# jzombie/rust-simd-r-drive

Measured on AMD Instinct MI355X. Metric: GiB/s hashed (device-resident), full-file validate+index scan, higher is better.
Workload: dtype u8

## Files before the change

include/srd_amd.h:

```cpp
#ifndef SRD_AMD_H
#define SRD_AMD_H
#include <stddef.h>
#include <stdint.h>

#ifdef __cplusplus
extern "C" {
#endif

#define SRD_OK 0
#define SRD_ERR_HIP (-1)
#define SRD_ERR_ALLOC (-2)
#define SRD_ERR_ARG (-3)
#define SRD_ERR_INTERNAL (-4)

#define SRD_MODE_OPTIMISTIC 0
#define SRD_MODE_FULL 1
#define SRD_MODE_SPAN_UNPROVEN 3

#define SRD_FULL_NONE 0
#define SRD_FULL_FORCED 1
#define SRD_FULL_SLOT_SPACE 2
#define SRD_FULL_WAVES 3
#define SRD_FULL_NO_START 4
#define SRD_FULL_UNPROVEN 5
#define SRD_FULL_CAP 6
#define SRD_FULL_LOOKBACK 7

#define SRD_FLAG_FORCE_FULL 1u
#define SRD_FLAG_NO_CRC 2u
#define SRD_FLAG_STAGE_PAGEABLE 4u
#define SRD_FLAG_STAGE_REGISTER 8u

typedef struct srd_ctx srd_ctx;

int srd_ctx_create(int device, srd_ctx **out);
void srd_ctx_destroy(srd_ctx *ctx);
void *srd_ctx_stream(srd_ctx *ctx);
uint64_t srd_ctx_device_bytes(srd_ctx *ctx);
int srd_ctx_scan_loads(srd_ctx *ctx);
int srd_ctx_scan_trial(srd_ctx *ctx, double *ms);
#define SRD_SCAN_BLOCKS_LAST 0
#define SRD_SCAN_BLOCKS_NEXT 1
#define SRD_SCAN_BLOCKS_EVEN 0
#define SRD_SCAN_BLOCKS_MEASURED 1
#define SRD_SCAN_BLOCKS_INSTALLED 2
typedef struct {
  uint64_t n_spans;
  uint32_t n_blocks;
  uint32_t source;
  uint32_t attempts;
  uint32_t first_source;
} srd_scan_blocks_info;
int srd_ctx_set_scan_blocks(srd_ctx *ctx, const uint64_t *starts,
                            uint32_t n_blocks, uint64_t n_spans);
int srd_ctx_scan_blocks(srd_ctx *ctx, int which, uint64_t *starts,
                        uint32_t cap, srd_scan_blocks_info *info);
const char *srd_last_error(void);
const char *srd_build_info(void);
#define SRD_TIMING_NONE 0
#define SRD_TIMING_SCAN 1
#define SRD_TIMING_CALL 2
int srd_ctx_set_timing(srd_ctx *ctx, int level);
int srd_ctx_set_timing_every(srd_ctx *ctx, int n);

int srd_ctx_timings(srd_ctx *ctx, double *scan_ms, int *scan_launches,
                    double *total_ms);
int srd_ctx_scan_list(srd_ctx *ctx, float *out, int cap);

typedef struct {
  uint64_t file_len;
  uint64_t final_len;
  uint64_t n_chain;
  uint64_t n_index;
  uint64_t n_crc_bad;
  uint64_t n_candidates;
  uint64_t full_reason;
  uint32_t mode;
  uint32_t reserved;
  uint64_t *meta_off, *key_hash, *prev_offset, *payload_start, *payload_len;
  uint32_t *crc_stored, *crc_computed;
  uint8_t *crc_ok;
  uint64_t *index_key_hash, *index_packed;
} srd_device_result;

uint64_t srd_padded_size(uint64_t file_len);

int srd_validate_index_device(srd_ctx *ctx, const uint8_t *d_file,
                              uint64_t file_len, uint32_t flags,
                              srd_device_result *out);

int srd_validate_span_device(srd_ctx *ctx, const uint8_t *d_span,
                             uint64_t span_off, uint64_t lo, uint64_t hi,
                             uint32_t flags, srd_device_result *out);

int srd_shard_cuts(const uint8_t *file, uint64_t file_len, uint32_t world,
                   uint64_t *cuts);

int srd_index_partition_device(srd_ctx *ctx, const uint64_t *d_keys,
                               const uint64_t *d_vals, uint64_t n,
                               uint32_t world, uint64_t *d_out_pairs,
                               uint64_t *counts);

int srd_index_build_device(srd_ctx *ctx, const uint64_t *d_pairs, uint64_t n,
                           uint64_t *d_out_keys, uint64_t *d_out_packed,
                           uint64_t *n_index);

typedef srd_device_result srd_result;
int srd_validate_index(srd_ctx *ctx, const uint8_t *file, uint64_t file_len,
                       uint32_t flags, srd_result *out);
void srd_result_free(srd_result *res);

int srd_validate_index_multi(srd_ctx *const *ctxs, uint32_t n_ctx,
                             const uint8_t *file, uint64_t file_len,
                             uint32_t flags, srd_result *out);

#define SRD_FLAG_MERGE_INDEX 16u
#define SRD_MULTI_COMPOSED 0u
#define SRD_MULTI_NEIGHBOUR 1u
#define SRD_MULTI_WHOLE_FILE 2u
typedef struct {
  uint64_t file_len, final_len;
  uint64_t n_chain, n_index, n_crc_bad, n_candidates;
  uint32_t mode;
  uint32_t path;
  uint32_t n_shards;
  uint32_t merged;
  uint32_t shard_errors;
  uint32_t peer_errors;
  double validate_ms;
  double exchange_ms;
  double total_ms;
  uint64_t *index_key_hash, *index_packed;
} srd_multi_summary;
int srd_validate_index_multi_device(srd_ctx *const *ctxs, uint32_t n_ctx,
                                    const uint8_t *const *d_spans,
                                    const uint64_t *span_offs,
                                    const uint64_t *cuts, uint32_t flags,
                                    srd_device_result *shards,
                                    srd_multi_summary *summary);
int srd_ctx_multi_summary(srd_ctx *ctx, srd_multi_summary *out);
int srd_ctx_multi_shard_ms(srd_ctx *ctx, double *out, int cap);
int srd_ctx_stage_info(srd_ctx *ctx, int *mode, double *stage_ms);

int srd_index_hash_device(srd_ctx *ctx, const uint64_t *d_keys, uint64_t n,
                          uint64_t *d_out, void *stream);

int srd_stream_probe_device(srd_ctx *ctx, const uint8_t *d_buf, uint64_t bytes,
                            int reps, double *best_ms, double *median_ms);

int srd_recover_valid_chain(srd_ctx *ctx, const uint8_t *file,
                            uint64_t file_len, uint64_t *final_len);

int srd_key_indexer_build(srd_ctx *ctx, const uint8_t *file, uint64_t tail,
                          uint64_t *key_hash_out, uint64_t *packed_out,
                          uint64_t cap, uint64_t *n_out);

int srd_crc32_batch(srd_ctx *ctx, const uint8_t *buf, uint64_t buf_len,
                    const uint64_t *offs, const uint64_t *lens, uint64_t n,
                    uint32_t *out);
int srd_crc32_batch_device(srd_ctx *ctx, const uint8_t *d_buf,
                           const uint64_t *d_offs, const uint64_t *d_lens,
                           uint64_t n, uint32_t *d_out, void *stream);

int srd_xxh3_64_batch(srd_ctx *ctx, const uint8_t *keys, uint64_t keys_len,
                      const uint64_t *offs, const uint64_t *lens, uint64_t n,
                      uint64_t *out);
int srd_xxh3_64_batch_device(srd_ctx *ctx, const uint8_t *d_keys,
                             const uint64_t *d_offs, const uint64_t *d_lens,
                             uint64_t n, uint64_t *d_out, void *stream);

#define SRD_WRITE_ALLOW_NULL 1u

typedef struct {
  uint64_t src;
  uint64_t len;
  uint64_t key_src;
  uint64_t tail;
  uint32_t key_len;
  uint32_t flags;
} srd_write_entry;
#define SRD_ENTRY_TOMB 1u
#define SRD_ENTRY_HASHED 2u

int srd_batch_layout(uint64_t tail, const uint8_t *payloads,
                     const uint64_t *key_offs, const uint64_t *key_lens,
                     const uint64_t *pay_offs, const uint64_t *pay_lens,
                     uint64_t n, uint32_t flags, srd_write_entry *out,
                     uint64_t *new_tail);

int srd_batch_write(srd_ctx *ctx, uint64_t tail, const uint8_t *keys,
                    const uint64_t *key_offs, const uint64_t *key_lens,
                    const uint8_t *payloads, const uint64_t *pay_offs,
// ... 119 lines not shown
```

rust-simd-r-drive_amd/csrc/srd_ctx.hip:

```cpp
static thread_local std::string g_err;
static void set_err(const std::string& s) { g_err = s; }

#define HIPCHK(x)                                                                         \
  do {                                                                                    \
    hipError_t e_ = (x);                                                                  \
    if (e_ != hipSuccess) {                                                               \
      set_err(std::string(#x) + ": " + hipGetErrorString(e_));                            \
      return SRD_ERR_HIP;                                                                 \
    }                                                                                     \
  } while (0)

namespace {

#define TRY(x)                 \
  do {                         \
    int r_ = (x);              \
    if (r_) return r_;         \
  } while (0)

static int launched(hipStream_t s, const char* name) {
  static const bool sync = [] { const char* e = getenv("SRD_SYNC_DEBUG"); return e && *e && *e != '0'; }();
  HIPCHK(hipGetLastError());
  if (!sync) return 0;
  hipError_t e = hipStreamSynchronize(s);
  if (e == hipSuccess) e = hipGetLastError();
  if (e == hipSuccess) return 0;
  set_err(std::string("kernel ") + name + ": " + hipGetErrorString(e));
  fprintf(stderr, "srd: kernel %s failed: %s\n", name, hipGetErrorString(e));
  return SRD_ERR_HIP;
}
#define LAUNCHED(s, name) TRY(launched(s, name))

struct Buf {
  void* p = nullptr;
  size_t n = 0;
};

struct CandCap {
  uint32_t cap;
  uint32_t grown_cap;
  uint64_t grown_bytes;
  uint32_t floor;
};

struct Worker {
  std::thread th;
  std::mutex mu;
  std::condition_variable cv;
  std::function<void()> job;
  bool has = false, stop = false;
  Worker() {
    th = std::thread([this] {
      std::unique_lock<std::mutex> lk(mu);
      for (;;) {
        cv.wait(lk, [this] { return has || stop; });
        if (!has) return;
        lk.unlock();
        job();
        lk.lock();
        has = false;
        job = nullptr;
        cv.notify_all();
      }
    });
  }
  ~Worker() {
    {
      std::lock_guard<std::mutex> lk(mu);
      stop = true;
    }
    cv.notify_all();
    th.join();
  }
  void post(std::function<void()> f) {
    std::lock_guard<std::mutex> lk(mu);
    job = std::move(f);
    has = true;
    cv.notify_all();
  }
  void wait() {
    std::unique_lock<std::mutex> lk(mu);
    cv.wait(lk, [this] { return !has; });
  }
};

struct Ctx {
  int device = 0;
  hipStream_t stream = nullptr;
  std::vector<Buf> bufs;
  CandCap copt{8, 8, 0, 8};
  CandCap cfull{32, 32, 0, 32};
  unsigned scan_blocks = 256;
  unsigned scan_cus = 256;
  uint32_t scan_wq[16] = {};
  uint32_t scan_variant = 0;
  uint64_t slot_limit = 1ull << 31;
  int loads_pin = -1;
  int last_loads = -1;
  struct LoadTune {
    uint64_t ns = ~0ull;
    uint32_t g = 0;
    uint32_t calls = 0;
    uint64_t best[2] = {0, 0};
    uint32_t n[2] = {0, 0};
    int choice = -1;
  } tune;
  bool glue_fused = true;
  uint32_t lb_fail = ~0u;
  bool xpart_on = true, xp_valid = false;
  uint32_t xp_par = 0, xp_g = 0;
  uint64_t xp_ns = 0;
  bool xp_installed = false;
  struct LastPart {
    bool any = false;
    uint64_t ns = 0;
    uint32_t g = 0, src = 0, par = 0;
    uint32_t attempts = 0, first_src = 0;
  } xp_last;
  srd_device_result res{};
  Buf file;
  hipEvent_t ev[4] = {nullptr, nullptr, nullptr, nullptr};
  int timing = SRD_TIMING_NONE;
  static constexpr uint32_t kScanRing = 64;
  hipEvent_t sev[2 * kScanRing] = {};
  uint32_t sev_next = 0, sev_pending = 0;
  double scan_ms = 0, total_ms = 0;
  int scan_launches = 0;
  uint32_t timing_every = 1, timing_seq = 0;
  std::vector<float> scan_list, scan_last;
  uint32_t gen = 0;
  uint64_t last_n = 0;
  Plan* h_plan = nullptr;
  uint64_t* h_pub = nullptr;
  uint64_t* h_small = nullptr;
  uint32_t pub_seq = 0;
  hipStream_t cstream = nullptr;
  hipEvent_t wev_copied[2] = {nullptr, nullptr}, wev_done[2] = {nullptr, nullptr};
  void* pin_ent[2] = {nullptr, nullptr};
  int stage_workers = 8;
  int stage_mode = -1;
  double stage_ms = 0;
  bool ev3_recorded = false;
  std::vector<void*> stage_pin;
  std::vector<hipStream_t> stage_streams;
  std::vector<hipEvent_t> stage_ev;
  srd_multi_summary last_multi{};
  std::vector<double> last_shard_ms;
  void* h_out = nullptr;
  uint64_t h_out_n = 0;
  uint8_t lgen = 0;
  Worker* worker = nullptr;
  hipEvent_t ev_ready = nullptr;
  bool ready_recorded = false;
};

enum BufId {
  B_TILE, B_SPAN_COUNT, B_SPAN_BASE,
  B_CM, B_CREC,
  B_COUNTERS,
  B_DM, B_DPAR, B_DSLOT, B_DHEAD, B_RUNHEAD, B_INTS, B_WALK,
  B_ST, B_JMP, B_VFLAG, B_VLIST, B_NV, B_VPOS, B_VPAR, B_VHEAD, B_VSLOT,
  B_ONPATH, B_CPOS, B_CHAIN_G, B_CORE,
  B_O_MO, B_O_KH, B_O_PREV, B_O_START, B_O_LEN, B_O_CRCST, B_O_CRC, B_O_OK,
  B_O_PIECES, B_O_SUF, B_O_SXM, B_O_TAIL, B_SLOW,
  B_HKEYS, B_HVALS, B_LATEST, B_IPOS, B_IKEY, B_IPACKED,
  B_CUB_TMP,
  B_PLAN, B_HASCHILD, B_CHILDOF, B_FLAG, B_PART, B_PARTEX, B_HOFF, B_SKEY, B_SIDX, B_LATEST8, B_XPART,
  B_MPLAN, B_MKEY, B_MVAL, B_PCNT, B_POFF, B_HASCHILD2,
  B_WPAY0, B_WPAY1, B_WKEY0, B_WKEY1, B_WENT0, B_WENT1, B_WKH, B_WMO,
  B_IT_FLAG, B_IT_POS, B_IT_ST, B_IT_EN, B_IT_KEPT, B_IT_OST, B_IT_OEN, B_IT_OKH, B_IT_ENT, B_IT_RLEN, B_IT_PST,
  B_GKEY, B_GVAL, B_GOKEY, B_GOPACKED,
  B_WTOT, B_WROOT, B_KTOT, B_DONE, B_SPAN_FIRST,
  B_XKEY, B_XVAL, B_GATHER, B_RFLAG, B_O_PACKED, B_VSCAN, B_LOOKB, B_PROBE, B_XTOT,
  B_LV_DSLOT, B_LV_DTOMB, B_LV_LSLOT, B_LV_OPS, B_LV_OPV, B_LV_CNT,
  B_LV_XK, B_LV_XP, B_LV_FLAG, B_LV_POS, B_LV_ENT, B_LV_TOMB,
  B_GA_ST, B_GA_PLEN, B_GA_CHK, B_GA_OFF, B_GA_CPRE, B_GA_CNT, B_GA_UNIT, B_GA_RAW, B_GA_CRC,
  B_AP_END, B_AP_NZ,
  B_CL_XK, B_CL_XP, B_CL_LEN, B_CL_MO, B_CL_PACKED, B_CL_CNT,
  B_COUNT_
};

int ensure(Ctx* c, BufId id, size_t bytes) {
  Buf& b = c->bufs[id];
  if (b.n >= bytes && b.p) return 0;
  if (b.p) HIPCHK(hipFree(b.p));
  b.p = nullptr;
  b.n = 0;
  size_t want = std::max<size_t>(bytes, 256);
  if (hipMalloc(&b.p, want) != hipSuccess) {
    set_err("hipMalloc failed for " + std::to_string(want) + " bytes");
    b.p = nullptr;
    return SRD_ERR_ALLOC;
  }
  b.n = want;
  return 0;
}
template <class T>
T* P(Ctx* c, BufId id) { return (T*)c->bufs[id].p; }

int ensure_z(Ctx* c, BufId id, size_t bytes) {
  void* before = c->bufs[id].p;
  size_t nb = c->bufs[id].n;
  int r = ensure(c, id, bytes);
  if (r) return r;
  if (c->bufs[id].p != before || c->bufs[id].n != nb) HIPCHK(hipMemsetAsync(c->bufs[id].p, 0, c->bufs[id].n, c->stream));
  return 0;
}

const CrcTables& host_tabs() {
  static CrcTables t;
  static const bool built = (build_crc_tables(t), true);
  (void)built;
  return t;
}

int upload_tables() {
  static std::mutex mu;
  std::lock_guard<std::mutex> lk(mu);
  const CrcTables& ht = host_tabs();
  int dev = 0;
  HIPCHK(hipGetDevice(&dev));
  static uint64_t uploaded = 0;
  if (uploaded & (1ull << dev)) return 0;
  DevTables t;
  memcpy(t.tab, ht.tab, sizeof t.tab);
  memcpy(t.lw, ht.lw, sizeof t.lw);
  memcpy(t.winit, ht.winit, sizeof t.winit);
  memcpy(t.zero_crc, ht.zero_crc, sizeof t.zero_crc);
  t.x32768 = ht.x32768;
  t.xtile[0] = kX0;
  for (int e = 1; e <= 64; e++) t.xtile[e] = mulp(ht.x32768, t.xtile[e - 1]);
  t.xt64[0] = kX0;
  for (int q = 1; q <= 64; q++) t.xt64[q] = mulp(t.xtile[64], t.xt64[q - 1]);
  for (int tb = 0; tb < 4; tb++)
    for (int b = 0; b < 256; b++) t.mx64[tb][b] = mulp(t.xtile[64], (uint32_t)b << (8 * tb));
  memcpy(t.pow8, ht.pow8, sizeof t.pow8);
  memcpy(t.invpow, ht.invpow, sizeof t.invpow);
  memcpy(t.m16k, ht.m16k, sizeof t.m16k);
  memcpy(t.m32k, ht.m32k, sizeof t.m32k);
  memcpy(t.mtk, ht.mtk, sizeof t.mtk);
  for (int pos = 0; pos < 8; pos++)
    for (int nb = 0; nb < 16; nb++)
      for (int l = 0; l < 32; l++)
        t.nib[((pos * 16 + nb) << 5) + l] = mulp(ht.lw[l + 32], (uint32_t)nb << (4 * pos));
  {
    for (int tb = 0; tb < 4; tb++)
      for (int b = 0; b < 256; b++) {
        for (int q = 0; q < 3; q++) {
          t.last[q][tb][b] = mulp(host_xpow8(ht, 4 + 16 * (3 - q)), (uint32_t)b << (8 * tb));
          t.last_c[q][tb][b] = mulp(host_xpow8(ht, 4 + 1024 * (3 - q)), (uint32_t)b << (8 * tb));
        }
        t.m4096[tb][b] = mulp(host_xpow8(ht, 512), (uint32_t)b << (8 * tb));
      }
    for (int pos = 0; pos < 8; pos++)
      for (int nb = 0; nb < 16; nb++)
        for (int l = 0; l < 32; l++)
          t.nib_c[((pos * 16 + nb) << 5) + l] = mulp(host_xpow8(ht, 16 * (31 - l)), (uint32_t)nb << (4 * pos));
  }
  HIPCHK(hipMemcpyToSymbol(HIP_SYMBOL(g_tabs), &t, sizeof t));
  uploaded |= 1ull << dev;
  return 0;
// ... 32 lines not shown
};
template <class T>
static SmallRead rd(const T* src, T* dst) { return SmallRead{src, dst, sizeof(T)}; }
static int read_small(Ctx* c, hipStream_t s, std::initializer_list<SmallRead> reads) {
  uint64_t* w = c->h_small + 8;
  for (const SmallRead& r : reads) {
    if (w + (r.bytes + 7) / 8 > c->h_small + 32) { set_err("internal: read_small over its pinned area"); return SRD_ERR_INTERNAL; }
    if (r.bytes) HIPCHK(hipMemcpyAsync(w, r.src, r.bytes, hipMemcpyDeviceToHost, s));
    w += (r.bytes + 7) / 8;
  }
  HIPCHK(spin_sync(s));
  w = c->h_small + 8;
  for (const SmallRead& r : reads) {
    if (r.bytes) memcpy(r.dst, w, r.bytes);
    w += (r.bytes + 7) / 8;
  }
  return 0;
}
static int enqueue_counters(Ctx* c) {
  HIPCHK(hipMemcpyAsync(c->h_small, P<uint64_t>(c, B_COUNTERS), 8 * 8, hipMemcpyDeviceToHost, c->stream));
  return 0;
}
static void counters_landed(Ctx* c, uint64_t* h) { memcpy(h, c->h_small, 64); }
int read_counters(Ctx* c, uint64_t* h, const uint64_t* extra_src = nullptr, uint64_t* extra = nullptr) {
  TRY(enqueue_counters(c));
  if (extra_src) TRY(read_small(c, c->stream, {rd(extra_src, extra)}));
  else HIPCHK(spin_sync(c->stream));
  counters_landed(c, h);
  return 0;
}

template <class In, class Out>
static int ensure_scan(Ctx* c, In in, Out out, uint64_t n) {
  size_t tb = 0;
  HIPCHK(hipcub::DeviceScan::ExclusiveSum(nullptr, tb, in, out, (int)n));
  return ensure(c, B_CUB_TMP, tb + 256);
}
template <class In, class Out>
static int scan_max(Ctx* c, In in, Out out, uint64_t n) {
  size_t tb = c->bufs[B_CUB_TMP].n;
  HIPCHK(hipcub::DeviceScan::InclusiveScan(P<void>(c, B_CUB_TMP), tb, in, out, hipcub::Max(), (int)n, c->stream));
  LAUNCHED(c->stream, "hipcub");
  return 0;
}
template <class In, class Out>
static int scan_sum(Ctx* c, In in, Out out, uint64_t n, hipStream_t s = nullptr) {
  if (!s) s = c->stream;
  size_t tb = c->bufs[B_CUB_TMP].n;
  HIPCHK(hipcub::DeviceScan::ExclusiveSum(P<void>(c, B_CUB_TMP), tb, in, out, (int)n, s));
  LAUNCHED(s, "hipcub");
  return 0;
}
template <class T, class U>
static int scan_sum_total(Ctx* c, T* in, U* out, uint64_t n, hipStream_t s, uint64_t* total, SmallRead r1 = {},
                          SmallRead r2 = {}, SmallRead r3 = {}) {
  if (!s) s = c->stream;
  TRY(scan_sum(c, in, out, n, s));
  U prefix{};
  typename std::remove_const<T>::type term{};
  TRY(read_small(c, s, {rd(out + n - 1, &prefix), rd(in + n - 1, &term), r1, r2, r3}));
  *total = (uint64_t)prefix + term;
  return 0;
}
static int sort_pairs48(Ctx* c, const uint64_t* kin, uint64_t* kout, const uint64_t* vin, uint64_t* vout, uint64_t n) {
  size_t tb = 0;
  HIPCHK(hipcub::DeviceRadixSort::SortPairs(nullptr, tb, kin, kout, vin, vout, (int)n, 0, 48, c->stream));
  TRY(ensure(c, B_CUB_TMP, tb + 256));
  tb = c->bufs[B_CUB_TMP].n;
  HIPCHK(hipcub::DeviceRadixSort::SortPairs(P<void>(c, B_CUB_TMP), tb, kin, kout, vin, vout, (int)n, 0, 48, c->stream));
  LAUNCHED(c->stream, "hipcub");
  return 0;
}

}

struct srd_ctx : Ctx {};

static int drain_scan_events(Ctx* c, uint32_t n) {
  for (; n && c->sev_pending; n--) {
    const uint32_t i = (c->sev_next - c->sev_pending) % Ctx::kScanRing;
    float ms = 0;
    HIPCHK(hipEventElapsedTime(&ms, c->sev[2 * i], c->sev[2 * i + 1]));
    c->scan_ms += ms;
    c->scan_launches++;
    if (c->scan_list.size() < (1u << 16)) c->scan_list.push_back(ms);
    c->sev_pending--;
  }
  return 0;
}
static int next_scan_events(Ctx* c, hipEvent_t* e0, hipEvent_t* e1) {
  *e0 = *e1 = nullptr;
  if (c->timing < SRD_TIMING_SCAN) return 0;
  if (c->timing_seq++ % c->timing_every) return 0;
  if (c->sev_pending == Ctx::kScanRing) TRY(drain_scan_events(c, 1));
  const uint32_t i = c->sev_next++ % Ctx::kScanRing;
  c->sev_pending++;
  *e0 = c->sev[2 * i];
  *e1 = c->sev[2 * i + 1];
  return 0;
}

static void weights_to_shares(const double (&f)[16], uint32_t (&wq)[16]) {
  double sum = 0;
  for (double x : f) sum += x;
  uint32_t used = 0;
  for (int v = 0; v < 15; v++) used += wq[v] = (uint32_t)(65536.0 * f[v] / sum);
  wq[15] = 65536 - used;
}

static void scan_weights(uint32_t (&wq)[16]) {
  double f[16] = {1.0000, 0.9787, 0.9796, 0.9788, 0.9081, 0.9072, 0.9074, 0.8915,
                  0.8432, 0.8324, 0.8337, 0.8314, 0.7726, 0.7701, 0.7712, 0.7590};
  if (const char* e = getenv("SRD_SCAN_WEIGHTS")) {
    double g[16], gs = 0;
    int n = 0;
    for (const char* q = e; n < 16 && *q;) {
      char* end = nullptr;
      const double x = strtod(q, &end);
      if (end == q || !(x > 0) || !std::isfinite(x)) { n = 0; break; }
      g[n++] = x;
      gs += x;
      q = *end == ',' ? end + 1 : end;
      if (*end && *end != ',') { n = 0; break; }
    }
    if (!std::isfinite(gs)) n = 0;
    if (n == 4)
      for (int v = 0; v < 16; v++) f[v] = g[v / 4];
    else if (n == 16)
      for (int v = 0; v < 16; v++) f[v] = g[v];
  }
  weights_to_shares(f, wq);
}
#ifdef SRD_DEBUG_API
extern "C" int srd_debug_set_scan_variant(srd_ctx* c, int v) {
  if (!c || !(v == 0 || v == 7 || v == 8 || v == SCAN_LINES)) return SRD_ERR_ARG;
  c->scan_variant = (uint32_t)v;
  return 0;
}
extern "C" int srd_debug_set_scan_bpc(srd_ctx* c, int bpc) {
  if (!c || bpc < 1 || bpc > 2) return SRD_ERR_ARG;
  c->scan_blocks = c->scan_cus * (unsigned)bpc;
  return 0;
}
extern "C" int srd_debug_set_xpart(srd_ctx* c, int on) {
  if (!c) return SRD_ERR_ARG;
  c->xpart_on = on != 0;
  return 0;
}
extern "C" int srd_debug_set_glue_fused(srd_ctx* c, int fused) {
  if (!c) return SRD_ERR_ARG;
  c->glue_fused = fused != 0;
  return 0;
}
extern "C" int srd_debug_set_scan_weights(srd_ctx* c, const double* w, int n) {
  if (!c || !w || (n != 4 && n != 16)) return SRD_ERR_ARG;
  double f[16], sum = 0;
  for (int v = 0; v < 16; v++) {
    sum += f[v] = n == 4 ? w[v / 4] : w[v];
    if (!(f[v] > 0) || !std::isfinite(f[v])) return SRD_ERR_ARG;
  }
  if (!std::isfinite(sum)) return SRD_ERR_ARG;
  weights_to_shares(f, c->scan_wq);
  return 0;
}
#endif
static int ctx_init(srd_ctx* c, int device) {
  c->device = device;
  c->bufs.resize(B_COUNT_);
  if (hipStreamCreateWithFlags(&c->stream, hipStreamNonBlocking) != hipSuccess) {
    set_err("hipStreamCreate failed");
    return SRD_ERR_HIP;
  }
  TRY(upload_tables());
  for (auto& e : c->ev) HIPCHK(hipEventCreateWithFlags(&e, hipEventReleaseToDevice));
  HIPCHK(hipEventCreateWithFlags(&c->ev_ready, hipEventDisableTiming));
  HIPCHK(hipHostMalloc((void**)&c->h_plan, sizeof(Plan), hipHostMallocDefault));
  HIPCHK(hipHostMalloc((void**)&c->h_pub, 64, hipHostMallocCoherent));
  memset(c->h_pub, 0, 64);
  HIPCHK(hipHostMalloc((void**)&c->h_small, 256, hipHostMallocDefault));
  c->stage_workers = (int)std::max(1u, std::min(8u, std::thread::hardware_concurrency()));
  int ncu = 0;
  if (hipDeviceGetAttribute(&ncu, hipDeviceAttributeMultiprocessorCount, device) == hipSuccess && ncu > 0)
    c->scan_cus = c->scan_blocks = (unsigned)ncu;
  scan_weights(c->scan_wq);
  if (const char* e = getenv("SRD_SLOT_LIMIT_LOG2")) {
    const long v = strtol(e, nullptr, 10);
    if (v >= 10 && v <= 31) c->slot_limit = 1ull << v;
  }
  if (const char* e = getenv("SRD_SCAN_LOADS")) {
    if (!strcmp(e, "lines")) c->loads_pin = SCAN_LINES;
    else if (!strcmp(e, "coal")) c->loads_pin = 0;
  }
  if (const char* e = getenv("SRD_GLUE_FUSED")) c->glue_fused = strcmp(e, "0") != 0;
  if (const char* e = getenv("SRD_XPART")) c->xpart_on = strcmp(e, "0") != 0;
  if (const char* e = getenv("SRD_LB_FAIL_BLOCK")) {
    char* end = nullptr;
    const unsigned long v = strtoul(e, &end, 10);
    if (end != e && v < CHAIN_BLOCKS) c->lb_fail = (uint32_t)v;
  }
  return 0;
}

extern "C" int srd_ctx_create(int device, srd_ctx** out) {
  if (!out) { set_err("null out"); return SRD_ERR_ARG; }
  int n = 0;
  HIPCHK(hipGetDeviceCount(&n));
  if (device < 0 || device >= n) { set_err("bad device index"); return SRD_ERR_ARG; }
  HIPCHK(hipSetDevice(device));
  auto* c = new srd_ctx();
  const int r = ctx_init(c, device);
  if (r) {
    srd_ctx_destroy(c);
    return r;
  }
  *out = c;
  return 0;
}

extern "C" void srd_ctx_destroy(srd_ctx* c) {
  if (!c) return;
  delete c->worker;
  hipSetDevice(c->device);
  if (c->ev_ready) hipEventDestroy(c->ev_ready);
  for (auto& b : c->bufs)
    if (b.p) hipFree(b.p);
  if (c->file.p) hipFree(c->file.p);
  for (auto& e : c->ev)
    if (e) hipEventDestroy(e);
  for (auto& e : c->sev)
    if (e) hipEventDestroy(e);
  if (c->h_plan) hipHostFree(c->h_plan);
  if (c->h_pub) hipHostFree(c->h_pub);
  if (c->h_small) hipHostFree(c->h_small);
  if (c->h_out) hipHostFree(c->h_out);
  for (int i = 0; i < 2; i++) {
    if (c->pin_ent[i]) hipHostFree(c->pin_ent[i]);
    if (c->wev_copied[i]) hipEventDestroy(c->wev_copied[i]);
    if (c->wev_done[i]) hipEventDestroy(c->wev_done[i]);
  }
  if (c->cstream) hipStreamDestroy(c->cstream);
  for (auto p : c->stage_pin)
    if (p) hipHostFree(p);
  for (auto e : c->stage_ev)
    if (e) hipEventDestroy(e);
  for (auto st : c->stage_streams)
    if (st) hipStreamDestroy(st);
  if (c->stream) hipStreamDestroy(c->stream);
  delete c;
}

extern "C" void* srd_ctx_stream(srd_ctx* c) { return c ? (void*)c->stream : nullptr; }
extern "C" int srd_ctx_scan_loads(srd_ctx* c) { return c ? c->last_loads : -1; }
extern "C" int srd_ctx_scan_trial(srd_ctx* c, double* ms) {
  if (!c) return -1;
  if (ms)
    for (int k = 0; k < 2; k++) ms[k] = c->tune.n[k] ? (double)c->tune.best[k] * 1e-5 : 0.0;
  return c->tune.choice;
}
extern "C" int srd_ctx_set_scan_blocks(srd_ctx* c, const uint64_t* starts, uint32_t n_blocks, uint64_t n_spans) {
  if (!c || !starts) { set_err("bad argument"); return SRD_ERR_ARG; }
  if (!c->xpart_on) { set_err("XCD-aware block shares are off on this context (SRD_XPART=0)"); return SRD_ERR_ARG; }
  if (!part_table_ok(starts, n_blocks, n_spans)) {
    set_err("bad argument: not a block-start table of n_blocks blocks over n_spans spans (srd_ctx_set_scan_blocks)");
    return SRD_ERR_ARG;
  }
  HIPCHK(hipSetDevice(c->device));
  TRY(ensure_z(c, B_XPART, sizeof(XPart)));
  HIPCHK(hipMemcpyAsync(&P<XPart>(c, B_XPART)->bs[c->xp_par][0], starts, ((size_t)n_blocks + 1) * 8,
                        hipMemcpyHostToDevice, c->stream));
  HIPCHK(hipStreamSynchronize(c->stream));
  c->xp_valid = true;
  c->xp_installed = true;
  c->xp_ns = n_spans;
  c->xp_g = n_blocks;
  return 0;
}
extern "C" int srd_ctx_scan_blocks(srd_ctx* c, int which, uint64_t* starts, uint32_t cap,
                                   srd_scan_blocks_info* info) {
  if (!c || !info || (cap && !starts) || (which != SRD_SCAN_BLOCKS_LAST && which != SRD_SCAN_BLOCKS_NEXT)) {
    set_err("bad argument");
    return SRD_ERR_ARG;
  }
  *info = srd_scan_blocks_info{};
  const Ctx::LastPart& l = c->xp_last;
  uint32_t par = 0;
  if (which == SRD_SCAN_BLOCKS_LAST) {
    if (!l.any) return 0;
    info->n_spans = l.ns;
    info->n_blocks = l.g;
    info->source = l.src;
    info->attempts = l.attempts;
    info->first_source = l.first_src;
    par = l.par;
  } else {
    if (!c->xp_valid) return 0;
    info->n_spans = c->xp_ns;
    info->n_blocks = c->xp_g;
    info->source = c->xp_installed ? SRD_SCAN_BLOCKS_INSTALLED : SRD_SCAN_BLOCKS_MEASURED;
    par = c->xp_par;
  }
  const size_t n = std::min<size_t>(cap, (size_t)info->n_blocks + 1);
  if (!n) return 0;
  if (info->source == SRD_SCAN_BLOCKS_EVEN) {
    for (size_t b = 0; b < n; b++) starts[b] = b * info->n_spans / info->n_blocks;
    return 0;
  }
  HIPCHK(hipSetDevice(c->device));
  HIPCHK(hipMemcpyAsync(starts, &P<XPart>(c, B_XPART)->bs[par][0], n * 8, hipMemcpyDeviceToHost, c->stream));
  HIPCHK(hipStreamSynchronize(c->stream));
  return 0;
}
extern "C" uint64_t srd_ctx_device_bytes(srd_ctx* c) {
  if (!c) return 0;
  uint64_t n = c->file.n;
  for (const Buf& b : c->bufs) n += b.n;
  return n;
}

extern "C" int srd_ctx_set_timing(srd_ctx* c, int level) {
  if (!c || level < SRD_TIMING_NONE || level > SRD_TIMING_CALL) { set_err("bad argument"); return SRD_ERR_ARG; }
  if (level >= SRD_TIMING_SCAN && !c->sev[0]) {
    HIPCHK(hipSetDevice(c->device));
    for (auto& e : c->sev) HIPCHK(hipEventCreateWithFlags(&e, hipEventReleaseToDevice));
  }
  c->timing = level;
  return 0;
}

extern "C" int srd_ctx_set_timing_every(srd_ctx* c, int n) {
  if (!c || n < 1) { set_err("bad argument"); return SRD_ERR_ARG; }
  c->timing_every = (uint32_t)n;
  c->timing_seq = 0;
  return 0;
}

extern "C" int srd_ctx_timings(srd_ctx* c, double* scan_ms, int* scan_launches, double* total_ms) {
  if (!c) { set_err("bad argument"); return SRD_ERR_ARG; }
  HIPCHK(hipSetDevice(c->device));
  TRY(drain_scan_events(c, c->sev_pending));
  if (scan_ms) *scan_ms = c->scan_ms;
  if (scan_launches) *scan_launches = c->scan_launches;
  if (total_ms) *total_ms = c->total_ms;
  c->scan_ms = 0;
  c->scan_launches = 0;
  c->scan_last.swap(c->scan_list);
  c->scan_list.clear();
  return 0;
}

extern "C" int srd_ctx_scan_list(srd_ctx* c, float* out, int cap) {
  if (!c || (cap > 0 && !out)) { set_err("bad argument"); return SRD_ERR_ARG; }
  const int n = (int)std::min<size_t>(c->scan_last.size(), (size_t)std::max(cap, 0));
  for (int i = 0; i < n; i++) out[i] = c->scan_last[i];
  return (int)c->scan_last.size();
}
```

rust-simd-r-drive_amd/csrc/srd_glue.hip:

```cpp
#pragma once

namespace srd {

#define GST(ptr, val) srd_gst(&(ptr), (val))

struct Plan {
  uint64_t K;
  uint64_t n_chain;
  uint64_t root_t;
  uint64_t start;
  uint64_t n_index;
  uint64_t n_bad;
  uint64_t n_slow;
  uint64_t chain_core;
  uint64_t max_root, top_gap, overflow;
  uint32_t status;
  uint32_t nroot;
  uint32_t troot;
  uint32_t idx_overflow;
  uint32_t idx_alias;
};
constexpr uint32_t ST_NOSTART = 1, ST_SHAPE = 2, ST_ROOTS = 4, ST_OVERFLOW = 16;
constexpr uint64_t NO_NODE = ~0ull;

constexpr int GLUE_BLOCKS = 1024;
constexpr int GLUE_THREADS = 256;

__device__ __forceinline__ uint32_t block_rank256(bool f, uint32_t* wsum, uint32_t* total) {
  const int lane = threadIdx.x & 63, w = threadIdx.x >> 6;
  const uint64_t bal = __ballot(f);
  const uint32_t pre = (uint32_t)__popcll(bal & ((1ull << lane) - 1));
  if (lane == 0) wsum[w] = (uint32_t)__popcll(bal);
  __syncthreads();
  uint32_t off = 0, tot = 0;
#pragma unroll
  for (int i = 0; i < 4; i++) {
    const uint32_t v = wsum[i];
    off += i < w ? v : 0u;
    tot += v;
  }
  __syncthreads();
  *total = tot;
  return off + pre;
}

template <int NW>
__device__ __forceinline__ uint32_t block_rank_n(bool f, uint32_t* wsum, uint32_t* total) {
  const int lane = threadIdx.x & 63, w = threadIdx.x >> 6;
  const uint64_t bal = __ballot(f);
  const uint32_t pre = (uint32_t)__popcll(bal & ((1ull << lane) - 1));
  if (lane == 0) wsum[w] = (uint32_t)__popcll(bal);
  __syncthreads();
  uint32_t off = 0, tot = 0;
#pragma unroll
  for (int i = 0; i < NW; i++) {
    const uint32_t v = wsum[i];
    off += i < w ? v : 0u;
    tot += v;
  }
  __syncthreads();
  *total = tot;
  return off + pre;
}
template <int NW>
__device__ __forceinline__ uint32_t block_sum_n(uint32_t v, uint32_t* wsum) {
  const int lane = threadIdx.x & 63, w = threadIdx.x >> 6;
#pragma unroll
  for (int o = 32; o; o >>= 1) v += __shfl_xor(v, o);
  if (lane == 0) wsum[w] = v;
  __syncthreads();
  uint32_t t = 0;
#pragma unroll
  for (int i = 0; i < NW; i++) t += wsum[i];
  __syncthreads();
  return t;
}
constexpr int CHAIN_BLOCKS = 256;
constexpr int CHAIN_THREADS = 1024;
constexpr int CHAIN_WAVES = CHAIN_THREADS / 64;

__device__ __forceinline__ uint32_t block_sum256(uint32_t v, uint32_t* wsum) {
  const int lane = threadIdx.x & 63, w = threadIdx.x >> 6;
#pragma unroll
  for (int o = 32; o; o >>= 1) v += __shfl_xor(v, o);
  if (lane == 0) wsum[w] = v;
  __syncthreads();
  const uint32_t t = wsum[0] + wsum[1] + wsum[2] + wsum[3];
  __syncthreads();
  return t;
}

__device__ __forceinline__ void chunk_of(uint64_t n, uint64_t* lo, uint64_t* hi) {
  const uint64_t ch = (n + gridDim.x - 1) / gridDim.x;
  *lo = min(n, (uint64_t)blockIdx.x * ch);
  *hi = min(n, *lo + ch);
}

__device__ __forceinline__ void block_prefix(const uint32_t* part, uint32_t np, uint32_t* wsum, uint64_t* before,
                                             uint64_t* total) {
  uint32_t b = 0, t = 0;
  for (uint32_t i = threadIdx.x; i < np; i += blockDim.x) {
    const uint32_t v = part[i];
    t += v;
    b += i < blockIdx.x ? v : 0u;
  }
  *before = block_sum256(b, wsum);
  *total = block_sum256(t, wsum);
}



__device__ uint64_t block_scan_partials(const uint32_t* part, uint32_t np, uint32_t* part_ex) {
  __shared__ uint64_t s[1024];
  const uint32_t t = threadIdx.x;
  uint64_t v = t < np ? part[t] : 0;
  s[t] = v;
  __syncthreads();
  for (uint32_t o = 1; o < 1024; o <<= 1) {
    const uint64_t a = t >= o ? s[t - o] : 0;
    __syncthreads();
    s[t] += a;
    __syncthreads();
  }
  if (t < np) part_ex[t] = (uint32_t)(s[t] - v);
  const uint64_t total = s[1023];
  __syncthreads();
  return total;
}

struct ShapeArgs {
  const uint8_t* file;
  uint64_t flen;
  uint32_t gen;
  const uint64_t* Kp;
  const uint64_t* wave_total;
  uint64_t wcap;
  uint32_t n_waves, wpb;
  uint64_t n_slots;
  const uint64_t* c_m;
  const int32_t* d_par;
  const u32x4* c_rec;
  const uint32_t* has_child;
  uint64_t* childof;
  uint8_t* flag;
  uint32_t* part;
  uint32_t* wpart;
  const unsigned long long* counters;
  Plan* plan;
  uint32_t coff;
  uint32_t* zero;
  uint32_t n_zero;
  uint32_t lb_fail;
};

__device__ __forceinline__ uint64_t start_node(const ShapeArgs& a) {
  const uint64_t t = a.counters[1], s1 = a.Kp[1];
  return (s1 && t >= 21 && a.c_m[s1 - 1] == t - 20) ? s1 - 1 : NO_NODE;
}
__device__ __forceinline__ bool dense_incomplete(const ShapeArgs& a) { return a.counters[2] != 0; }

constexpr uint32_t BW_MAX = 64;
__device__ __forceinline__ uint32_t block_waves(const ShapeArgs& a, uint32_t* s_pre) {
  const uint64_t w0 = (uint64_t)blockIdx.x * a.wpb;
  const uint32_t t = threadIdx.x, lane = t & 63;
  if (t < 64) {
    const uint64_t w = w0 + lane;
    const uint32_t c = lane < a.wpb && w < a.n_waves ? (uint32_t)min(a.wave_total[w] & ~(1ull << 63), a.wcap) : 0u;
    uint32_t x = c;
#pragma unroll
    for (int d = 1; d < 64; d <<= 1) {
      const uint32_t y = __shfl_up(x, d);
      if (lane >= (uint32_t)d) x += y;
    }
    s_pre[lane + 1] = x;
    if (lane == 0) s_pre[0] = 0;
  }
  __syncthreads();
  return s_pre[a.wpb];
}
__device__ __forceinline__ uint64_t slot_of(const ShapeArgs& a, const uint32_t* s_pre, uint32_t i) {
  uint32_t v = 0;
  for (uint32_t st = BW_MAX / 2; st; st >>= 1)
    if (v + st < a.wpb && s_pre[v + st] <= i) v += st;
  return ((uint64_t)blockIdx.x * a.wpb + v) * a.wcap + (i - s_pre[v]);
}

__device__ __forceinline__ bool is_core(const ShapeArgs& a, uint64_t g, uint64_t start) {
  if (g == start) return true;
  const int64_t p = a.d_par[g];
  return a.has_child[g] == a.gen && (p >= 0 || p == PAR_ROOT);
}

__global__ __launch_bounds__(256) void marks_from_claims_kernel(ShapeArgs a, uint32_t* marks_out) {
  if (dense_incomplete(a)) return;
  for (uint64_t g = (uint64_t)blockIdx.x * blockDim.x + threadIdx.x; g < a.n_slots; g += (uint64_t)gridDim.x * blockDim.x)
    if ((a.childof[g] >> 32) == a.gen) marks_out[g] = a.gen;
}

__global__ __launch_bounds__(256) void prune_kernel(ShapeArgs a, uint32_t* marks_out, uint32_t gen_out) {
  if (dense_incomplete(a)) return;
  const uint64_t start = start_node(a);
  for (uint64_t g = (uint64_t)blockIdx.x * blockDim.x + threadIdx.x; g < a.n_slots; g += (uint64_t)gridDim.x * blockDim.x) {
    const int64_t p = a.d_par[g];
    if (p >= 0 && is_core(a, g, start)) marks_out[p] = gen_out;
  }
}

__global__ __launch_bounds__(256) void child2_kernel(ShapeArgs a) {
  for (uint32_t i = blockIdx.x * blockDim.x + threadIdx.x; i < a.n_zero; i += gridDim.x * blockDim.x) a.zero[i] = 0;
  if (dense_incomplete(a)) return;
  const uint64_t start = start_node(a);
  const uint64_t K = a.n_slots;
  constexpr int CR = 4;
  const uint64_t stride = (uint64_t)gridDim.x * blockDim.x;
  for (uint64_t g0 = (uint64_t)blockIdx.x * blockDim.x + threadIdx.x; g0 < K; g0 += CR * stride) {
    int64_t par[CR];
    uint32_t hc[CR];
#pragma unroll
    for (int r = 0; r < CR; r++) {
      const uint64_t g = g0 + r * stride, gg = g < K ? g : g0;
      par[r] = a.d_par[gg];
      hc[r] = a.has_child[gg];
    }
#pragma unroll
    for (int r = 0; r < CR; r++) {
      const uint64_t g = g0 + r * stride;
      if (g >= K) break;
      const int64_t p = par[r];
      if (p >= 0 && (g == start || hc[r] == a.gen)) a.childof[p] = claim_word(a.gen, g);
    }
  }
}

enum Shape { SHAPE_LEAF, SHAPE_CORE, SHAPE_ROOT, SHAPE_FAIL };
template <class Linked, class IsStart>
__device__ __forceinline__ Shape shape_test(uint32_t gen, uint64_t g, int64_t p, int64_t pp, uint64_t cp, Linked linked,
                                            IsStart is_start) {
  if (!(is_start(g) || (linked(false) && (p >= 0 || p == PAR_ROOT)))) return SHAPE_LEAF;
  if (p == PAR_ROOT) return SHAPE_ROOT;
  if (p < 0 || !(is_start((uint64_t)p) || (linked(true) && (pp >= 0 || pp == PAR_ROOT)))) return SHAPE_FAIL;
  return cp != claim_word(gen, g) ? SHAPE_FAIL : SHAPE_CORE;
}
__global__ __launch_bounds__(CHAIN_THREADS) void check_kernel(ShapeArgs a) {
  __shared__ uint32_t wsum[CHAIN_WAVES];
  __shared__ uint32_t s_pre[BW_MAX + 1];
  if (dense_incomplete(a)) return;
  const uint64_t start = start_node(a);
  const uint64_t tag = (uint64_t)a.gen << 32;
  const bool marks = a.has_child != nullptr;
  const uint32_t n = block_waves(a, s_pre);
  uint32_t cnt = 0;
  bool fail = false;
  const uint32_t wi = threadIdx.x >> 6, lane = threadIdx.x & 63;
  const uint32_t chunk = (n + CHAIN_WAVES - 1) / CHAIN_WAVES;
  const uint32_t c0 = min(n, wi * chunk), c1 = min(n, c0 + chunk);
  constexpr int CR = 4;
  for (uint32_t base = c0; base < c1; base += CR * 64) {
    uint64_t g[CR], cg[CR], cp[CR];
    int64_t par[CR], pp[CR];
    uint32_t hc[CR], hp[CR];
    bool in[CR];
#pragma unroll
    for (int r = 0; r < CR; r++) {
      const uint32_t i = base + (uint32_t)r * 64 + lane;
      in[r] = i < c1;
      g[r] = slot_of(a, s_pre, in[r] ? i : c0);
      par[r] = a.d_par[g[r]];
      cg[r] = a.childof[g[r]];
      hc[r] = marks ? a.has_child[g[r]] : 0u;
    }
#pragma unroll
    for (int r = 0; r < CR; r++) {
      const uint64_t q = par[r] >= 0 ? (uint64_t)par[r] : g[r];
      pp[r] = a.d_par[q];
      cp[r] = a.childof[q];
      hp[r] = marks ? a.has_child[q] : 0u;
    }
#pragma unroll
    for (int r = 0; r < CR; r++) {
      if (!in[r]) break;
      const Shape s = shape_test(
          a.gen, g[r], par[r], pp[r], cp[r],
          [&](bool parent) {
            return marks ? (parent ? hp[r] : hc[r]) == a.gen : ((parent ? cp[r] : cg[r]) & ~0xffffffffull) == tag;
          },
          [&](uint64_t node) { return node == start; });
      GST(a.flag[g[r]], (uint8_t)(s != SHAPE_LEAF));
      if (s == SHAPE_LEAF) continue;
      cnt++;
      fail = fail || s == SHAPE_FAIL;
      if (s == SHAPE_ROOT) {
        atomicAdd(&a.plan->nroot, 1u);
        const u32x4 r0 = a.c_rec[g[r]];
        a.plan->root_t = (uint64_t)r0[0] | ((uint64_t)r0[1] << 32);
      }
    }
  }
  {
    uint32_t wc = cnt;
#pragma unroll
    for (int o = 32; o; o >>= 1) wc += __shfl_xor(wc, o);
    if (lane == 0) a.wpart[blockIdx.x * CHAIN_WAVES + wi] = wc;
  }
  const uint32_t tot = block_sum_n<CHAIN_WAVES>(cnt, wsum);
  if (__syncthreads_or(fail) && threadIdx.x == 0) atomicOr(&a.plan->status, ST_SHAPE);
  if (threadIdx.x == 0) a.part[blockIdx.x] = tot;
}

constexpr int IDX_HBLOCKS = 256;
constexpr int IDX_TCAP = 2048;
constexpr int IDX_BUCKET_AVG = 1280;
constexpr uint64_t IDX_EMPTY = ~0ull;
constexpr int PUB_WORDS = 7;

struct IdxArgs {
  const uint64_t* kh;
  const uint64_t* mo;
  const uint64_t* n_dev;
  const uint32_t* status;
  uint32_t log2_nbk;
  uint32_t* bfill;
  uint64_t* srec;
  uint8_t* latest;
  uint8_t lgen;
  uint32_t alias;
  uint64_t* pub;
  uint32_t pub_seq;
  uint32_t* ccount;
  const uint64_t* scan_ticks;
  uint64_t* okey;
  uint64_t* opacked;
  Plan* plan;
};

__device__ __forceinline__ uint64_t idx_n(const IdxArgs& a) { return *a.status ? 0 : *a.n_dev; }

template <int NW>
__device__ __forceinline__ void block_prefix_n(const uint32_t* part, uint32_t np, uint32_t* wsum, uint64_t* before,
                                               uint64_t* total) {
  uint32_t b = 0, t = 0;
  for (uint32_t i = threadIdx.x; i < np; i += blockDim.x) {
    const uint32_t v = part[i];
    t += v;
    b += i < blockIdx.x ? v : 0u;
  }
  *before = block_sum_n<NW>(b, wsum);
  *total = block_sum_n<NW>(t, wsum);
}

__device__ __forceinline__ uint32_t idx_bucket(uint64_t key, uint32_t log2_nbk) {
  return (uint32_t)(xxh3_64_u64(key) >> (64 - log2_nbk));
}
__device__ __forceinline__ uint64_t idx_rec(uint64_t hh, uint64_t c) { return (c << 32) | (uint32_t)hh; }

template <int NW, int R>
__device__ __forceinline__ uint32_t block_rank_rounds(const bool* f, uint32_t* wsum, uint32_t* rank) {
  const int lane = threadIdx.x & 63, w = threadIdx.x >> 6;
  const uint64_t lt = (1ull << lane) - 1;
  uint32_t pre[R];
#pragma unroll
  for (int r = 0; r < R; r++) {
    const uint64_t bal = __ballot(f[r]);
    pre[r] = (uint32_t)__popcll(bal & lt);
    if (lane == 0) wsum[r * NW + w] = (uint32_t)__popcll(bal);
  }
  __syncthreads();
  uint32_t acc = 0;
#pragma unroll
  for (int r = 0; r < R; r++) {
    uint32_t off = 0, t = 0;
#pragma unroll
    for (int i = 0; i < NW; i++) {
      const uint32_t v = wsum[r * NW + i];
      off += i < w ? v : 0u;
      t += v;
    }
    rank[r] = acc + off + pre[r];
    acc += t;
  }
  __syncthreads();
  return acc;
}

#ifndef SRD_FIN_R
#define SRD_FIN_R 2
#endif
constexpr int FIN_R = SRD_FIN_R;
constexpr uint32_t WSLOW = 256;

struct FinLds {
  uint32_t tab[1024];
  uint32_t m16k[1024];
  uint32_t m32k[1024];
  uint32_t mtk[3 * 1024];
  uint32_t winit[64], zero_crc[64];
  uint32_t invpow[4097];
};
constexpr int FIN_LDS_WORDS = 13;
__device__ __forceinline__ void fin_lds_words(FinLds& lt, uint32_t ti, uint32_t (&r)[FIN_LDS_WORDS], bool store) {
  static_assert(CHAIN_THREADS == 1024, "one word of each 1024-word table per thread");
  int i = 0;
  auto word = [&](uint32_t& dst, const uint32_t& src, bool mine = true) {
    if (!store) r[i] = src;
    else if (mine) dst = r[i];
    i++;
  };
  word(lt.tab[ti], (&g_tabs.tab[0][0])[ti]);
  word(lt.m16k[ti], (&g_tabs.m16k[0][0])[ti]);
  word(lt.m32k[ti], (&g_tabs.m32k[0][0])[ti]);
#pragma unroll
  for (int j = 0; j < 3; j++) word(lt.mtk[1024 * j + ti], (&g_tabs.mtk[0][0][0])[1024 * j + ti]);
#pragma unroll
  for (int j = 0; j < 4; j++) word(lt.invpow[1024 * j + ti], g_tabs.invpow[1024 * j + ti]);
  word(lt.invpow[4096], g_tabs.invpow[4096], ti == 0);
  word(lt.winit[ti & 63], g_tabs.winit[ti & 63], ti < 64);
  word(lt.zero_crc[ti & 63], g_tabs.zero_crc[ti & 63], ti < 64);
}


__device__ __forceinline__ bool fin_load_record(const ShapeArgs& a, const FinArgs& f, uint64_t gi, bool in, FinIn& e,
                                                uint64_t& kh, int64_t& par, uint32_t& own_suf) {
  const bool fl = in && a.flag[gi];
  par = a.d_par[gi];
  e.mo = f.c_m[gi];
  const u32x4 r0 = f.c_rec[gi], r1 = f.c_rec1[gi];
  e.p = (uint64_t)r0[0] | ((uint64_t)r0[1] << 32);
  kh = (uint64_t)r1[0] | ((uint64_t)r1[1] << 32);
  e.crc_st = r0[3];
  e.sxv = r1[2];
  e.fl = r0[2];
  own_suf = r1[3];
  return fl;
}
__device__ __forceinline__ uint32_t fin_rank(const bool (&fl)[FIN_R], uint64_t lt_mask, uint32_t (&rank)[FIN_R]) {
  uint32_t tot = 0;
#pragma unroll
  for (int r = 0; r < FIN_R; r++) {
    const uint64_t b = __ballot(fl[r]);
    rank[r] = tot + (uint32_t)__popcll(b & lt_mask);
    tot += (uint32_t)__popcll(b);
  }
  return tot;
}
__device__ __forceinline__ void fin_load_tiles(const FinArgs& f, bool fl, FinIn& e) {
  const u32x4* t4 = (const u32x4*)f.tile;
  const uint64_t mo = fl ? e.mo : f.flen - 1;
  const uint64_t st0 = fl ? fin_start(e.fl, e.p) : mo;
  e.t0 = t4[st0 / TILE];
  e.t1 = t4[mo / TILE];
}
struct SlowQueue {
  uint32_t* q;
  uint64_t run0;
  uint32_t n;
  __device__ __forceinline__ void flush(const FinArgs& f) {
    if (!n) return;
    const uint32_t lane = threadIdx.x & 63;
    wave_lds_sync();
    unsigned long long sbase = 0;
    if (lane == 0) sbase = atomicAdd(f.n_slow, (unsigned long long)n);
    sbase = __shfl(sbase, 0);
    for (uint32_t i = lane; i < n; i += 64) f.slow_list[sbase + i] = run0 + q[i];
    wave_lds_sync();
    n = 0;
  }
  __device__ __forceinline__ void push(const FinArgs& f, bool slow, uint64_t c, uint64_t lt_mask) {
    const uint64_t sb = __ballot(slow);
    const uint32_t k = (uint32_t)__popcll(sb);
    if (!k) return;
    if (n + k > WSLOW) flush(f);
    if (slow) q[n + __popcll(sb & lt_mask)] = (uint32_t)(c - run0);
    n += k;
  }
};
__device__ __forceinline__ void fin_emit(const FinArgs& f, const FinLds& lt, uint32_t* hist, uint32_t log2_nbk,
                                         uint64_t run, uint64_t lt_mask, const bool (&fl)[FIN_R],
                                         const uint32_t (&rank)[FIN_R], const FinIn (&e)[FIN_R],
                                         const uint64_t (&kh)[FIN_R], SlowQueue& sq) {
#pragma unroll
  for (int r = 0; r < FIN_R; r++) {
    if (!fl[r]) continue;
    const uint64_t c = run + rank[r];
    GST(f.o_mo[c], e[r].mo);
    GST(f.o_kh[c], kh[r]);
    GST(f.o_packed[c], ((kh[r] >> 48) << 48) | (e[r].mo & 0xFFFFFFFFFFFFull));
    GST(f.o_prev[c], e[r].p);
    GST(f.o_crc_st[c], e[r].crc_st);
    atomicAdd(&hist[idx_bucket(kh[r], log2_nbk)], 1u);
  }
#pragma unroll
  for (int r = 0; r < FIN_R; r++) {
    const uint64_t c = run + rank[r];
    sq.push(f, fl[r] && finalize_in<true>(f, c, e[r], lt), c, lt_mask);
  }
}

constexpr uint32_t ST_LOOKBACK = 32;
#ifdef SRD_GLUE_STAMPS
__device__ uint64_t g_glue_stamp[CHAIN_BLOCKS * 8];
#define GLUE_STAMP(i) \
  do { if (FUSED && threadIdx.x == 0) g_glue_stamp[blockIdx.x * 8 + (i)] = __builtin_amdgcn_s_memrealtime(); } while (0)
#else
#define GLUE_STAMP(i) do {} while (0)
#endif
constexpr uint64_t LB_CNT = (1ull << 35) - 1;
__device__ __forceinline__ uint64_t lb_pack(uint32_t tag, uint32_t st, bool fail, uint32_t nr, uint64_t cnt) {
  return ((uint64_t)tag << 40) | ((uint64_t)st << 38) | ((uint64_t)fail << 37) | ((uint64_t)min(nr, 3u) << 35) |
         (cnt & LB_CNT);
}
__device__ __forceinline__ uint32_t lb_tag(uint32_t gen) { return gen % 0xFFFFFFu + 1u; }
__device__ bool lb_lookback(unsigned long long* desc, uint32_t b, uint32_t tag, uint64_t* cnt, bool* fail,
                            uint32_t* nr) {
  typedef __attribute__((address_space(1))) unsigned long long gu64;
  const uint32_t lane = threadIdx.x & 63;
  uint64_t sum = 0;
  bool f = false;
  uint32_t n = 0;
  uint32_t spins = 0;
  for (int64_t j = (int64_t)b - 1; j >= 0; j -= 64) {
    const int64_t idx = j - (int64_t)lane;
    uint64_t v;
    for (;;) {
      v = idx >= 0 ? __hip_atomic_load((gu64*)(desc + idx), __ATOMIC_RELAXED, __HIP_MEMORY_SCOPE_AGENT)
                   : lb_pack(tag, 2, false, 0, 0);
      const bool ok = (v >> 40) == tag && ((v >> 38) & 3) != 0;
      if (__all(ok)) break;
      if (++spins > (1u << 22)) return false;
      __builtin_amdgcn_s_sleep(2);
    }
    const uint32_t stv = (uint32_t)(v >> 38) & 3u;
    const uint64_t inc = __ballot(stv >= 2);
    const uint32_t first = inc ? (uint32_t)__builtin_ctzll(inc) : 64u;
    const bool take = lane <= first;
    if (__ballot(take && stv == 3)) return false;
    uint64_t c = take ? (v & LB_CNT) : 0;
    uint32_t r = take ? (uint32_t)((v >> 35) & 3) : 0u;
    uint32_t fl = take ? (uint32_t)((v >> 37) & 1) : 0u;
#pragma unroll
    for (int o = 32; o; o >>= 1) {
      c += __shfl_xor(c, o);
      r += __shfl_xor(r, o);
      fl |= __shfl_xor(fl, o);
    }
    sum += c;
    n += r;
    f = f || fl;
    if (inc) break;
  }
  *cnt = sum;
  *fail = f;
  *nr = n;
  return true;
}

__device__ __forceinline__ uint32_t prev_lane(uint32_t v, uint32_t lane0) {
  return (uint32_t)__builtin_amdgcn_update_dpp((int)lane0, (int)v, DPP_WAVE_SHR1, 0xF, 0xF, false);
}
__device__ __forceinline__ uint64_t prev_lane64(uint64_t v, uint64_t lane0) {
  return (uint64_t)prev_lane((uint32_t)v, (uint32_t)lane0) | ((uint64_t)prev_lane((uint32_t)(v >> 32), (uint32_t)(lane0 >> 32)) << 32);
}
__device__ __forceinline__ uint64_t lane63_64(uint64_t v) {
  return (uint64_t)(uint32_t)__builtin_amdgcn_readlane((uint32_t)v, 63) |
         ((uint64_t)(uint32_t)__builtin_amdgcn_readlane((uint32_t)(v >> 32), 63) << 32);
}

template <bool FUSED>
__global__ __launch_bounds__(CHAIN_THREADS) void chain_finalize_kernel(ShapeArgs a, FinArgs f, IdxArgs ia,
                                                                      uint32_t log2_nbk,
                                                                      unsigned long long* lb_desc) {
  __shared__ uint32_t wsum[CHAIN_WAVES * FIN_R];
  __shared__ uint32_t s_pre[BW_MAX + 1];
  __shared__ uint32_t wslow[CHAIN_WAVES][WSLOW];
  __shared__ FinLds lt;
  extern __shared__ uint32_t hist[];
  GLUE_STAMP(0);
  uint32_t ltw[FIN_LDS_WORDS];
  fin_lds_words(lt, threadIdx.x, ltw, false);
  const uint64_t K = a.Kp[0];
  const bool incomplete = dense_incomplete(a);
  uint64_t before = 0, total = 0;
  if constexpr (!FUSED)
    block_prefix_n<CHAIN_WAVES>(a.part, incomplete ? 0u : (uint32_t)CHAIN_BLOCKS, wsum, &before, &total);
  Plan* pl = a.plan;
  uint32_t st = FUSED ? 0u : pl->status;
  const uint64_t top = a.counters[1];
  auto ld_prev_at = [&](uint64_t o) -> uint64_t {
    const uint32_t* q = (const uint32_t*)(a.file + (o & ~3ull));
    const uint32_t sh = (uint32_t)(o & 3) * 8, w0 = q[0], w1 = q[1], w2 = q[2];
    return (uint64_t)alignb(w1, w0, sh) | ((uint64_t)alignb(w2, w1, sh) << 32);
  };
  const bool troot = a.coff && top >= 21 && ld_prev_at(top - 12) == 0;
  uint64_t root_t = troot ? top : FUSED ? 0 : pl->root_t;
  if (a.counters[2]) st |= ST_OVERFLOW;
  const uint64_t s1 = a.Kp[1];
  const uint64_t start = FUSED ? NO_NODE : incomplete ? NO_NODE : start_node(a);
  if (!FUSED && start == NO_NODE) st |= ST_NOSTART;
  if (!FUSED && pl->nroot != 1) st |= ST_ROOTS;
  if (FUSED) st = 0;
  if (!FUSED) __syncthreads();
  const uint32_t nbk = 1u << log2_nbk;
  auto write_plan = [&](uint32_t s2, uint64_t tot) {
    pl->K = K;
    pl->max_root = a.counters[0];
    pl->top_gap = top ? a.flen - top : 0;
    pl->overflow = a.counters[2];
    pl->troot = troot;
    if (troot) {
      pl->status = 0;
      pl->n_chain = 1;
      pl->root_t = top;
      pl->chain_core = 0;
    } else {
      if (!FUSED) pl->start = start;
      pl->status = s2;
      pl->chain_core = tot;
      pl->n_chain = s2 ? 0 : a.coff + tot;
    }
  };
  const bool plan_block = FUSED ? blockIdx.x + 1 == gridDim.x : blockIdx.x == 0;
  if (!FUSED && plan_block && threadIdx.x == 0) write_plan(st, total);
  if (FUSED && troot && plan_block && threadIdx.x == 0) write_plan(0, 0);
  if (st && !troot) return;
  __shared__ uint32_t s_vcnt[BW_MAX];
  __shared__ uint64_t s_lb[2];
  __shared__ uint32_t s_fail, s_nroot, s_lbok;
  __shared__ unsigned long long s_root_t;
  if constexpr (FUSED) {
    if (!troot) {
      if (threadIdx.x == 0) { s_fail = 0; s_nroot = 0; s_root_t = 0; }
      __syncthreads();
      const uint64_t tag = (uint64_t)a.gen << 32;
      const uint32_t wi = threadIdx.x >> 6, lane = threadIdx.x & 63;
      uint32_t nr = 0;
      bool fail = false;
      constexpr int CR = 4;
      for (uint32_t v = wi; v < a.wpb; v += CHAIN_WAVES) {
        const uint64_t w = (uint64_t)blockIdx.x * a.wpb + v;
        const uint32_t n = w < a.n_waves ? (uint32_t)min(a.wave_total[w] & ~(1ull << 63), a.wcap) : 0u;
        const uint64_t gb = w * a.wcap;
        int64_t c_par = PAR_MISS;
        uint64_t c_cg = 0;
        uint32_t cnt = 0;
        for (uint32_t base = 0; base < n; base += CR * 64) {
          uint64_t g[CR], cg[CR], cp[CR];
          int64_t par[CR], pp[CR];
          bool in[CR], need[CR];
#pragma unroll
          for (int r = 0; r < CR; r++) {
            const uint32_t i = base + (uint32_t)r * 64 + lane;
            in[r] = i < n;
            g[r] = gb + (in[r] ? i : 0u);
            par[r] = a.d_par[g[r]];
            cg[r] = a.childof[g[r]];
          }
          bool any = false;
#pragma unroll
          for (int r = 0; r < CR; r++) {
            const uint32_t i = base + (uint32_t)r * 64 + lane;
            const int64_t l0p = r ? (int64_t)(int32_t)__builtin_amdgcn_readlane((uint32_t)par[r - 1], 63) : c_par;
            const uint64_t l0c = r ? lane63_64(cg[r - 1]) : c_cg;
            pp[r] = (int64_t)(int32_t)prev_lane((uint32_t)par[r], (uint32_t)l0p);
            cp[r] = prev_lane64(cg[r], l0c);
            need[r] = in[r] && par[r] >= 0 && !(i > 0 && (uint64_t)par[r] == g[r] - 1);
            any = any || need[r];
          }
          if (__ballot(any)) {
#pragma unroll
            for (int r = 0; r < CR; r++)
              if (need[r]) {
                pp[r] = a.d_par[par[r]];
                cp[r] = a.childof[par[r]];
              }
          }
          c_par = (int64_t)(int32_t)__builtin_amdgcn_readlane((uint32_t)par[CR - 1], 63);
          c_cg = lane63_64(cg[CR - 1]);
#pragma unroll
          for (int r = 0; r < CR; r++) {
            if (!in[r]) break;
            const Shape s = shape_test(
                a.gen, g[r], par[r], pp[r], cp[r],
                [&](bool parent) { return ((parent ? cp[r] : cg[r]) & ~0xffffffffull) == tag; },
                [&](uint64_t node) { return top >= 21 && node == s1 - 1 && a.c_m[node] == top - 20; });
            GST(a.flag[g[r]], (uint8_t)(s != SHAPE_LEAF));
            if (s == SHAPE_LEAF) continue;
            cnt++;
            fail = fail || s == SHAPE_FAIL;
            if (s == SHAPE_ROOT) {
              nr++;
              const u32x4 r0 = a.c_rec[g[r]];
              s_root_t = (uint64_t)r0[0] | ((uint64_t)r0[1] << 32);
            }
          }
        }
#pragma unroll
        for (int o = 32; o; o >>= 1) cnt += __shfl_xor(cnt, o);
        if (lane == 0) s_vcnt[v] = cnt;
      }
#pragma unroll
      for (int o = 32; o; o >>= 1) nr += __shfl_xor(nr, o);
      if (lane == 0 && nr) atomicAdd(&s_nroot, nr);
      if (__ballot(fail) && lane == 0) s_fail = 1;
      __syncthreads();
      GLUE_STAMP(1);
      for (uint32_t k = threadIdx.x; k < nbk; k += blockDim.x) hist[k] = 0;
      fin_lds_words(lt, threadIdx.x, ltw, true);
      uint32_t btot = 0;
      for (uint32_t v = 0; v < a.wpb; v++) btot += s_vcnt[v];
      const uint32_t ltag = lb_tag(a.gen);
      typedef __attribute__((address_space(1))) unsigned long long gu64;
      if (threadIdx.x == 0 && blockIdx.x > 0)
        __hip_atomic_store((gu64*)(lb_desc + blockIdx.x), lb_pack(ltag, 1, s_fail, s_nroot, btot), __ATOMIC_RELAXED,
                           __HIP_MEMORY_SCOPE_AGENT);
      if (wi == 0) {
        uint64_t pc = 0;
        bool pf = false;
        uint32_t pn = 0;
        const bool ok = blockIdx.x != a.lb_fail && lb_lookback(lb_desc, blockIdx.x, ltag, &pc, &pf, &pn);
        if (lane == 0) {
          const bool f2 = pf || s_fail;
          const uint32_t n2 = pn + s_nroot;
          __hip_atomic_store((gu64*)(lb_desc + blockIdx.x),
                             ok ? lb_pack(ltag, 2, f2, n2, pc + btot) : lb_pack(ltag, 3, true, 0, 0), __ATOMIC_RELAXED,
                             __HIP_MEMORY_SCOPE_AGENT);
          s_lb[0] = pc;
          s_lb[1] = pc + btot;
          s_lbok = ok;
          if (plan_block) {
            const uint64_t stn = incomplete ? NO_NODE : start_node(a);
            pl->start = stn;
            write_plan((ok ? 0u : ST_LOOKBACK) | (f2 ? ST_SHAPE : 0u) | (n2 != 1 ? ST_ROOTS : 0u) |
                           (a.counters[2] ? ST_OVERFLOW : 0u) | (stn == NO_NODE ? ST_NOSTART : 0u),
                       pc + btot);
          }
        }
      }
      __syncthreads();
      GLUE_STAMP(2);
      before = s_lb[0];
      total = s_lb[1];
      if (!s_lbok) return;
      root_t = s_root_t;
    }
  }
  if (!FUSED || troot) {
    for (uint32_t k = threadIdx.x; k < nbk; k += blockDim.x) hist[k] = 0;
    fin_lds_words(lt, threadIdx.x, ltw, true);
    __syncthreads();
  }
  GLUE_STAMP(3);
  bool root_slow = false;
  const bool root_block = FUSED && !troot ? root_t != 0 : blockIdx.x == 0;
  if (root_block && a.coff && threadIdx.x == 0) {
    uint64_t kh;
    root_slow = finalize_core<true>(f, 0, NO_REC, -1, root_t, &kh, lt);
    atomicAdd(&hist[idx_bucket(kh, log2_nbk)], 1u);
  }
  uint64_t bend = a.coff + before;
  if (!troot) {
    const uint32_t wi = threadIdx.x >> 6, lane = threadIdx.x & 63;
    const uint64_t lt_mask = (1ull << lane) - 1;
    SlowQueue sq = {wslow[wi], 0, 0};
    if constexpr (FUSED) {
      uint32_t btot = 0;
      for (uint32_t v = 0; v < a.wpb; v++) btot += s_vcnt[v];
      bend += btot;
      for (uint32_t v = wi; v < a.wpb; v += CHAIN_WAVES) {
        const uint64_t w = (uint64_t)blockIdx.x * a.wpb + v;
        const uint32_t n = w < a.n_waves ? (uint32_t)min(a.wave_total[w] & ~(1ull << 63), a.wcap) : 0u;
        const uint64_t gb = w * a.wcap;
        uint32_t voff = 0;
        for (uint32_t u = 0; u < v; u++) voff += s_vcnt[u];
        uint64_t run = a.coff + before + voff;
        sq.run0 = run;
        uint32_t c_fl = F_NO_PARENT, c_suf = 0;
        for (uint32_t base = 0; base < n; base += 64 * FIN_R) {
          bool fl[FIN_R];
          uint64_t gi[FIN_R], kh[FIN_R];
          int64_t par[FIN_R];
          uint32_t psuf[FIN_R], rank[FIN_R];
          FinIn e[FIN_R];
#pragma unroll
          for (int r = 0; r < FIN_R; r++) {
            const uint32_t i = base + (uint32_t)r * 64 + lane;
            gi[r] = gb + (i < n ? i : 0u);
            fl[r] = fin_load_record(a, f, gi[r], i < n, e[r], kh[r], par[r], psuf[r]);
          }
          const uint32_t tot = fin_rank(fl, lt_mask, rank);
          bool any = false, need[FIN_R];
#pragma unroll
          for (int r = 0; r < FIN_R; r++) {
            const uint32_t i = base + (uint32_t)r * 64 + lane;
            const uint32_t l0f = r ? (uint32_t)__builtin_amdgcn_readlane(e[r - 1].fl, 63) : c_fl;
            const uint32_t l0s = r ? (uint32_t)__builtin_amdgcn_readlane(psuf[r - 1], 63) : c_suf;
            const uint32_t nf = prev_lane(e[r].fl, l0f), ns = prev_lane(psuf[r], l0s);
            need[r] = fl[r] && par[r] >= 0 && !(i > 0 && (uint64_t)par[r] == gi[r] - 1);
            any = any || need[r];
            e[r].pfl = par[r] >= 0 ? nf : F_NO_PARENT;
            e[r].psuf = ns;
            fin_load_tiles(f, fl[r], e[r]);
          }
          if (__ballot(any)) {
#pragma unroll
            for (int r = 0; r < FIN_R; r++)
              if (need[r]) {
                e[r].pfl = f.c_rec[par[r]][2];
                e[r].psuf = f.c_rec1[par[r]][3];
              }
          }
          c_fl = (uint32_t)__builtin_amdgcn_readlane(e[FIN_R - 1].fl, 63);
          c_suf = (uint32_t)__builtin_amdgcn_readlane(psuf[FIN_R - 1], 63);
          fin_emit(f, lt, hist, log2_nbk, run, lt_mask, fl, rank, e, kh, sq);
          run += tot;
        }
        sq.flush(f);
      }
    } else {
      const uint32_t n = block_waves(a, s_pre);
      uint32_t woff, btot;
      {
        const uint32_t v = lane < CHAIN_WAVES ? a.wpart[blockIdx.x * CHAIN_WAVES + lane] : 0u;
        uint32_t x = lane < wi ? v : 0u, y = v;
#pragma unroll
        for (int o = 32; o; o >>= 1) {
          x += __shfl_xor(x, o);
          y += __shfl_xor(y, o);
        }
        woff = x;
        btot = y;
      }
      bend += btot;
      uint64_t run = a.coff + before + woff;
      sq.run0 = run;
      const uint32_t chunk = (n + CHAIN_WAVES - 1) / CHAIN_WAVES;
      const uint32_t c0 = min(n, wi * chunk), c1 = min(n, c0 + chunk);
      for (uint32_t base = c0; base < c1; base += 64 * FIN_R) {
        bool fl[FIN_R];
        uint64_t gi[FIN_R], kh[FIN_R];
        int64_t par[FIN_R];
        uint32_t own_suf, rank[FIN_R];
        FinIn e[FIN_R];
#pragma unroll
        for (int r = 0; r < FIN_R; r++) {
          const uint32_t i = base + (uint32_t)r * 64 + lane;
          gi[r] = slot_of(a, s_pre, i < c1 ? i : c0);
          fl[r] = fin_load_record(a, f, gi[r], i < c1, e[r], kh[r], par[r], own_suf);
        }
        const uint32_t tot = fin_rank(fl, lt_mask, rank);
#pragma unroll
        for (int r = 0; r < FIN_R; r++) {
          const uint64_t pg = fl[r] && par[r] >= 0 ? (uint64_t)par[r] : gi[r];
          e[r].pfl = par[r] >= 0 ? f.c_rec[pg][2] : F_NO_PARENT;
          e[r].psuf = f.c_rec1[pg][3];
          fin_load_tiles(f, fl[r], e[r]);
        }
        fin_emit(f, lt, hist, log2_nbk, run, lt_mask, fl, rank, e, kh, sq);
        run += tot;
      }
      sq.flush(f);
    }
  }
  if (root_slow) f.slow_list[atomicAdd(f.n_slow, 1ull)] = 0;
  __syncthreads();
  GLUE_STAMP(4);
  for (uint32_t k = threadIdx.x; k < nbk; k += blockDim.x) {
    const uint32_t n = hist[k];
    hist[k] = n ? atomicAdd(&ia.bfill[k], n) : 0u;
  }
  __syncthreads();
  GLUE_STAMP(5);
  uint64_t clo, chi;
  if constexpr (FUSED) {
    clo = troot ? 0 : a.coff + before;
    chi = troot ? (blockIdx.x == 0 ? 1 : 0) : bend;
    if (!troot && root_block && a.coff && threadIdx.x == 0) {
      const uint64_t h0 = xxh3_64_u64(f.o_kh[0]);
      const uint32_t bk = (uint32_t)(h0 >> (64 - log2_nbk));
      const uint32_t pos = atomicAdd(&hist[bk], 1u);
      if (pos < IDX_TCAP) ia.srec[(uint64_t)bk * IDX_TCAP + pos] = idx_rec(h0, 0);
    }
  } else {
    const uint64_t n_chain = troot ? 1 : a.coff + total;
    clo = min(n_chain, blockIdx.x ? a.coff + before : 0);
    chi = min(n_chain, bend);
  }
  constexpr int SR = 4;
  for (uint64_t base = clo; base < chi; base += SR * CHAIN_THREADS) {
    uint64_t k[SR];
#pragma unroll
    for (int r = 0; r < SR; r++) {
      const uint64_t c = base + (uint64_t)r * CHAIN_THREADS + threadIdx.x;
      k[r] = f.o_kh[c < chi ? c : clo];
    }
#pragma unroll
    for (int r = 0; r < SR; r++) {
      const uint64_t c = base + (uint64_t)r * CHAIN_THREADS + threadIdx.x;
      if (c >= chi) break;
      const uint64_t hh = xxh3_64_u64(k[r]);
      const uint32_t bk = (uint32_t)(hh >> (64 - log2_nbk));
      const uint32_t pos = atomicAdd(&hist[bk], 1u);
      if (pos < IDX_TCAP) ia.srec[(uint64_t)bk * IDX_TCAP + pos] = idx_rec(hh, c);
    }
  }
  GLUE_STAMP(6);
}

__global__ void index_prep_kernel(Plan* pl, uint64_t n, uint32_t* zero, uint32_t nz) {
  const uint32_t i = blockIdx.x * blockDim.x + threadIdx.x;
  if (i < nz) zero[i] = 0;
  if (i < sizeof(Plan) / 4) ((uint32_t*)pl)[i] = 0;
  __syncthreads();
  if (i == 0) pl->n_chain = n;
}
__global__ void index_prep_dev_kernel(Plan* pl, const uint64_t* d_n, uint32_t* zero, uint32_t nz) {
  const uint32_t i = blockIdx.x * blockDim.x + threadIdx.x;
  if (i < nz) zero[i] = 0;
  if (i < sizeof(Plan) / 4) ((uint32_t*)pl)[i] = 0;
  __syncthreads();
  if (i == 0) pl->n_chain = *d_n;
}
__global__ __launch_bounds__(256) void idx_hist_scatter_kernel(IdxArgs a) {
  extern __shared__ uint32_t lds_u32[];
  const uint32_t nbk = 1u << a.log2_nbk;
  for (uint32_t k = threadIdx.x; k < nbk; k += blockDim.x) lds_u32[k] = 0;
  __syncthreads();
  uint64_t lo, hi;
  chunk_of(idx_n(a), &lo, &hi);
  for (uint64_t c = lo + threadIdx.x; c < hi; c += blockDim.x)
    atomicAdd(&lds_u32[xxh3_64_u64(a.kh[c]) >> (64 - a.log2_nbk)], 1u);
  __syncthreads();
  for (uint32_t k = threadIdx.x; k < nbk; k += blockDim.x) {
    const uint32_t n = lds_u32[k];
    lds_u32[k] = n ? atomicAdd(&a.bfill[k], n) : 0u;
  }
  __syncthreads();
  for (uint64_t c = lo + threadIdx.x; c < hi; c += blockDim.x) {
    const uint64_t hh = xxh3_64_u64(a.kh[c]);
    const uint32_t bk = (uint32_t)(hh >> (64 - a.log2_nbk));
    const uint32_t pos = atomicAdd(&lds_u32[bk], 1u);
    if (pos < IDX_TCAP) a.srec[(uint64_t)bk * IDX_TCAP + pos] = idx_rec(hh, c);
  }
}

__device__ __forceinline__ void publish_outcome(const IdxArgs& a, const Plan* pl, uint64_t n, uint64_t nl_total) {
  const uint64_t tag = (uint64_t)a.pub_seq << 32;
  const uint32_t fl = (pl->status & 0xffu) | (a.alias && nl_total == 0 ? 0x100u : 0u) | (pl->idx_overflow ? 0x200u : 0u);
  const uint64_t w[PUB_WORDS] = {tag | fl, tag | (uint32_t)pl->n_chain, tag | (uint32_t)(n - nl_total),
                                 tag | (uint32_t)pl->n_bad, tag | (uint32_t)pl->K, tag | (uint32_t)pl->top_gap,
                                 tag | (a.scan_ticks ? (uint32_t)min<uint64_t>(*a.scan_ticks, 0xFFFFFFFFull) : 0u)};
#pragma unroll
  for (int i = 0; i < PUB_WORDS; i++) __hip_atomic_store(a.pub + i, w[i], __ATOMIC_RELAXED, __HIP_MEMORY_SCOPE_SYSTEM);
}

constexpr int DD_SLOTS = 3 * IDX_TCAP / 2;
constexpr uint32_t DD_EMPTY32 = 0xFFFFFFFFu;
__global__ __launch_bounds__(512) __attribute__((amdgpu_waves_per_eu(8, 8))) void idx_dedup_kernel(IdxArgs a, FinArgs f) {
  __shared__ unsigned long long dd_lds[DD_SLOTS + DD_SLOTS / 2];
  unsigned long long* const keys = dd_lds;
  uint32_t* const vals = (uint32_t*)(dd_lds + DD_SLOTS);
  __shared__ uint32_t special, collide;
  if (f.n_slow) {
    const unsigned long long ns = *f.n_slow;
    constexpr uint32_t NW = 512 / 64;
    if ((uint64_t)blockIdx.x * NW < ns) {
      static_assert(sizeof(SlowLds) <= sizeof(dd_lds), "the slow path's tables in the hash table's LDS");
      SlowLds& L = *reinterpret_cast<SlowLds*>(dd_lds);
      load_slow_lds(L);
      __syncthreads();
      for (uint64_t q = (uint64_t)blockIdx.x * NW + (threadIdx.x >> 6); q < ns; q += (uint64_t)gridDim.x * NW)
        slow_one(f, f.slow_list[q], L);
      __syncthreads();
    }
  }
  if (*a.status) return;
  const uint32_t k = blockIdx.x;
  const uint32_t fill = a.bfill[k];
  if (fill == 0) return;
  if (fill > IDX_TCAP) {
    if (threadIdx.x == 0) a.plan->idx_overflow = 1;
    return;
  }
  const uint64_t lo = (uint64_t)k * IDX_TCAP, hi = lo + fill;
  constexpr int DR = IDX_TCAP / 512;
  uint64_t rec[DR];
  uint32_t slot[DR];
  bool in[DR], mark[DR];
#pragma unroll
  for (int r = 0; r < DR; r++) {
    const uint64_t i = lo + (uint64_t)r * 512 + threadIdx.x;
    in[r] = i < hi;
    rec[r] = a.srec[in[r] ? i : lo];
    mark[r] = false;
  }
  uint32_t slots = 64;
  while (slots < 2 * (hi - lo) && slots < 2048) slots <<= 1;
  const bool pw2 = slots >= 2 * (hi - lo);
  if (!pw2) slots = DD_SLOTS;
  const uint32_t M = slots - 1;
  auto slot_of = [&](uint32_t h) { return pw2 ? h & M : (uint32_t)(((uint64_t)h * DD_SLOTS) >> 32); };
  uint32_t* const hkeys = (uint32_t*)dd_lds;
  for (uint32_t i = threadIdx.x; i < slots; i += blockDim.x) { hkeys[i] = DD_EMPTY32; vals[i] = 0; }
  if (threadIdx.x == 0) { special = 0; collide = 0; }
  __syncthreads();
#pragma unroll
  for (int r = 0; r < DR; r++) {
    if (!in[r]) break;
    const uint32_t h = (uint32_t)rec[r], hk = h == DD_EMPTY32 ? DD_EMPTY32 - 1 : h;
    const uint32_t v = (uint32_t)(rec[r] >> 32) + 1;
    uint32_t s = slot_of(h);
    while (true) {
      const uint32_t old = atomicCAS(&hkeys[s], DD_EMPTY32, hk);
      if (old == DD_EMPTY32 || old == hk) { atomicMax(&vals[s], v); break; }
      s = s == M ? 0u : s + 1;
    }
    slot[r] = s;
  }
  __syncthreads();
#pragma unroll
  for (int r = 0; r < DR; r++) {
    if (!in[r]) break;
    const uint32_t c = (uint32_t)(rec[r] >> 32), best = vals[slot[r]];
    if (best != c + 1) {
      if (a.kh[c] == a.kh[best - 1]) mark[r] = true;
      else collide = 1;
    }
  }
  __syncthreads();
  if (collide) {
    uint64_t key[DR];
#pragma unroll
    for (int r = 0; r < DR; r++) key[r] = in[r] ? a.kh[(uint32_t)(rec[r] >> 32)] : 0;
    for (uint32_t i = threadIdx.x; i < slots; i += blockDim.x) { keys[i] = IDX_EMPTY; vals[i] = 0; }
    __syncthreads();
#pragma unroll
    for (int r = 0; r < DR; r++) {
      if (!in[r]) break;
      const uint32_t v = (uint32_t)(rec[r] >> 32) + 1;
      if (key[r] == IDX_EMPTY) { atomicMax(&special, v); continue; }
      uint32_t s = slot_of((uint32_t)xxh3_64_u64(key[r]));
      while (true) {
        const unsigned long long old = atomicCAS(&keys[s], (unsigned long long)IDX_EMPTY, (unsigned long long)key[r]);
        if (old == IDX_EMPTY || old == key[r]) { atomicMax(&vals[s], v); break; }
        s = s == M ? 0u : s + 1;
      }
      slot[r] = s;
    }
    __syncthreads();
#pragma unroll
    for (int r = 0; r < DR; r++) {
      if (!in[r]) break;
      const uint32_t c = (uint32_t)(rec[r] >> 32);
      mark[r] = (key[r] == IDX_EMPTY ? special : vals[slot[r]]) != c + 1;
    }
  }
  const uint64_t n = idx_n(a);
  const uint64_t ch = n ? (n + GLUE_BLOCKS - 1) / GLUE_BLOCKS : 1;
#pragma unroll
  for (int r = 0; r < DR; r++) {
    if (!mark[r]) continue;
    const uint32_t c = (uint32_t)(rec[r] >> 32);
    a.latest[c] = a.lgen;
    atomicAdd(&a.ccount[c / ch], 1u);
  }
}

__global__ __launch_bounds__(256) void idx_emit_kernel(IdxArgs a) {
  __shared__ uint32_t wsum[4];
  const uint64_t n = idx_n(a);
  uint64_t nl_before = 0, nl_total = 0;
  block_prefix(a.ccount, GLUE_BLOCKS, wsum, &nl_before, &nl_total);
  if (blockIdx.x == 0 && threadIdx.x == 0) {
    a.plan->n_index = n - nl_total;
    a.plan->idx_alias = a.alias && nl_total == 0;
    if (a.pub) publish_outcome(a, a.plan, n, nl_total);
  }
  if (a.alias && nl_total == 0) return;
  uint64_t lo, hi;
  chunk_of(n, &lo, &hi);
  uint64_t run = lo - nl_before;
  constexpr int ER = 4;
  __shared__ uint32_t wsum_r[4 * ER];
  for (uint64_t base = lo; base < hi; base += ER * 256) {
    bool f[ER];
    uint64_t key[ER], mo[ER];
#pragma unroll
    for (int r = 0; r < ER; r++) {
      const uint64_t c = base + (uint64_t)r * 256 + threadIdx.x, cc = c < hi ? c : lo;
      f[r] = c < hi && a.latest[cc] != a.lgen;
      key[r] = a.kh[cc];
      mo[r] = a.mo[cc];
    }
    uint32_t rank[ER];
    const uint32_t tot = block_rank_rounds<4, ER>(f, wsum_r, rank);
#pragma unroll
    for (int r = 0; r < ER; r++) {
      if (!f[r]) continue;
      a.okey[run + rank[r]] = key[r];
      a.opacked[run + rank[r]] = ((key[r] >> 48) << 48) | (mo[r] & 0xFFFFFFFFFFFFull);
    }
    run += tot;
  }
}

__device__ __forceinline__ uint32_t owner_of(uint64_t key, uint32_t world) {
  return (uint32_t)(((key >> 32) * (uint64_t)world) >> 32);
}
constexpr uint32_t PART_MAX_WORLD = 64;
struct PartArgs {
  const uint64_t* keys;
  const uint64_t* vals;
  uint64_t n;
  uint32_t world;
  uint32_t* cnt;
  uint32_t* off;
  uint64_t* out;
  uint64_t* out_v;
  uint64_t* counts;
};
__global__ __launch_bounds__(256) void part_count_kernel(PartArgs a) {
  __shared__ uint32_t h[PART_MAX_WORLD];
  for (uint32_t o = threadIdx.x; o < a.world; o += blockDim.x) h[o] = 0;
  if (blockIdx.x == 0 && threadIdx.x == 0) a.cnt[(uint64_t)a.world * GLUE_BLOCKS] = 0;
  __syncthreads();
  uint64_t lo, hi;
  chunk_of(a.n, &lo, &hi);
  for (uint64_t i = lo + threadIdx.x; i < hi; i += blockDim.x) atomicAdd(&h[owner_of(a.keys[i], a.world)], 1u);
  __syncthreads();
  for (uint32_t o = threadIdx.x; o < a.world; o += blockDim.x) a.cnt[(uint64_t)o * GLUE_BLOCKS + blockIdx.x] = h[o];
// ... 110 lines not shown
```

rust-simd-r-drive_amd/csrc/srd_index_build.hip:

```cpp

static int alloc_hash(Ctx* c, uint64_t n) {
  const uint64_t hc = table_capacity(n);
  TRY(ensure(c, B_HKEYS, hc * 8));
  TRY(ensure(c, B_HVALS, hc * 8));
  TRY(ensure(c, B_LATEST, (n + 1) * 4));
  TRY(ensure(c, B_IPOS, (n + 1) * 4));
  TRY(ensure_cub(c, n + 1));
  return 0;
}

static int index_global(Ctx* c, uint64_t n, uint64_t* n_index, const uint64_t* kh = nullptr,
                        const uint64_t* mo = nullptr, uint64_t* okey = nullptr, uint64_t* opacked = nullptr) {
  if (!kh) { kh = P<uint64_t>(c, B_O_KH); mo = P<uint64_t>(c, B_O_MO); }
  TRY(alloc_hash(c, n));
  if (!okey) { okey = P<uint64_t>(c, B_IKEY); opacked = P<uint64_t>(c, B_IPACKED); }
  uint64_t* cnt = P<uint64_t>(c, B_COUNTERS);
  const uint64_t hc = table_capacity(n);
  HIPCHK(hipMemsetAsync(P<void>(c, B_HKEYS), 0xff, hc * 8, c->stream));
  HIPCHK(hipMemsetAsync(P<void>(c, B_HVALS), 0, hc * 8, c->stream));
  HIPCHK(hipMemsetAsync(cnt + 7, 0, 8, c->stream));
  HIPCHK(hipMemsetAsync(P<uint32_t>(c, B_LATEST) + n, 0, 4, c->stream));
  if (n) {
    index_insert_kernel<<<blocks(n, 256), 256, 0, c->stream>>>(
        kh, mo, n, P<uint64_t>(c, B_HKEYS), P<unsigned long long>(c, B_HVALS), hc - 1, (unsigned long long*)(cnt + 7));
    LAUNCHED(c->stream, "index_insert_kernel");
    index_latest_kernel<<<blocks(n, 256), 256, 0, c->stream>>>(
        kh, mo, n, P<uint64_t>(c, B_HKEYS), P<unsigned long long>(c, B_HVALS), hc - 1, (unsigned long long*)(cnt + 7),
        P<uint32_t>(c, B_LATEST));
    LAUNCHED(c->stream, "index_latest_kernel");
  }
  TRY(scan_sum(c, P<uint32_t>(c, B_LATEST), P<uint32_t>(c, B_IPOS), n + 1));
  if (n) {
    index_emit_kernel<<<blocks(n, 256), 256, 0, c->stream>>>(kh, mo, P<uint32_t>(c, B_LATEST), P<uint32_t>(c, B_IPOS),
                                                             n, okey, opacked);
    LAUNCHED(c->stream, "index_emit_kernel");
  }
  uint32_t nidx = 0;
  TRY(read_small(c, c->stream, {rd(P<uint32_t>(c, B_IPOS) + n, &nidx)}));
  *n_index = nidx;
  return 0;
}

static int alloc_index(Ctx* c, uint64_t n_cap, uint32_t log2_nbk) {
  const uint64_t nbk = (uint64_t)1 << log2_nbk;
  TRY(ensure(c, B_HOFF, (nbk + GLUE_BLOCKS) * 4));
  TRY(ensure(c, B_SKEY, nbk * IDX_TCAP * 8));
  TRY(ensure_z(c, B_LATEST8, n_cap + 1));
  return 0;
}
static int next_lgen(Ctx* c) {
  if (++c->lgen == 0) {
    HIPCHK(hipMemsetAsync(P<void>(c, B_LATEST8), 0, c->bufs[B_LATEST8].n, c->stream));
    c->lgen = 1;
  }
  return 0;
}
static uint32_t* index_zero_words(Ctx* c, uint32_t log2_nbk, uint32_t* n) {
  *n = (1u << log2_nbk) + GLUE_BLOCKS;
  return P<uint32_t>(c, B_HOFF);
}
static uint32_t index_log2_buckets(uint64_t n_est) {
  uint32_t log2_nbk = 1;
  while (log2_nbk < 14 && ((uint64_t)IDX_BUCKET_AVG << log2_nbk) < n_est) log2_nbk++;
  return log2_nbk;
}
static IdxArgs index_args(Ctx* c, uint32_t log2_nbk) {
  IdxArgs ia{};
  ia.log2_nbk = log2_nbk;
  ia.bfill = P<uint32_t>(c, B_HOFF);
  ia.ccount = ia.bfill + ((size_t)1 << log2_nbk);
  ia.srec = P<uint64_t>(c, B_SKEY);
  ia.latest = P<uint8_t>(c, B_LATEST8);
  ia.lgen = c->lgen;
  return ia;
}
static int launch_index_bucketed(Ctx* c, const uint64_t* kh, const uint64_t* mo, const uint64_t* n_dev,
                                 const uint32_t* status, uint32_t log2_nbk, uint64_t* okey, uint64_t* opacked,
                                 Plan* pl, bool fused = false, const FinArgs* slow = nullptr, bool zeroed = false,
                                 const uint64_t* scan_ticks = nullptr) {
  TRY(next_lgen(c));
  IdxArgs ia = index_args(c, log2_nbk);
  ia.alias = fused ? 1u : 0u;
  if (fused) {
    ia.pub = c->h_pub;
    ia.pub_seq = ++c->pub_seq;
    ia.scan_ticks = scan_ticks;
  }
  ia.kh = kh;
  ia.mo = mo;
  ia.n_dev = n_dev;
  ia.status = status;
  ia.okey = okey;
  ia.opacked = opacked;
  ia.plan = pl;
  const uint32_t nbk = 1u << log2_nbk;
  if (!fused) {
    uint32_t nz = 0;
    uint32_t* zw = index_zero_words(c, log2_nbk, &nz);
    if (!zeroed) HIPCHK(hipMemsetAsync(zw, 0, (size_t)nz * 4, c->stream));
    idx_hist_scatter_kernel<<<IDX_HBLOCKS, 256, nbk * 4, c->stream>>>(ia);
    LAUNCHED(c->stream, "idx_hist_scatter_kernel");
  }
  FinArgs fs{};
  if (slow) fs = *slow;
  idx_dedup_kernel<<<nbk, 512, 0, c->stream>>>(ia, fs);
  LAUNCHED(c->stream, "idx_dedup_kernel");
  idx_emit_kernel<<<GLUE_BLOCKS, GLUE_THREADS, 0, c->stream>>>(ia);
  LAUNCHED(c->stream, "idx_emit_kernel");
  return 0;
}

static int partition_impl(Ctx* c, const uint64_t* keys, const uint64_t* vals, uint64_t n, uint32_t world,
                          uint64_t* out, uint64_t* out_v, uint64_t* counts, const uint64_t** d_counts = nullptr) {
  const uint64_t nc = (uint64_t)world * GLUE_BLOCKS + 1;
  TRY(ensure(c, B_PCNT, nc * 4));
  TRY(ensure(c, B_POFF, nc * 4 + 8 * PART_MAX_WORLD));
  TRY(ensure_cub(c, nc));
  PartArgs a{};
  a.keys = keys;
  a.vals = vals;
  a.n = n;
  a.world = world;
  a.cnt = P<uint32_t>(c, B_PCNT);
  a.off = P<uint32_t>(c, B_POFF);
  a.out = out;
  a.out_v = out_v;
  a.counts = (uint64_t*)(P<uint32_t>(c, B_POFF) + ((nc + 1) & ~1ull));
  part_count_kernel<<<GLUE_BLOCKS, 256, 0, c->stream>>>(a);
  LAUNCHED(c->stream, "part_count_kernel");
  TRY(scan_sum(c, a.cnt, a.off, nc));
  part_scatter_kernel<<<GLUE_BLOCKS, 256, 0, c->stream>>>(a);
  LAUNCHED(c->stream, "part_scatter_kernel");
  part_counts_kernel<<<1, 64, 0, c->stream>>>(a);
  LAUNCHED(c->stream, "part_counts_kernel");
  if (d_counts) *d_counts = a.counts;
  if (counts) {
    HIPCHK(hipMemcpyAsync(counts, a.counts, world * 8, hipMemcpyDeviceToHost, c->stream));
    HIPCHK(spin_sync(c->stream));
  }
  return 0;
}

extern "C" int srd_index_partition_device(srd_ctx* c, const uint64_t* d_keys, const uint64_t* d_vals, uint64_t n,
                                          uint32_t world, uint64_t* d_out_pairs, uint64_t* counts) {
  if (!c || !counts || world == 0 || world > PART_MAX_WORLD || (n && (!d_keys || !d_vals || !d_out_pairs))) {
    set_err("bad argument");
    return SRD_ERR_ARG;
  }
  HIPCHK(hipSetDevice(c->device));
  return partition_impl(c, d_keys, d_vals, n, world, d_out_pairs, nullptr, counts);
}

static int index_build_sep(Ctx* c, const uint64_t* keys, const uint64_t* vals, uint64_t n, uint64_t* okeys,
                           uint64_t* opacked, uint64_t* n_index, const uint64_t* d_n = nullptr,
                           uint64_t n_est = 0) {
  *n_index = 0;
  if (!n) return 0;
  TRY(ensure(c, B_MPLAN, sizeof(Plan)));
  const uint32_t log2_nbk = index_log2_buckets(d_n ? std::max<uint64_t>(n_est, 1) : n);
  TRY(alloc_index(c, n, log2_nbk));
  Plan* pl = P<Plan>(c, B_MPLAN);
  uint32_t nz = 0;
  uint32_t* zw = index_zero_words(c, log2_nbk, &nz);
  if (d_n) {
    index_prep_dev_kernel<<<(std::max<uint32_t>(nz, 64) + 255) / 256, 256, 0, c->stream>>>(pl, d_n, zw, nz);
    LAUNCHED(c->stream, "index_prep_dev_kernel");
  } else {
    index_prep_kernel<<<(nz + 255) / 256, 256, 0, c->stream>>>(pl, n, zw, nz);
    LAUNCHED(c->stream, "index_prep_kernel");
  }
  TRY(launch_index_bucketed(c, keys, vals, &pl->n_chain, &pl->status, log2_nbk, okeys, opacked, pl, false, nullptr,
                            true));
  HIPCHK(hipMemcpyAsync(c->h_plan, pl, sizeof(Plan), hipMemcpyDeviceToHost, c->stream));
  HIPCHK(spin_sync(c->stream));
  if (c->h_plan->idx_overflow) return index_global(c, c->h_plan->n_chain, n_index, keys, vals, okeys, opacked);
  *n_index = c->h_plan->n_index;
  return 0;
}

extern "C" int srd_index_build_device(srd_ctx* c, const uint64_t* d_pairs, uint64_t n, uint64_t* d_out_keys,
                                      uint64_t* d_out_packed, uint64_t* n_index) {
  if (!c || !n_index || (n && (!d_pairs || !d_out_keys || !d_out_packed))) { set_err("bad argument"); return SRD_ERR_ARG; }
  if (n >= (1ull << 31)) { set_err("too many pairs"); return SRD_ERR_ARG; }
  HIPCHK(hipSetDevice(c->device));
  *n_index = 0;
  if (!n) return 0;
  TRY(ensure(c, B_MKEY, n * 8));
  TRY(ensure(c, B_MVAL, n * 8));
  deinterleave_kernel<<<blocks(std::min<uint64_t>(n, 1 << 20), 256), 256, 0, c->stream>>>(
      d_pairs, n, P<uint64_t>(c, B_MKEY), P<uint64_t>(c, B_MVAL));
  LAUNCHED(c->stream, "deinterleave_kernel");
  return index_build_sep(c, P<uint64_t>(c, B_MKEY), P<uint64_t>(c, B_MVAL), n, d_out_keys, d_out_packed, n_index);
}

extern "C" int srd_index_hash_device(srd_ctx* c, const uint64_t* d_keys, uint64_t n, uint64_t* d_out, void* stream) {
  if (!c || (n && (!d_keys || !d_out))) { set_err("bad argument"); return SRD_ERR_ARG; }
  if (!n) return 0;
  HIPCHK(hipSetDevice(c->device));
  hipStream_t s = stream_of(c, stream);
  index_hash_kernel<<<(unsigned)std::min<uint64_t>((n + 255) / 256, 8192), 256, 0, s>>>(d_keys, n, d_out);
  LAUNCHED(s, "index_hash_kernel");
  return 0;
}
```

rust-simd-r-drive_amd/csrc/srd_kernels.hip:

```cpp
#include <hip/hip_runtime.h>
#include <stdint.h>

#include "srd_crc.h"
#include "srd_xxh3.h"
#include "srd_part.h"
#include "srd_fin.h"

namespace srd {


typedef uint32_t u32x4 __attribute__((ext_vector_type(4)));
typedef uint64_t u64x2 __attribute__((ext_vector_type(2)));
typedef uint16_t u16x2 __attribute__((ext_vector_type(2)));

constexpr int SPAN_TILES = 4;
constexpr uint64_t SPAN_BYTES = (uint64_t)TILE * SPAN_TILES;
constexpr int64_t PAR_ROOT = -1;
constexpr int64_t PAR_MISS = -2;

constexpr uint32_t F_NT = 256u, F_ZB = 512u;

struct DevTables {
  uint32_t tab[4][256];
  uint32_t lw[64];
  uint32_t winit[64];
  uint32_t zero_crc[64];
  uint32_t x32768;
  uint32_t pow8[64];
  uint32_t invpow[4097];
  alignas(16) uint32_t nib[8 * 16 * 32];
  uint32_t m16k[4][256];
  alignas(16) uint32_t last[3][4][256];
  uint32_t xtile[65];
  uint32_t xt64[65];
  uint32_t mx64[4][256];
  alignas(16) uint32_t last_c[3][4][256];
  alignas(16) uint32_t nib_c[8 * 16 * 32];
  uint32_t m4096[4][256];
  uint32_t m32k[4][256];
  uint32_t mtk[3][4][256];
};
__device__ DevTables g_tabs;
#ifdef SRD_WAVE_STAMPS
__device__ uint64_t g_wave_stamp[8192 + 1024];
#ifdef SRD_WAVE_STAMPS
__device__ uint64_t g_wave_clk[4096 + 256];
#endif
#endif

constexpr float XP_CLAMP = 0.10f;
struct XPart {
  uint64_t bs[2][XP_MAX_BLOCKS + 1];
  uint32_t xcc[XP_MAX_BLOCKS];
  uint32_t dur[XP_MAX_BLOCKS];
  uint64_t t0[XP_MAX_BLOCKS];
  float w[8];
  uint64_t scan_ticks;
};

struct ScanArgs {
  ScanPart part;
  const uint8_t* file;
  uint64_t flen;
  uint64_t n_tiles, n_spans;
  uint32_t cap;
  uint32_t* tile;
  uint32_t* span_count;
  uint64_t* c_m;
  u32x4* c_rec;
  u32x4* c_rec1;
  unsigned long long* counters;
  uint32_t filt_hb;
  uint64_t k_lo;
  uint64_t m_lo;
  uint32_t* zero_words;
  uint32_t n_zero_words;
  uint32_t* sentinel;
  uint64_t* wave_total;
  uint64_t* wave_root;
  uint64_t* k_total;
  uint32_t* done;
  uint32_t* span_first;
  uint64_t wcap;
  int32_t* d_par;
  unsigned long long* childof;
  uint32_t gen;
  uint64_t span_lo;
  uint32_t* zero2;
  uint32_t n_zero2;
  uint32_t variant;
  XPart* xp;
  uint32_t xp_next;
};

__device__ __forceinline__ uint32_t ld_dw_guarded(const uint8_t* f, uint64_t n, uint64_t o) {
  if (o + 4 <= n) return *(const uint32_t*)(f + o);
  uint32_t v = 0;
  for (int k = 0; k < 4; k++)
    if (o + k < n) v |= (uint32_t)f[o + k] << (8 * k);
  return v;
}
__device__ __forceinline__ uint64_t ld_u64_unaligned(const uint8_t* f, uint64_t o) {
  uint64_t v = 0;
  for (int k = 0; k < 8; k++) v |= (uint64_t)f[o + k] << (8 * k);
  return v;
}
__device__ __forceinline__ uint32_t ld_u32_unaligned(const uint8_t* f, uint64_t o) {
  uint32_t v = 0;
  for (int k = 0; k < 4; k++) v |= (uint32_t)f[o + k] << (8 * k);
  return v;
}

#ifndef SRD_GLUE_STORE
#define SRD_GLUE_STORE 1
#endif
template <class T, class V>
__device__ __forceinline__ void srd_gst(T* p, V v) {
  if constexpr (SRD_GLUE_STORE == 1) __hip_atomic_store(p, (T)v, __ATOMIC_RELAXED, __HIP_MEMORY_SCOPE_SYSTEM);
  else if constexpr (SRD_GLUE_STORE == 2) __hip_atomic_store(p, (T)v, __ATOMIC_RELAXED, __HIP_MEMORY_SCOPE_AGENT);
  else __builtin_nontemporal_store((T)v, p);
}

__device__ __forceinline__ unsigned long long claim_word(uint32_t gen, uint64_t g) {
  return ((unsigned long long)gen << 32) | (0xffffffffull - (g & 0xffffffffull));
}
__device__ __forceinline__ void ld_meta(const uint8_t* f, uint64_t m, uint64_t* kh, uint64_t* p, uint32_t* crc) {
  const uint32_t* q = (const uint32_t*)(f + (m & ~3ull));
  const uint32_t sh = (uint32_t)(m & 3) * 8;
  uint32_t w[6], v[5];
#pragma unroll
  for (int i = 0; i < 6; i++) w[i] = q[i];
#pragma unroll
  for (int i = 0; i < 5; i++) v[i] = __builtin_amdgcn_alignbit(w[i + 1], w[i], sh);
  *kh = (uint64_t)v[0] | ((uint64_t)v[1] << 32);
  *p = (uint64_t)v[2] | ((uint64_t)v[3] << 32);
  *crc = v[4];
}
__device__ __forceinline__ uint32_t mask_past_end(uint32_t v, uint64_t o, uint64_t n) {
  if (o + 4 <= n) return v;
  if (o >= n) return 0u;
  return v & ((1u << (8 * (uint32_t)(n - o))) - 1u);
}
__device__ __forceinline__ uint32_t mask_past_end32(uint32_t v, uint32_t o, uint32_t n) {
  if (o + 4 <= n) return v;
  if (o >= n) return 0u;
  return v & ((1u << (8 * (n - o))) - 1u);
}

typedef uint32_t u32x2 __attribute__((ext_vector_type(2)));
constexpr uint32_t OOB_OFF = 0xFFFFFFFFu;
__device__ __forceinline__ __amdgpu_buffer_rsrc_t out_rsrc(const void* base, uint32_t bytes) {
  return __builtin_amdgcn_make_buffer_rsrc(const_cast<void*>(base), 0, (int)bytes, 0x00020000);
}

__device__ __forceinline__ uint32_t alignb(uint32_t hi, uint32_t lo, uint32_t sh) {
  return __builtin_amdgcn_alignbit(hi, lo, sh);
}

__device__ __forceinline__ uint64_t wave_max_u64(uint64_t v) {
  for (int o = 32; o > 0; o >>= 1) {
    uint64_t w = __shfl_xor(v, o);
    v = w > v ? w : v;
  }
  return v;
}

constexpr int SCAN_WAVES_V2 = 16;
struct alignas(2048) ScanLds {
  uint32_t last[3 * 4 * 256];
  uint32_t tab[4 * 256 * 32];
  uint32_t nib[8 * 16 * 32];
  uint32_t win[SCAN_WAVES_V2][24];
  uint64_t s_root[SCAN_WAVES_V2], s_ovf[SCAN_WAVES_V2];
// ... 40 lines not shown
  return (uint32_t)__builtin_amdgcn_update_dpp(0, (int)v, CTRL, 0xF, 0xF, true);
}
constexpr int DPP_WAVE_SHL1 = 0x130;
constexpr int DPP_WAVE_SHR1 = 0x138;
constexpr int DPP_ROW_SHL = 0x100;

__device__ __forceinline__ uint32_t lane_weight(uint32_t c, const uint32_t* __restrict__ nib, int lane) {
  uint32_t v[8];
  const char* base = (const char*)(nib + (lane & 31));
#pragma unroll
  for (int pos = 0; pos < 8; pos++) {
    const uint32_t nb = __builtin_amdgcn_ubfe(c, 4 * pos, 4);
    v[pos] = *(const uint32_t*)(base + pos * 2048 + (nb << 7));
  }
  return xor3(xor3(v[0], v[1], v[2]), xor3(v[3], v[4], v[5]), v[6] ^ v[7]);
}
__device__ int srd_llvm_writelane(int val, int lane, int old) __asm("llvm.amdgcn.writelane.i32");
__device__ __forceinline__ uint32_t writelane_u32(uint32_t val, int lane, uint32_t old) {
  return (uint32_t)srd_llvm_writelane((int)val, lane, (int)old);
}
__device__ __forceinline__ uint32_t lds_off(const void* p) {
  return (uint32_t)(uintptr_t)(const __attribute__((address_space(3))) void*)p;
}
__device__ __forceinline__ uint32_t lds_ld(uint32_t off) {
  return *(const __attribute__((address_space(3))) uint32_t*)(uintptr_t)off;
}
__device__ __forceinline__ uint32_t crc_line4_wide(const uint32_t (&d)[16], const ScanLds& L, const uint32_t (&R)[4]) {
  constexpr uint32_t SEL0 = 0x0c020400u, SEL1 = 0x0c020500u, SEL2 = 0x0c020600u, SEL3 = 0x0c020700u;
  uint32_t s[4] = {d[0], d[4], d[8], d[12]};
  __builtin_amdgcn_sched_barrier(0);
#pragma unroll
  for (int j = 0; j < 3; j++) {
    uint32_t t[4][4];
#pragma unroll
    for (int q = 0; q < 4; q++) {
      t[q][3] = tab_lookup(L, s[q], R[3], SEL0);
      t[q][2] = tab_lookup(L, s[q], R[2], SEL1);
      t[q][1] = tab_lookup(L, s[q], R[1], SEL2);
      t[q][0] = tab_lookup(L, s[q], R[0], SEL3);
    }
#pragma unroll
    for (int q = 0; q < 4; q++) s[q] = xor3(xor3(t[q][3], t[q][2], d[4 * q + j + 1]), t[q][1], t[q][0]);
    __builtin_amdgcn_sched_group_barrier(0x0002, 16, 0);
    __builtin_amdgcn_sched_group_barrier(0x0100, 16, 0);
    __builtin_amdgcn_sched_group_barrier(0x0002, 8, 0);
  }
  const uint32_t lb = lds_off(L.last);
  uint32_t t[4][4];
#pragma unroll
  for (int q = 0; q < 3; q++)
#pragma unroll
    for (int i = 0; i < 4; i++) t[q][i] = lds_ld(lb + 4096u * q + 1024u * i + 4u * ((s[q] >> (8 * i)) & 0xffu));
  t[3][3] = tab_lookup(L, s[3], R[3], SEL0);
  t[3][2] = tab_lookup(L, s[3], R[2], SEL1);
  t[3][1] = tab_lookup(L, s[3], R[1], SEL2);
  t[3][0] = tab_lookup(L, s[3], R[0], SEL3);
  uint32_t v[4];
#pragma unroll
  for (int q = 0; q < 4; q++) v[q] = xor3(t[q][0], t[q][1], t[q][2]) ^ t[q][3];
  __builtin_amdgcn_sched_group_barrier(0x0002, 16, 0);
  __builtin_amdgcn_sched_group_barrier(0x0100, 16, 0);
  const uint32_t r = xor3(v[0], v[1], v[2]) ^ v[3];
  __builtin_amdgcn_sched_barrier(0);
  return r;
}
__device__ __forceinline__ uint32_t lane_weight_or(uint32_t c, uint32_t lbase) {
  uint32_t v[8];
#pragma unroll
  for (int pos = 0; pos < 8; pos++) {
    const int sh = 4 * pos - 7;
    const uint32_t x = sh < 0 ? c << (-sh) : c >> sh;
    v[pos] = lds_ld(((x & 0x780u) | lbase) + pos * 2048);
  }
  return xor3(xor3(v[0], v[1], v[2]), xor3(v[3], v[4], v[5]), v[6] ^ v[7]);
}
__device__ __forceinline__ uint32_t half_suffix_xor(uint32_t v, int lane) {
  v ^= dpp<DPP_ROW_SHL + 1>(v);
  v ^= dpp<DPP_ROW_SHL + 2>(v);
  v ^= dpp<DPP_ROW_SHL + 4>(v);
  v ^= dpp<DPP_ROW_SHL + 8>(v);
  const uint32_t t = (uint32_t)__builtin_amdgcn_update_dpp(0, (int)v, 0x150, 0xA, 0xF, false);
  const auto sw = __builtin_amdgcn_permlane16_swap(t, 0u, false, false);
  (void)lane;
  return v ^ sw[1];
}

template <bool COAL = false>
__device__ __forceinline__ void load_crc_lds(ScanLds& lds) {
  static_assert(SCAN_WAVES_V2 * 64 == 1024 && sizeof(lds.nib) == 1024 * 16 && sizeof(lds.last) <= 1024 * 16,
                "one 16-byte piece of nib / last per thread");
  const uint32_t u = threadIdx.x;
  const uint32_t tv = g_tabs.tab[2 * (u >> 9) + (u & 1)][(u >> 1) & 255];
  const u32x4 nv = ((const u32x4*)(COAL ? g_tabs.nib_c : g_tabs.nib))[u];
  constexpr uint32_t NLAST = sizeof(lds.last) / 16;
  const u32x4 lv = ((const u32x4*)(COAL ? &g_tabs.last_c[0][0][0] : &g_tabs.last[0][0][0]))[u < NLAST ? u : 0];
  u32x4* const tr = (u32x4*)(lds.tab + 32 * u);
#pragma unroll
  for (int j = 0; j < 8; j++) tr[j] = u32x4{tv, tv, tv, tv};
  ((u32x4*)lds.nib)[u] = nv;
  if (u < NLAST) ((u32x4*)lds.last)[u] = lv;
  __syncthreads();
}
__device__ __forceinline__ void crc_lane_bases(uint32_t (&R)[4], int lane) {
#pragma unroll
  for (int t = 0; t < 4; t++) R[t] = ((uint32_t)(t >> 1) << 16) | ((uint32_t)(t & 1) * 128u + 4u * (lane & 31));
}

constexpr uint32_t TOP_WINDOW = 256;
__device__ __forceinline__ uint64_t find_top(const uint8_t* file, uint64_t flen, bool search) {
  const int lane = threadIdx.x & 63;
  const uint32_t steps = search ? TOP_WINDOW / 64 : 1;
  for (uint32_t s = 0; s < steps; s++) {
    const uint64_t d = (uint64_t)s * 64 + (uint64_t)lane;
    const bool has = (search || lane == 0) && flen >= 21 + d;
    const uint64_t m = (has ? flen - d : flen) - 20;
    uint64_t kh, p;
    uint32_t crc;
    ld_meta(file, m, &kh, &p, &crc);
    const uint32_t bw = *(const uint32_t*)(file + ((m - 1) & ~3ull));
    const bool zb = ((bw >> (8 * ((m - 1) & 3))) & 0xffu) == 0;
    const bool tomb = m > p && m - p == 1 && zb;
    const uint64_t es = tomb ? p : p + prepad64(p);
    const uint64_t pass = __ballot(has && es < m);
    if (!pass) continue;
    const int l = __builtin_ctzll(pass);
    const uint64_t pl = ((uint64_t)(uint32_t)__builtin_amdgcn_readlane((uint32_t)(p >> 32), l) << 32) |
                        (uint64_t)(uint32_t)__builtin_amdgcn_readlane((uint32_t)p, l);
    const uint32_t cl = (uint32_t)__builtin_amdgcn_readlane(crc, l);
    const bool zl = __builtin_amdgcn_readlane((uint32_t)zb, l) != 0;
    const uint64_t t = flen - ((uint64_t)s * 64 + (uint64_t)l), ml = t - 20, dp = ml - pl;
    const bool strong = pl >= 20 && pl < ml && cl != 0 && (dp > prepad64(pl) || (dp == 1 && zl));
    return (pl == 0 || strong) ? t : 0;
  }
  return 0;
}

__device__ void link_record(const ScanArgs& a, uint64_t w, uint64_t r) {
  const uint64_t gi = w * a.wcap + r;
  uint64_t gprev = 0;
  bool hp = true;
  if (r > 0) {
    gprev = gi - 1;
  } else if (w == 0) {
    hp = false;
  } else {
    const uint64_t wt = a.wave_total[w - 1] & ~(1ull << 63);
    hp = wt > 0 && wt <= a.wcap;
    gprev = (w - 1) * a.wcap + (hp ? wt - 1 : 0);
  }
  const bool hp2 = r >= 2;
  const uint64_t m = a.c_m[gi], mprev = hp ? a.c_m[gprev] : 0, mprev2 = hp2 ? a.c_m[gi - 2] : 0;
  const u32x4 r0 = a.c_rec[gi];
  const uint64_t p = (uint64_t)r0[0] | ((uint64_t)r0[1] << 32);
  bool node = true, tomb = false;
  if (r0[2] & F_NT) {
    const uint64_t dp = m - p;
    tomb = dp == 1 && (r0[2] & F_ZB);
    node = p >= 20 && p < m && (tomb || dp > prepad64(p));
  }
  const uint64_t mp = p - 20;
  const uint64_t sp2 = (mp + 14) / SPAN_BYTES;
  int64_t par = hp && mprev == mp ? (int64_t)gprev : hp2 && mprev2 == mp ? (int64_t)(gi - 2) : PAR_MISS;
  uint64_t pp = 1;
  const bool res = mp >= a.k_lo * (uint64_t)TILE;
  if (node && par == PAR_MISS && res) pp = ld_u64_unaligned(a.file, p - 12);
  const bool maybe_rec = !res || (pp >= 20 && pp < mp);
  if (node && par == PAR_MISS && maybe_rec && sp2 >= a.part.s_lo && sp2 < a.n_spans) {
    const uint64_t w2 = part_span_wave(a.part, sp2 - a.part.s_lo);
    const uint32_t f2 = a.span_first[sp2];
    const uint32_t n2 = (uint32_t)min<uint64_t>(a.span_count[sp2], a.wcap - min<uint64_t>(f2, a.wcap));
    uint32_t lo = 0, hi = n2;
    const uint64_t* cm = a.c_m + w2 * a.wcap + f2;
    while (lo < hi) {
      const uint32_t mid = (lo + hi) >> 1;
      if (cm[mid] < mp) lo = mid + 1; else hi = mid;
    }
    if (lo < n2 && cm[lo] == mp) par = (int64_t)(w2 * a.wcap + f2 + lo);
  }
  if (!node) {
    par = PAR_MISS;
  } else if (par == PAR_MISS) {
    if (a.span_lo) {
      if (p == a.span_lo) par = PAR_ROOT;
    } else if (p >= 21 && pp == 0) {
      par = PAR_ROOT;
    }
  }
  if (tomb) a.c_rec[gi] = u32x4{r0[0], r0[1], r0[2] | F_TOMB, r0[3]};
  a.d_par[gi] = (int32_t)par;
  if (par >= 0) atomicMax(&a.childof[par], claim_word(a.gen, gi));
}

constexpr uint32_t LINK_WPB = 1;
__device__ void xpart_update(const ScanArgs& a) {
  __shared__ unsigned long long s_sp[8], s_du[8], s_t0, s_t1;
  __shared__ float s_w[8];
  __shared__ double s_pre[256 / 64 + 1];
  XPart* xp = a.xp;
  const ScanPart& p = a.part;
  const uint32_t g = p.g, t = threadIdx.x, lane = t & 63, wv = t >> 6;
  if (t < 8) { s_sp[t] = 0; s_du[t] = 0; }
  if (t == 0) { s_t0 = ~0ull; s_t1 = 0; }
  __syncthreads();
  for (uint32_t b = t; b < g; b += 256) {
    const uint32_t x = xp->xcc[b] & 7u;
    const uint64_t t0 = xp->t0[b], du = xp->dur[b];
    atomicAdd(&s_sp[x], (unsigned long long)(part_block_start(p, b + 1) - part_block_start(p, b)));
    atomicAdd(&s_du[x], (unsigned long long)du);
    atomicMin(&s_t0, (unsigned long long)t0);
    atomicMax(&s_t1, (unsigned long long)(t0 + du));
  }
  __syncthreads();
  if (t == 0) {
    xp->scan_ticks = s_t1 > s_t0 ? s_t1 - s_t0 : 0;
    float sp[8], mean = 0;
    int nx = 0;
    for (int x = 0; x < 8; x++) {
      sp[x] = s_du[x] && s_sp[x] ? (float)s_sp[x] / (float)s_du[x] : 0.f;
      if (sp[x] > 0) { mean += sp[x]; nx++; }
    }
    mean = nx ? mean / nx : 1.f;
    for (int x = 0; x < 8; x++) {
      const float m = sp[x] > 0 ? sp[x] / mean : 1.f, old = xp->w[x];
      float v = old > 0 ? 0.25f * old + 0.75f * m : m;
      v = fminf(fmaxf(v, 1.f - XP_CLAMP), 1.f + XP_CLAMP);
      xp->w[x] = v;
      s_w[x] = v;
    }
  }
  __syncthreads();
  auto q_of = [&](uint32_t b) -> double { return b < g ? (double)s_w[xp->xcc[b] & 7u] : 0.0; };
  double part = 0;
  for (uint32_t b = t; b < g; b += 256) part += q_of(b);
#pragma unroll
  for (int o = 32; o; o >>= 1) part += __shfl_xor(part, o);
  if (lane == 0) s_pre[wv] = part;
  __syncthreads();
  const double tot = s_pre[0] + s_pre[1] + s_pre[2] + s_pre[3];
  __syncthreads();
  uint64_t* nb = xp->bs[a.xp_next];
  double acc = 0;
  for (uint32_t b0 = 0; b0 < g; b0 += 256) {
    const uint32_t b = b0 + t;
    const double q = q_of(b);
    double x = q;
#pragma unroll
    for (int o = 1; o < 64; o <<= 1) {
      const double y = __shfl_up(x, o);
      if ((int)lane >= o) x += y;
    }
    if (lane == 63) s_pre[wv] = x;
    __syncthreads();
    double wpre = 0, ctot = 0;
    for (uint32_t i = 0; i < 4; i++) {
      wpre += i < wv ? s_pre[i] : 0.0;
      ctot += s_pre[i];
    }
    __syncthreads();
    if (b < g) nb[b] = b == 0 ? 0 : (uint64_t)((double)p.ns * ((acc + wpre + x - q) / tot) + 0.5);
    acc += ctot;
  }
  if (t == 0) nb[g] = p.ns;
}
__device__ void scan_reduce(const ScanArgs& a, uint32_t n_waves) {
  __shared__ unsigned long long s_sum, s_smax, s_rmax, s_ovf;
  if (threadIdx.x == 0) { s_sum = 0; s_smax = 0; s_rmax = 0; s_ovf = 0; }
  __syncthreads();
  const uint32_t i = blockIdx.x * 256 + threadIdx.x;
  uint64_t sum = 0, smax = 0, rmax = 0, o = 0;
  if (i < n_waves) {
    const uint64_t v = a.wave_total[i], cnt = v & ~(1ull << 63);
    sum = cnt;
    o = v >> 63;
    rmax = a.wave_root[i];
    if (cnt) smax = (uint64_t)i * a.wcap + min(cnt, a.wcap);
  }
  rmax = wave_max_u64(rmax);
  smax = wave_max_u64(smax);
#pragma unroll
  for (int d = 32; d > 0; d >>= 1) {
    o |= __shfl_xor(o, d);
    sum += __shfl_xor(sum, d);
  }
  if ((threadIdx.x & 63) == 0) {
    atomicAdd(&s_sum, (unsigned long long)sum);
    atomicMax(&s_smax, (unsigned long long)smax);
    atomicMax(&s_rmax, (unsigned long long)rmax);
    atomicOr(&s_ovf, (unsigned long long)o);
  }
  __syncthreads();
  if (threadIdx.x == 0) {
    atomicAdd((unsigned long long*)&a.k_total[0], s_sum);
    atomicMax((unsigned long long*)&a.k_total[1], s_smax);
    atomicMax((unsigned long long*)&a.counters[0], s_rmax);
    atomicOr((unsigned long long*)&a.counters[2], s_ovf);
  }
}
__global__ __launch_bounds__(256 * LINK_WPB) void link2_kernel(ScanArgs a, uint32_t n_waves) {
  const uint64_t w = (uint64_t)blockIdx.x * LINK_WPB + threadIdx.x / 256;
  if (w < n_waves) {
    const uint64_t nrec = min(a.wave_total[w] & ~(1ull << 63), a.wcap);
    for (uint64_t r = threadIdx.x % 256; r < nrec; r += 256) link_record(a, w, r);
  }
  if ((uint64_t)blockIdx.x * 256 < n_waves) scan_reduce(a, n_waves);
  if (a.xp && blockIdx.x == min((n_waves + 255) / 256, gridDim.x - 1)) xpart_update(a);
}

__device__ __forceinline__ uint32_t coal_lane_off(int lane, int j) {
  return 1024u * (uint32_t)j + 256u * (((uint32_t)lane >> 2) & 3u) + 64u * ((uint32_t)lane & 3u) +
         16u * ((uint32_t)lane >> 4);
}
template <int RB, bool P32>
__device__ __forceinline__ void coal_pswap(uint32_t (&d)[16]) {
#pragma unroll
  for (int r0 = 0; r0 < 4; r0++) {
    if (r0 & RB) continue;
    const int r1 = r0 | RB;
#pragma unroll
    for (int i = 0; i < 4; i++) {
      const auto w = P32 ? __builtin_amdgcn_permlane32_swap(d[4 * r0 + i], d[4 * r1 + i], false, false)
                         : __builtin_amdgcn_permlane16_swap(d[4 * r0 + i], d[4 * r1 + i], false, false);
      d[4 * r0 + i] = w[0];
      d[4 * r1 + i] = w[1];
    }
  }
}
__device__ __forceinline__ void coal_to_lines(uint32_t (&d)[16]) {
  coal_pswap<1, false>(d);
  coal_pswap<2, true>(d);
}

constexpr int SCAN_LINES = 34;
constexpr int scan_nw(int) { return SCAN_WAVES_V2; }

template <bool FULL, bool WIDE, int V = 0>
__global__ __launch_bounds__(SCAN_WAVES_V2 * 64) __attribute__((amdgpu_waves_per_eu(4, 4)))
void scan_kernel(ScanArgs a) {
  constexpr int NW = SCAN_WAVES_V2;
  static_assert(V == 0 || V == SCAN_LINES || V == 7 || V == 8, "scan variants: 0, SCAN_LINES, 7, 8");
  constexpr bool COALT = V != SCAN_LINES;
  constexpr bool MEMONLY = V == 7, NOHBM = V == 8;
  uint32_t memonly_acc = 0;
  using Lds = ScanLds;
  __shared__ Lds lds;
  constexpr uint64_t RQ_LANES = 64;
  if (blockIdx.x == 0) {
    for (uint32_t i = threadIdx.x; i < a.n_zero_words; i += blockDim.x) a.zero_words[i] = 0;
    for (uint32_t i = threadIdx.x; i < a.n_zero2; i += blockDim.x) a.zero2[i] = 0;
    if (threadIdx.x == 0 && a.sentinel) *a.sentinel = 0;
    if (!FULL && threadIdx.x == 0) {
      a.k_total[0] = 0;
      a.k_total[1] = 0;
      a.counters[0] = 0;
      a.counters[2] = 0;
    }
  }
  uint64_t xp_t0 = 0;
  if (a.xp && threadIdx.x == 0) xp_t0 = __builtin_amdgcn_s_memrealtime();
#ifdef SRD_WAVE_STAMPS
  if (threadIdx.x == 0) {
    g_wave_stamp[8192 + blockIdx.x] = __builtin_amdgcn_s_memrealtime();
    if (blockIdx.x < 256) g_wave_clk[4096 + blockIdx.x] = __builtin_amdgcn_s_memtime();
    uint32_t xcc, hwid;
    asm volatile("s_getreg_b32 %0, hwreg(HW_REG_XCC_ID)" : "=s"(xcc));
    asm volatile("s_getreg_b32 %0, hwreg(HW_REG_HW_ID)" : "=s"(hwid));
    if (blockIdx.x < 256) g_wave_stamp[8192 + 512 + blockIdx.x] = ((uint64_t)hwid << 32) | xcc;
  }
#endif
  load_crc_lds(lds);
#ifdef SRD_WAVE_STAMPS
  if (threadIdx.x == 0 && blockIdx.x < 256) g_wave_stamp[8192 + 256 + blockIdx.x] = __builtin_amdgcn_s_memrealtime();
#endif

  const int lane = threadIdx.x & 63;
  const int wv = __builtin_amdgcn_readfirstlane(threadIdx.x >> 6);
  uint32_t R[4];
  crc_lane_bases(R, lane);
  const uint8_t* __restrict__ file = a.file;
  const uint64_t flen = a.flen;
  uint32_t* win = lds.win[wv];
  const uint32_t nib_lane = lds_off(lds.nib) + 4u * (lane & 31);
  auto line_crc = [&](const uint32_t (&x)[16]) -> uint32_t { return crc_line4(x, lds, R); };
  auto lane_wt = [&](uint32_t c) -> uint32_t { return lane_weight_or(c, nib_lane); };

  const uint64_t total_waves = (uint64_t)gridDim.x * NW;
  const uint64_t w = (uint64_t)blockIdx.x * NW + wv;
  uint64_t r0, r1;
  part_wave_range(a.part, blockIdx.x, (uint32_t)wv, &r0, &r1);
  uint64_t k0 = (a.part.s_lo + r0) * SPAN_TILES;
  uint64_t k1 = min((a.part.s_lo + r1) * SPAN_TILES, a.n_tiles);
  if (k0 >= k1) k0 = k1 = a.k_lo;

  const uint64_t top = FULL ? 0 : find_top(file, flen, a.m_lo == 0);
  if (!FULL && top == 0) {
    const uint64_t sa = k0 / SPAN_TILES, sb = (k1 + SPAN_TILES - 1) / SPAN_TILES;
    for (uint64_t sp = sa + lane; sp < sb; sp += 64) {
      a.span_count[sp] = 0;
      a.span_first[sp] = 0;
    }
    k0 = k1 = a.k_lo;
  }

  uint32_t count = 0;
  uint64_t wtotal = 0;
  bool ovf = false;
  uint32_t tacc0 = 0, tacc1 = 0, scnt = 0, sfirst = 0;
  bool tg_pend = false, sg_pend = false;
  uint64_t tg_base = 0, sg_base = 0;
  uint32_t tg_par = 0, tg_lo = 0, tg_hi = 0, sg_lo = 0, sg_hi = 0;
  uint32_t rq[10];
#pragma unroll
  for (int i = 0; i < 10; i++) rq[i] = 0;
  uint64_t flushed = 0;
  uint64_t rvalid = 0;

  const uint64_t nohbm_k = (a.part.s_lo + part_block_start(a.part, blockIdx.x)) * SPAN_TILES;
  auto load_tile = [&](uint64_t k, uint32_t (&o)[16]) {
    if constexpr (COALT) {
      const uint8_t* tb = file + (NOHBM ? nohbm_k + (k & 1) : k) * (uint64_t)TILE;
#pragma unroll
      for (int j = 0; j < 4; j++) {
        const u32x4 v = __builtin_nontemporal_load((const u32x4*)(tb + coal_lane_off(lane, j)));
        o[4 * j] = v[0]; o[4 * j + 1] = v[1]; o[4 * j + 2] = v[2]; o[4 * j + 3] = v[3];
      }
      return;
    }
    const u32x4* q = (const u32x4*)(file + k * (uint64_t)TILE + 64ull * lane);
#pragma unroll
    for (int j = 0; j < 4; j++) {
      const u32x4 v = q[j];
      o[4 * j] = v[0]; o[4 * j + 1] = v[1]; o[4 * j + 2] = v[2]; o[4 * j + 3] = v[3];
    }
  };

  const uint32_t hb = a.filt_hb;
  uint64_t rootmax = 0;
  {
    uint32_t pl[16];
    const bool has_prev = k0 > a.k_lo;
    const u32x4* q = (const u32x4*)(file + (has_prev ? k0 * (uint64_t)TILE - 64 : k0 * (uint64_t)TILE));
#pragma unroll
    for (int j = 0; j < 4; j++) {
      const u32x4 v = q[j];
      pl[4 * j] = v[0]; pl[4 * j + 1] = v[1]; pl[4 * j + 2] = v[2]; pl[4 * j + 3] = v[3];
    }
    const uint32_t cp = line_crc(pl);
    if (lane == 0) {
#pragma unroll
      for (int j = 0; j < 4; j++) win[j] = has_prev ? pl[12 + j] : 0u;
      win[22] = has_prev ? cp : 0u;
    }
  }

  auto next_head = [&](uint64_t k, uint32_t* n0, uint32_t* n1) {
    const __attribute__((address_space(4))) uint32_t* q =
        (const __attribute__((address_space(4))) uint32_t*)(file + (k + 1) * (uint64_t)TILE);
    *n0 = q[0];
    *n1 = q[1];
// ... 1035 lines not shown
```

rust-simd-r-drive_amd/csrc/srd_validate.hip:

```cpp

static int wait_publish(Ctx* c, uint64_t* w) {
  const uint32_t seq = c->pub_seq;
  volatile const uint64_t* pub = c->h_pub;
  const auto read = [&] {
    bool ok = true;
    for (int i = 0; i < PUB_WORDS; i++) {
      w[i] = pub[i];
      ok = ok && (uint32_t)(w[i] >> 32) == seq;
    }
    return ok;
  };
  for (uint64_t it = 0;; it++) {
    if (read()) return 0;
    if ((it & 1023) == 1023) {
      const hipError_t e = hipStreamQuery(c->stream);
      if (e == hipSuccess) {
        if (read()) return 0;
        set_err("internal: the glue finished without publishing its outcome");
        return SRD_ERR_INTERNAL;
      }
      if (e != hipErrorNotReady) HIPCHK(e);
    }
  }
}
// ... 144 lines not shown
  uint64_t h[8];
  counters_landed(c, h);
  out->n_index = nidx;
  out->n_crc_bad = h[6];
  out->n_chain = n;
  set_out_ptrs(c, out);
  return 0;
}

static int run_scan(Ctx* c, const uint8_t* d_file, uint64_t flen, uint64_t* K, uint64_t* h) {
  const uint64_t n_tiles = (flen + TILE - 1) / TILE;
  const uint64_t n_spans = (n_tiles + SPAN_TILES - 1) / SPAN_TILES;
  fit_cap(c->cfull, flen);
  while (true) {
    TRY(alloc_scan(c, n_tiles, n_spans, c->cfull.cap));
    TRY(ensure_cub(c, n_spans + 1));
    uint64_t* cnt = P<uint64_t>(c, B_COUNTERS);
    HIPCHK(hipMemsetAsync(cnt, 0, 64, c->stream));
    HIPCHK(hipMemsetAsync(P<uint32_t>(c, B_SPAN_COUNT) + n_spans, 0, 4, c->stream));
    ScanArgs a;
    TRY(scan_args(c, d_file, flen, scan_variant_for(c), c->cfull.cap, &a));
    a.tile = P<uint32_t>(c, B_TILE);
    a.span_count = P<uint32_t>(c, B_SPAN_COUNT);
    TRY(ensure(c, B_SPAN_FIRST, (n_spans + 1) * 4));
    a.span_first = P<uint32_t>(c, B_SPAN_FIRST);
    a.wcap = 0;
    if (n_spans) {
      uint32_t nw;
      const unsigned g = scan_grid(c, a.variant, n_spans, &nw);
      a.part = scan_part(c, 0, n_spans, g, nw);
      hipEvent_t e0, e1;
      TRY(next_scan_events(c, &e0, &e1));
      launch_scan<true>(g, a, c->stream, e0, e1);
      LAUNCHED(c->stream, "scan_kernel");
    }
    TRY(scan_sum(c, P<uint32_t>(c, B_SPAN_COUNT), P<uint64_t>(c, B_SPAN_BASE), n_spans + 1));
    TRY(read_counters(c, h, P<uint64_t>(c, B_SPAN_BASE) + n_spans, K));
    if (*K >= 0xFFFFFFFFull) { set_err("more than 2^32 - 2 chain-node candidates (full pass)"); return SRD_ERR_ALLOC; }
    if ((uint32_t)h[2] == 0) break;
    if (c->cfull.cap >= SPAN_BYTES) { set_err("candidate overflow"); return SRD_ERR_INTERNAL; }
    grow_cap(c->cfull, flen);
  }
  if (*K) {
    TRY(alloc_dense(c, *K));
    LinkArgs l{};
    l.file = d_file;
    l.flen = flen;
    l.n_spans = n_spans;
    l.cap = c->cfull.cap;
    l.span_count = P<uint32_t>(c, B_SPAN_COUNT);
    l.span_base = P<uint64_t>(c, B_SPAN_BASE);
    l.c_m = P<uint64_t>(c, B_CM);
    l.c_rec = P<u32x4>(c, B_CREC);
    l.d_m = P<uint64_t>(c, B_DM);
    l.d_par = P<int64_t>(c, B_DPAR);
    l.d_slot = P<uint64_t>(c, B_DSLOT);
    link_kernel<<<blocks(n_spans, 256 / LINK_LANES), 256, 0, c->stream>>>(l);
    LAUNCHED(c->stream, "link_kernel");
  } else {
    TRY(alloc_dense(c, 1));
  }
  return 0;
}

static int set_single_root(Ctx* c, uint64_t t) {
  WalkState w{};
  w.status = 1;
  w.chain_len = 1;
  w.root_t = t;
  w.final_len = t;
  HIPCHK(hipMemcpyAsync(P<WalkState>(c, B_WALK), &w, sizeof w, hipMemcpyHostToDevice, c->stream));
  return 0;
}

static int alloc_fast(Ctx* c, uint64_t capK, uint32_t log2_nbk) {
  TRY(ensure(c, B_DPAR, capK * 4));
  TRY(ensure_z(c, B_HASCHILD, capK * 4));
  TRY(ensure_z(c, B_HASCHILD2, capK * 4));
  TRY(ensure_z(c, B_CHILDOF, capK * 8));
  TRY(ensure(c, B_FLAG, capK));
  TRY(ensure(c, B_PART, GLUE_BLOCKS * 4));
  TRY(ensure(c, B_PARTEX, CHAIN_BLOCKS * CHAIN_WAVES * 4));
  TRY(ensure_z(c, B_LOOKB, CHAIN_BLOCKS * 8));
  TRY(ensure(c, B_PLAN, sizeof(Plan)));
  TRY(alloc_out(c, capK + 1));
  TRY(alloc_index(c, capK, log2_nbk));
  return 0;
}

struct OptAttempt {
  const uint8_t* d_file;
  uint64_t flen;
  uint32_t flags;
  uint32_t coff;
  uint32_t log2_nbk;
  uint32_t var;
  uint64_t total_waves;
  uint64_t wcap;
  uint64_t capK;
  uint32_t wpb;
  XPart* xp;
  ScanArgs a;
};

static int opt_scan(Ctx* c, OptAttempt& o, const ScanPart& part, unsigned g, uint64_t lo, uint64_t k_lo,
                    uint64_t s_lo) {
  ScanArgs& a = o.a;
  TRY(scan_args(c, o.d_file, o.flen, o.var, c->copt.cap, &a));
  a.part = part;
  a.xp = o.xp;
  a.xp_next = c->xp_par ^ 1u;
  a.tile = P<uint32_t>(c, B_TILE) - 4 * k_lo;
  a.span_count = P<uint32_t>(c, B_SPAN_COUNT) - s_lo;
  a.span_first = P<uint32_t>(c, B_SPAN_FIRST) - s_lo;
  a.wcap = o.wcap;
  a.k_lo = k_lo;
  a.m_lo = lo;
  a.zero_words = P<uint32_t>(c, B_PLAN);
  a.n_zero_words = (uint32_t)(sizeof(Plan) / 4);
  a.d_par = P<int32_t>(c, B_DPAR);
  a.childof = P<unsigned long long>(c, B_CHILDOF);
  a.gen = c->gen;
  a.span_lo = lo;
  a.zero2 = index_zero_words(c, o.log2_nbk, &a.n_zero2);
  hipEvent_t e0, e1;
  TRY(next_scan_events(c, &e0, &e1));
  launch_scan<false>(g, a, c->stream, e0, e1);
  LAUNCHED(c->stream, "scan_kernel");
  return 0;
}

static ShapeArgs shape_args(Ctx* c, const OptAttempt& o) {
  ShapeArgs sa{};
  sa.file = o.d_file;
  sa.flen = o.flen;
  sa.Kp = o.a.k_total;
  sa.wave_total = o.a.wave_total;
  sa.wcap = o.wcap;
  sa.n_waves = (uint32_t)o.total_waves;
  sa.wpb = o.wpb;
  sa.n_slots = o.capK;
  sa.coff = o.coff;
  sa.c_m = o.a.c_m;
  sa.d_par = o.a.d_par;
  sa.c_rec = o.a.c_rec;
  sa.childof = P<uint64_t>(c, B_CHILDOF);
  sa.flag = P<uint8_t>(c, B_FLAG);
  sa.part = P<uint32_t>(c, B_PART);
  sa.wpart = P<uint32_t>(c, B_PARTEX);
  sa.counters = P<const unsigned long long>(c, B_COUNTERS);
  sa.plan = P<Plan>(c, B_PLAN);
  sa.zero = index_zero_words(c, o.log2_nbk, &sa.n_zero);
  sa.lb_fail = c->lb_fail;
  return sa;
}

static int opt_outcome(Ctx* c, const OptAttempt& o, Plan* hp) {
  if (!(c->timing >= SRD_TIMING_CALL)) {
    uint64_t w[PUB_WORDS];
    TRY(wait_publish(c, w));
    const uint32_t fl = (uint32_t)w[0];
    if ((fl & 0x3ffu) == 0x100u) {
      scan_tune_feedback(c, o.var, (uint32_t)w[6]);
      *hp = Plan{};
      hp->n_chain = (uint32_t)w[1];
      hp->n_index = (uint32_t)w[2];
      hp->n_bad = (uint32_t)w[3];
      hp->K = (uint32_t)w[4];
      hp->top_gap = (uint32_t)w[5];
      hp->idx_alias = 1;
      return 0;
    }
  }
  HIPCHK(hipMemcpyAsync(c->h_plan, P<Plan>(c, B_PLAN), sizeof(Plan), hipMemcpyDeviceToHost, c->stream));
  HIPCHK(spin_sync(c->stream));
  *hp = *c->h_plan;
  return 0;
}

static int opt_glue(Ctx* c, const OptAttempt& o, Plan* hp) {
  Plan* pl = P<Plan>(c, B_PLAN);
  uint32_t* marks = P<uint32_t>(c, B_HASCHILD);
  uint32_t* marks2 = P<uint32_t>(c, B_HASCHILD2);
  uint32_t mgen = c->gen;
  const uint32_t log2_nbk = o.log2_nbk;
  for (int rounds = 0;; rounds += 2) {
    if (rounds) HIPCHK(hipMemsetAsync(pl, 0, sizeof(Plan), c->stream));
    ShapeArgs sa = shape_args(c, o);
    if (rounds == 0) {
      sa.has_child = nullptr;
      sa.gen = mgen;
    } else {
      if (rounds == 2) {
        sa.gen = mgen;
        marks_from_claims_kernel<<<GLUE_BLOCKS, GLUE_THREADS, 0, c->stream>>>(sa, marks);
        LAUNCHED(c->stream, "marks_from_claims_kernel");
      }
      for (int r = 0; r < 2; r++) {
        sa.has_child = marks;
        sa.gen = mgen;
        const uint32_t g2 = ++c->gen;
        prune_kernel<<<GLUE_BLOCKS, GLUE_THREADS, 0, c->stream>>>(sa, marks2, g2);
        LAUNCHED(c->stream, "prune_kernel");
        std::swap(marks, marks2);
        mgen = g2;
      }
      sa.has_child = marks;
      sa.gen = mgen;
      child2_kernel<<<GLUE_BLOCKS, GLUE_THREADS, 0, c->stream>>>(sa);
      LAUNCHED(c->stream, "child2_kernel");
    }
    const bool fused = rounds == 0 && c->glue_fused;
    if (!fused) {
      check_kernel<<<CHAIN_BLOCKS, CHAIN_THREADS, 0, c->stream>>>(sa);
      LAUNCHED(c->stream, "check_kernel");
    }
    FinArgs f = fin_args(c, o.d_file, o.flen, o.flags);
    f.tile = o.a.tile;
    f.coff = o.coff;
    f.n_bad = (unsigned long long*)&pl->n_bad;
    f.n_slow = (unsigned long long*)&pl->n_slow;
    f.o_packed = P<uint64_t>(c, B_O_PACKED);
    unsigned long long* lb = P<unsigned long long>(c, B_LOOKB);
    if (fused)
      chain_finalize_kernel<true><<<CHAIN_BLOCKS, CHAIN_THREADS, (1u << log2_nbk) * 4, c->stream>>>(
          sa, f, index_args(c, log2_nbk), log2_nbk, lb);
    else
      chain_finalize_kernel<false><<<CHAIN_BLOCKS, CHAIN_THREADS, (1u << log2_nbk) * 4, c->stream>>>(
          sa, f, index_args(c, log2_nbk), log2_nbk, lb);
    LAUNCHED(c->stream, "chain_finalize_kernel");
    TRY(launch_index_bucketed(c, f.o_kh, f.o_mo, &pl->n_chain, &pl->status, log2_nbk, P<uint64_t>(c, B_IKEY),
                              P<uint64_t>(c, B_IPACKED), pl, true, &f, false, o.xp ? &o.xp->scan_ticks : nullptr));
    if (c->timing >= SRD_TIMING_CALL) {
      HIPCHK(hipEventRecord(c->ev[3], c->stream));
      c->ev3_recorded = true;
    }
    TRY(opt_outcome(c, o, hp));
    if (debug_env()) {
      fprintf(stderr, "plan K=%lu n_chain=%lu root_t=%lu start=%lu n_index=%lu bad=%lu slow=%lu st=%u nroot=%u "
              "troot=%u idxov=%u log2nbk=%u capK=%lu rounds=%d\n",
              (unsigned long)hp->K, (unsigned long)hp->n_chain, (unsigned long)hp->root_t, (unsigned long)hp->start,
              (unsigned long)hp->n_index, (unsigned long)hp->n_bad, (unsigned long)hp->n_slow, hp->status, hp->nroot,
              hp->troot, hp->idx_overflow, log2_nbk, (unsigned long)o.capK, rounds);
    }
    const uint32_t retry_bits = ST_SHAPE | ST_ROOTS;
    if (!(hp->status & retry_bits) || (hp->status & ~retry_bits) || rounds >= 6) return 0;
  }
}

static int optimistic_pass(Ctx* c, const uint8_t* d_span, uint64_t span_off, uint64_t lo, uint64_t flen,
                           uint32_t flags, srd_device_result* out, bool* done) {
  *done = false;
  const uint64_t n_tiles = (flen + TILE - 1) / TILE;
  const uint64_t n_spans = (n_tiles + SPAN_TILES - 1) / SPAN_TILES;
  const uint64_t k_lo = span_off / TILE, s_lo = k_lo / SPAN_TILES;
  const uint64_t nt_rel = n_tiles - k_lo, ns_rel = n_spans - s_lo;
  OptAttempt o{};
  o.d_file = d_span - span_off;
  o.flen = flen;
  o.flags = flags;
  o.coff = lo ? 0u : 1u;
  fit_cap(c->copt, flen - span_off);
  for (int attempt = 0; attempt < 6; attempt++) {
    const uint64_t n_est = std::max<uint64_t>(std::max<uint64_t>(c->last_n, (flen - span_off) / 4096), 1);
    o.log2_nbk = index_log2_buckets(n_est);
    uint32_t nw;
    const unsigned g = scan_grid(c, 0, ns_rel, &nw);
    o.var = scan_variant_tune(c, ns_rel, g);
    c->last_loads = o.var == SCAN_LINES ? 1 : o.var == 0 ? 0 : -1;
    ScanPart part = scan_part(c, s_lo, ns_rel, g, nw);
    const bool xpart = c->xpart_on && g <= XP_MAX_BLOCKS;
    o.xp = nullptr;
    if (xpart) {
      TRY(ensure_z(c, B_XPART, sizeof(XPart)));
      o.xp = P<XPart>(c, B_XPART);
      if (c->xp_valid && c->xp_ns == ns_rel && c->xp_g == g) part.bs = &o.xp->bs[c->xp_par][0];
    }
    {
      Ctx::LastPart& l = c->xp_last;
      l.any = true;
      l.ns = ns_rel;
      l.g = g;
      l.par = c->xp_par;
      l.src = !part.bs ? SRD_SCAN_BLOCKS_EVEN : c->xp_installed ? SRD_SCAN_BLOCKS_INSTALLED : SRD_SCAN_BLOCKS_MEASURED;
      l.attempts = attempt + 1;
      if (!attempt) l.first_src = l.src;
    }
    o.total_waves = (uint64_t)g * nw;
    const uint64_t spw = part_max_wave_spans(part, xpart);
    o.wcap = spw * c->copt.cap;
    o.capK = o.total_waves * o.wcap;
    if (o.capK >= c->slot_limit) { out->full_reason = SRD_FULL_SLOT_SPACE; return 0; }
    o.wpb = (uint32_t)((o.total_waves + CHAIN_BLOCKS - 1) / CHAIN_BLOCKS);
    if (o.wpb > BW_MAX) { out->full_reason = SRD_FULL_WAVES; return 0; }
    TRY(alloc_scan(c, nt_rel, std::max<uint64_t>(ns_rel, o.total_waves * spw), c->copt.cap));
    TRY(ensure(c, B_SPAN_FIRST, (ns_rel + 1) * 4));
    TRY(alloc_fast(c, o.capK, o.log2_nbk));
    if (c->gen >= 0xFFFFFFF0u || c->gen == 0) {
      c->gen = 0;
      HIPCHK(hipMemsetAsync(P<void>(c, B_HASCHILD), 0, c->bufs[B_HASCHILD].n, c->stream));
      HIPCHK(hipMemsetAsync(P<void>(c, B_HASCHILD2), 0, c->bufs[B_HASCHILD2].n, c->stream));
      HIPCHK(hipMemsetAsync(P<void>(c, B_CHILDOF), 0, c->bufs[B_CHILDOF].n, c->stream));
    }
    ++c->gen;
    TRY(opt_scan(c, o, part, g, lo, k_lo, s_lo));
#ifdef SRD_DEBUG_API
    if (flags & kDbgScanOnly) {
      HIPCHK(hipStreamSynchronize(c->stream));
      *done = true;
      return 0;
    }
#endif
    link2_kernel<<<(unsigned)((o.total_waves + LINK_WPB - 1) / LINK_WPB), 256 * LINK_WPB, 0, c->stream>>>(
        o.a, (uint32_t)o.total_waves);
    LAUNCHED(c->stream, "link2_kernel");
    if (o.xp) {
      c->xp_par ^= 1u;
      c->xp_valid = true;
      c->xp_installed = false;
      c->xp_ns = ns_rel;
      c->xp_g = g;
    }
    Plan hp{};
    TRY(opt_glue(c, o, &hp));
    out->n_candidates = hp.K;
    if (hp.status & ST_OVERFLOW) {
      if (c->copt.cap >= SPAN_BYTES) { out->full_reason = SRD_FULL_CAP; return 0; }
      grow_cap(c->copt, flen - span_off);
      out->full_reason = SRD_FULL_CAP;
      continue;
    }
    if (hp.status) {
      out->full_reason = (hp.status & ST_LOOKBACK) ? SRD_FULL_LOOKBACK
                         : (hp.status & ST_NOSTART) ? SRD_FULL_NO_START
                                                    : SRD_FULL_UNPROVEN;
      return 0;
    }
    out->full_reason = SRD_FULL_NONE;
    out->final_len = flen - hp.top_gap;
    out->n_chain = hp.n_chain;
    out->n_crc_bad = hp.n_bad;
    out->n_index = hp.n_index;
    c->last_n = hp.n_chain;
    if (hp.idx_overflow) {
      c->ev3_recorded = false;
      TRY(index_global(c, hp.n_chain, &out->n_index));
      hp.idx_alias = 0;
    }
    set_out_ptrs(c, out);
    if (hp.idx_alias) {
      out->index_key_hash = P<uint64_t>(c, B_O_KH);
      out->index_packed = P<uint64_t>(c, B_O_PACKED);
    }
    *done = true;
    return 0;
  }
  return 0;
}

static int full_pass(Ctx* c, const uint8_t* d_file, uint64_t flen, uint32_t flags, srd_device_result* out) {
  uint64_t K = 0, h[8];
  out->mode = 1;
  TRY(run_scan(c, d_file, flen, &K, h));
  out->n_candidates = K;
  if (debug_env()) fprintf(stderr, "full pass: K=%lu candidates (reason %lu)\n", (unsigned long)K,
                           (unsigned long)out->full_reason);
  const uint64_t max_root = h[0];
  uint64_t best_g1 = 0, tlin = 0;
  if (K) {
    TRY(ensure(c, B_ST, K));
    TRY(ensure(c, B_JMP, K * 8));
    TRY(ensure(c, B_VFLAG, K * 4));
    const unsigned kb = blocks(K, 256);
    const int64_t* par = P<int64_t>(c, B_DPAR);
    uint8_t* core = P<uint8_t>(c, B_CORE);
    uint32_t* chead = P<uint32_t>(c, B_RUNHEAD);
    uint8_t* st = P<uint8_t>(c, B_ST);
    int64_t* jmp = P<int64_t>(c, B_JMP);
    TRY(core_runs(c, par, K, "core_flag_key_kernel", [&](unsigned nb, uint8_t* co, uint32_t* key) {
      core_flag_key_kernel<<<nb, 256, 0, c->stream>>>(co, K, key);
    }));
    status_init_kernel<<<kb, 256, 0, c->stream>>>(par, core, chead, K, st, jmp);
    LAUNCHED(c->stream, "status_init_kernel");
    uint64_t* cnt = P<uint64_t>(c, B_COUNTERS);
    int rounds = 1;
    while ((1ull << rounds) < K) rounds++;
    TRY(ensure(c, B_RFLAG, 4 * 72));
    unsigned int* rflag = P<unsigned int>(c, B_RFLAG);
    int done_rounds = 0;
    for (int pass = 0; pass < 8; pass++) {
      const int nr = std::max(1, std::min(pass ? 4 << pass : 12, rounds + 1 - done_rounds));
      done_rounds += nr;
      HIPCHK(hipMemsetAsync(rflag, 0, 4 * 72, c->stream));
      for (int r = 0; r < std::min(nr, 70); r++) {
        status_round_kernel<<<std::min(kb, 1024u), 256, 0, c->stream>>>(K, core, chead, st, jmp, rflag + r,
                                                                       r ? rflag + r - 1 : nullptr);
        LAUNCHED(c->stream, "status_round_kernel");
      }
      HIPCHK(hipMemsetAsync(cnt + 4, 0, 8, c->stream));
      status_round_kernel<<<std::min(kb, 1024u), 256, 0, c->stream>>>(K, core, chead, st, jmp, (unsigned int*)(cnt + 4),
                                                                     nullptr);
      LAUNCHED(c->stream, "status_round_kernel");
      TRY(read_counters(c, h));
      if (!h[4]) break;
      if (pass == 7) { set_err("internal: pointer jumping did not converge"); return SRD_ERR_INTERNAL; }
    }
    status_spread_core_kernel<<<kb, 256, 0, c->stream>>>(K, core, chead, st);
    LAUNCHED(c->stream, "status_spread_core_kernel");
    status_spread_leaf_kernel<<<kb, 256, 0, c->stream>>>(K, par, core, st);
    LAUNCHED(c->stream, "status_spread_leaf_kernel");
    const unsigned vb = blocks(K, 256);
    TRY(ensure(c, B_JMP, std::max<uint64_t>(K, vb) * 8));
    valid_max_kernel<<<vb, 256, 0, c->stream>>>(P<uint8_t>(c, B_ST), K, P<uint64_t>(c, B_JMP), P<uint32_t>(c, B_VFLAG));
    LAUNCHED(c->stream, "valid_max_kernel");
    max_reduce_kernel<<<1, 1024, 0, c->stream>>>(P<uint64_t>(c, B_JMP), vb, (unsigned long long*)(cnt + 3),
                                                 P<uint64_t>(c, B_DM), (unsigned long long*)(cnt + 7));
    LAUNCHED(c->stream, "max_reduce_kernel");
    TRY(read_counters(c, h));
    best_g1 = h[3];
    if (best_g1) tlin = h[7] + 20;
  }
  const uint64_t final_len = std::max(tlin, max_root);
  out->final_len = final_len;
  if (final_len == 0) return finish(c, d_file, flen, 0, flags, out);
  if (final_len == max_root && max_root > tlin) {
    TRY(set_single_root(c, final_len));
    return finish(c, d_file, flen, 1, flags, out);
  }
  TRY(ensure(c, B_VLIST, K * 8));
  TRY(ensure(c, B_NV, 8));
  TRY(ensure(c, B_VPOS, K * 8));
  TRY(ensure(c, B_VPAR, K * 8));
  TRY(ensure(c, B_VSLOT, K * 8));
  TRY(ensure(c, B_VSCAN, K * 4));
  TRY(scan_sum(c, P<uint32_t>(c, B_VFLAG), P<uint32_t>(c, B_VSCAN), K));
  compact_valid_kernel<<<blocks(K, 256), 256, 0, c->stream>>>(P<uint32_t>(c, B_VFLAG), P<uint32_t>(c, B_VSCAN), K,
                                                              P<uint64_t>(c, B_VLIST), P<uint64_t>(c, B_VPOS),
                                                              P<uint64_t>(c, B_NV));
  LAUNCHED(c->stream, "compact_valid_kernel");
  remap_kernel<<<blocks(K, 256), 256, 0, c->stream>>>(P<uint64_t>(c, B_VLIST), P<uint64_t>(c, B_NV),
                                                      P<int64_t>(c, B_DPAR), P<uint64_t>(c, B_VPOS),
                                                      P<int64_t>(c, B_VPAR), P<uint64_t>(c, B_VSLOT),
                                                      P<uint64_t>(c, B_DSLOT));
  LAUNCHED(c->stream, "remap_kernel");
  walk_start_kernel<<<1, 64, 0, c->stream>>>(P<WalkState>(c, B_WALK), P<uint64_t>(c, B_VPOS), best_g1 - 1);
  LAUNCHED(c->stream, "walk_start_kernel");
  uint64_t nv = 0;
  TRY(read_small(c, c->stream, {rd(P<uint64_t>(c, B_NV), &nv)}));
  WalkState hw{};
  TRY(walk_and_mark(c, P<int64_t>(c, B_VPAR), P<uint64_t>(c, B_VSLOT), nv, P<uint64_t>(c, B_VLIST), &hw));
  if (hw.status != 1) { set_err("internal: valid walk did not reach a root"); return SRD_ERR_INTERNAL; }
  return finish(c, d_file, flen, hw.chain_len, flags, out);
}

static int validate_device_impl(srd_ctx* c, const uint8_t* d_file, uint64_t flen, uint32_t flags,
                                srd_device_result* out) {
  if (!c || !out || (!d_file && flen)) { set_err("bad argument"); return SRD_ERR_ARG; }
  if (flen > kMaxFile) { set_err("stores above 2^48 bytes cannot be indexed (48-bit packed offsets)"); return SRD_ERR_ARG; }
  HIPCHK(hipSetDevice(c->device));
  memset(out, 0, sizeof *out);
  out->file_len = flen;
  if (flen < 21) {
    TRY(alloc_dense(c, 1));
    TRY(alloc_scan(c, 1, 1, c->copt.cap));
    return finish(c, d_file, flen, 0, flags, out);
  }
  if (flags & SRD_FLAG_FORCE_FULL) {
    out->full_reason = SRD_FULL_FORCED;
  } else {
    bool done = false;
    TRY(optimistic_pass(c, d_file, 0, 0, flen, flags, out, &done));
    if (done) return 0;
  }
  return full_pass(c, d_file, flen, flags, out);
}

static int call_begin(Ctx* c) {
// ... 62 lines not shown
```

rust-simd-r-drive_amd/srd_amd.py:

```python
from __future__ import annotations

import ctypes as C
import mmap as _mmap
import os
import subprocess

import numpy as np

HERE = os.path.dirname(os.path.abspath(__file__))
LIB_PATH = os.environ.get("SRD_LIB_PATH") or os.path.join(HERE, "build", "libsrd_amd.so")

SRD_FLAG_FORCE_FULL = 1
SRD_FLAG_NO_CRC = 2
SRD_FLAG_STAGE_PAGEABLE = 4
SRD_FLAG_STAGE_REGISTER = 8
STAGE_MODES = {0: "pinned input", 1: "registered mapping", 2: "bounce buffers", 3: "pageable copy"}
TIMING_NONE, TIMING_SCAN, TIMING_CALL = 0, 1, 2
SRD_MODE_OPTIMISTIC = 0
SRD_MODE_FULL = 1
SRD_MODE_SPAN_UNPROVEN = 3
SRD_FULL_NONE, SRD_FULL_FORCED, SRD_FULL_SLOT_SPACE, SRD_FULL_WAVES = 0, 1, 2, 3
SRD_FULL_NO_START, SRD_FULL_UNPROVEN, SRD_FULL_CAP, SRD_FULL_LOOKBACK = 4, 5, 6, 7
SRD_ERR_ARG, SRD_ERR_FULL = -3, -5
SCAN_BLOCKS_LAST, SCAN_BLOCKS_NEXT = 0, 1
SCAN_BLOCKS_EVEN, SCAN_BLOCKS_MEASURED, SCAN_BLOCKS_INSTALLED = 0, 1, 2
SRD_FLAG_MERGE_INDEX = 16
SRD_MULTI_COMPOSED, SRD_MULTI_NEIGHBOUR, SRD_MULTI_WHOLE_FILE = 0, 1, 2
SPAN_ALIGN = 16384
METADATA_SIZE = 20
NULL_BYTE = b"\x00"
TAG_BITS = 16
OFFSET_MASK = (1 << 48) - 1

EXPORTS = [
    "srd_ctx_create", "srd_ctx_destroy", "srd_ctx_stream", "srd_ctx_device_bytes", "srd_ctx_scan_loads",
    "srd_ctx_scan_trial", "srd_ctx_set_scan_blocks", "srd_ctx_scan_blocks",
    "srd_last_error", "srd_build_info",
    "srd_ctx_timings",
    "srd_ctx_set_timing",
    "srd_validate_index_device", "srd_validate_index", "srd_result_free",
    "srd_recover_valid_chain", "srd_key_indexer_build", "srd_crc32_batch",
    "srd_crc32_batch_device", "srd_xxh3_64_batch", "srd_xxh3_64_batch_device",
    "srd_synth_store_device", "srd_selftest_host", "srd_padded_size",
    "srd_validate_span_device", "srd_index_partition_device", "srd_index_build_device",
    "srd_synth_span_device", "srd_batch_layout", "srd_batch_write", "srd_batch_write_device",
    "srd_index_table_bytes", "srd_index_table_build_device", "srd_index_get_packed_device",
    "srd_batch_read_hashed_device", "srd_batch_read",
    "srd_iter_entries_device", "srd_estimate_compaction_savings_device", "srd_compact_device",
    "srd_shard_cuts", "srd_validate_index_multi", "srd_ctx_stage_info", "srd_index_hash_device",
    "srd_validate_index_multi_device", "srd_ctx_multi_summary", "srd_ctx_scan_list", "srd_ctx_set_timing_every",
    "srd_stream_probe_device", "srd_ctx_multi_shard_ms",
    "srd_index_table_apply_device", "srd_index_table_export_device", "srd_batch_delete_hashed_device",
    "srd_payload_gather_device", "srd_batch_append_device", "srd_compact_live_device",
]


class DeviceResult(C.Structure):
    _fields_ = [
        ("file_len", C.c_uint64), ("final_len", C.c_uint64), ("n_chain", C.c_uint64),
        ("n_index", C.c_uint64), ("n_crc_bad", C.c_uint64), ("n_candidates", C.c_uint64),
        ("full_reason", C.c_uint64), ("mode", C.c_uint32), ("reserved", C.c_uint32),
        ("meta_off", C.c_void_p), ("key_hash", C.c_void_p), ("prev_offset", C.c_void_p),
        ("payload_start", C.c_void_p), ("payload_len", C.c_void_p),
        ("crc_stored", C.c_void_p), ("crc_computed", C.c_void_p), ("crc_ok", C.c_void_p),
        ("index_key_hash", C.c_void_p), ("index_packed", C.c_void_p),
    ]


class ScanBlocksInfo(C.Structure):
    _fields_ = [("n_spans", C.c_uint64), ("n_blocks", C.c_uint32), ("source", C.c_uint32),
                ("attempts", C.c_uint32), ("first_source", C.c_uint32)]


class MultiSummary(C.Structure):
    _fields_ = [
        ("file_len", C.c_uint64), ("final_len", C.c_uint64), ("n_chain", C.c_uint64),
        ("n_index", C.c_uint64), ("n_crc_bad", C.c_uint64), ("n_candidates", C.c_uint64),
        ("mode", C.c_uint32), ("path", C.c_uint32), ("n_shards", C.c_uint32), ("merged", C.c_uint32),
        ("shard_errors", C.c_uint32), ("peer_errors", C.c_uint32),
        ("validate_ms", C.c_double), ("exchange_ms", C.c_double), ("total_ms", C.c_double),
        ("index_key_hash", C.c_void_p), ("index_packed", C.c_void_p),
    ]


class ApplyStats(C.Structure):
    _fields_ = [("n_inserted", C.c_uint64), ("n_updated", C.c_uint64), ("n_removed", C.c_uint64)]

    def as_tuple(self):
        return int(self.n_inserted), int(self.n_updated), int(self.n_removed)


class CompactStats(C.Structure):
    _fields_ = [("n_entries", C.c_uint64), ("new_len", C.c_uint64), ("kept_bytes", C.c_uint64),
                ("n_crc_bad", C.c_uint64), ("first_bad", C.c_uint64)]

    def __repr__(self):
        return "CompactStats(" + ", ".join(f"{n}={int(getattr(self, n))}" for n, _ in self._fields_) + ")"


def build_info() -> str:
    return lib().srd_build_info().decode()


def build() -> str:
    subprocess.check_call(["make", "-s", "-C", HERE])
    return LIB_PATH


_lib = None


def lib():
    global _lib
    if _lib is None:
        if not os.path.exists(LIB_PATH):
            raise RuntimeError(f"{LIB_PATH} missing: run `make -C {HERE}` (no CPU fallback exists)")
        try:
            import torch
        except Exception:
            pass
        L = C.CDLL(LIB_PATH)
        vp, u64, u32, i32 = C.c_void_p, C.c_uint64, C.c_uint32, C.c_int
        L.srd_build_info.restype = C.c_char_p
        L.srd_ctx_device_bytes.argtypes = [vp]
        L.srd_ctx_device_bytes.restype = u64
        L.srd_ctx_scan_loads.argtypes = [vp]
        L.srd_ctx_scan_trial.argtypes = [vp, C.POINTER(C.c_double)]
        L.srd_ctx_set_scan_blocks.argtypes = [vp, vp, u32, u64]
        L.srd_ctx_scan_blocks.argtypes = [vp, i32, vp, u32, C.POINTER(ScanBlocksInfo)]
        if not os.environ.get("SRD_LIB_PATH"):
            import importlib.util
            spec = importlib.util.spec_from_file_location("srd_src_hash", os.path.join(HERE, "src_hash.py"))
            sh = importlib.util.module_from_spec(spec)
            spec.loader.exec_module(sh)
            want, got = sh.source_hash(), L.srd_build_info().decode()
            if got != want:
                raise RuntimeError(f"{LIB_PATH} was built from other sources (sha256 {got}, the sources here "
                                   f"{want}): run `make -C {HERE}`")
        L.srd_ctx_create.argtypes = [i32, C.POINTER(vp)]
        L.srd_ctx_destroy.argtypes = [vp]
        L.srd_ctx_stream.argtypes = [vp]
        L.srd_ctx_stream.restype = vp
        L.srd_last_error.restype = C.c_char_p
        L.srd_ctx_timings.argtypes = [vp, C.POINTER(C.c_double), C.POINTER(C.c_int), C.POINTER(C.c_double)]
        L.srd_ctx_set_timing.argtypes = [vp, C.c_int]
        L.srd_ctx_scan_list.argtypes = [vp, C.POINTER(C.c_float), C.c_int]
        L.srd_ctx_set_timing_every.argtypes = [vp, C.c_int]
        L.srd_validate_index_device.argtypes = [vp, vp, u64, u32, C.POINTER(DeviceResult)]
        L.srd_validate_index.argtypes = [vp, vp, u64, u32, C.POINTER(DeviceResult)]
        L.srd_result_free.argtypes = [C.POINTER(DeviceResult)]
        L.srd_recover_valid_chain.argtypes = [vp, vp, u64, C.POINTER(u64)]
        L.srd_key_indexer_build.argtypes = [vp, vp, u64, vp, vp, u64, C.POINTER(u64)]
        L.srd_crc32_batch.argtypes = [vp, vp, u64, vp, vp, u64, vp]
        L.srd_crc32_batch_device.argtypes = [vp, vp, vp, vp, u64, vp, vp]
        L.srd_xxh3_64_batch.argtypes = [vp, vp, u64, vp, vp, u64, vp]
        L.srd_xxh3_64_batch_device.argtypes = [vp, vp, vp, vp, u64, vp, vp]
        L.srd_padded_size.argtypes = [u64]
        L.srd_padded_size.restype = u64
        L.srd_synth_store_device.argtypes = [vp, vp, u64, u64, vp, u64, C.POINTER(u64)]
        L.srd_validate_span_device.argtypes = [vp, vp, u64, u64, u64, u32, C.POINTER(DeviceResult)]
        L.srd_shard_cuts.argtypes = [vp, u64, u32, vp]
        L.srd_index_partition_device.argtypes = [vp, vp, vp, u64, u32, vp, vp]
        L.srd_index_build_device.argtypes = [vp, vp, u64, vp, vp, C.POINTER(u64)]
        L.srd_synth_span_device.argtypes = [vp, vp, u64, u64, u64, u64, vp, u64, C.POINTER(u64), C.POINTER(u64)]
        L.srd_batch_layout.argtypes = [u64, vp, vp, vp, vp, vp, u64, u32, vp, C.POINTER(u64)]
        L.srd_batch_write.argtypes = [vp, u64, vp, vp, vp, vp, vp, vp, u64, u32, vp, u64, C.POINTER(u64), vp, vp]
        L.srd_batch_write_device.argtypes = [vp, vp, vp, vp, u64, vp, u64, vp, vp, vp]
        L.srd_index_table_bytes.argtypes = [u64]
        L.srd_index_table_bytes.restype = u64
        L.srd_index_table_build_device.argtypes = [vp, vp, vp, u64, vp, u64]
        L.srd_index_get_packed_device.argtypes = [vp, vp, u64, vp, u64, vp, vp]
        L.srd_batch_read_hashed_device.argtypes = [vp, vp, u64, vp, u64, vp, vp, u64, vp, vp, vp]
        L.srd_batch_read.argtypes = [vp, vp, u64, vp, u64, vp, vp, vp, u64, vp, vp]
        L.srd_index_table_apply_device.argtypes = [vp, vp, u64, C.POINTER(u64), vp, vp, vp, u64,
                                                   C.POINTER(ApplyStats), vp]
        L.srd_index_table_export_device.argtypes = [vp, vp, u64, vp, vp, u64, C.POINTER(u64)]
        L.srd_batch_delete_hashed_device.argtypes = [vp, vp, u64, C.POINTER(u64), vp, u64, u64, vp, u64,
                                                     C.POINTER(u64), C.POINTER(u64)]
        L.srd_payload_gather_device.argtypes = [vp, vp, u64, vp, vp, u64, u32, vp, u64, vp, vp, vp,
                                                C.POINTER(u64), vp]
        L.srd_batch_append_device.argtypes = [vp, vp, u64, vp, vp, vp, u64, u32, u64, vp, u64, C.POINTER(u64), vp, vp]
        L.srd_compact_live_device.argtypes = [vp, vp, u64, vp, u64, vp, u64, vp, u64, C.POINTER(CompactStats)]
        L.srd_iter_entries_device.argtypes = [vp, vp, u64, vp, u64, vp, vp, vp, vp, C.POINTER(u64)]
        L.srd_estimate_compaction_savings_device.argtypes = [vp, vp, u64, vp, u64, C.POINTER(u64)]
        L.srd_compact_device.argtypes = [vp, vp, u64, vp, u64, vp, u64, C.POINTER(u64), vp, vp]
        L.srd_validate_index_multi.argtypes = [C.POINTER(vp), u32, vp, u64, u32, C.POINTER(DeviceResult)]
        L.srd_ctx_stage_info.argtypes = [vp, C.POINTER(i32), C.POINTER(C.c_double)]
        L.srd_index_hash_device.argtypes = [vp, vp, u64, vp, vp]
        L.srd_validate_index_multi_device.argtypes = [C.POINTER(vp), u32, C.POINTER(vp), vp, vp, u32,
                                                      C.POINTER(DeviceResult), C.POINTER(MultiSummary)]
        L.srd_ctx_multi_summary.argtypes = [vp, C.POINTER(MultiSummary)]
        L.srd_ctx_multi_shard_ms.argtypes = [vp, C.POINTER(C.c_double), i32]
        L.srd_stream_probe_device.argtypes = [vp, vp, u64, i32, C.POINTER(C.c_double), C.POINTER(C.c_double)]
        for f in EXPORTS:
            if f not in ("srd_ctx_destroy", "srd_result_free", "srd_ctx_stream", "srd_ctx_device_bytes", "srd_last_error",
                         "srd_build_info",
                         "srd_padded_size", "srd_index_table_bytes"):
                getattr(L, f).restype = i32
        _lib = L
    return _lib


class WriteEntry(C.Structure):
    _fields_ = [("src", C.c_uint64), ("len", C.c_uint64), ("key_src", C.c_uint64), ("tail", C.c_uint64),
                ("key_len", C.c_uint32), ("flags", C.c_uint32)]


WRITE_ALLOW_NULL = 1


class SrdError(RuntimeError):
    pass


def _check(rc):
    if rc != 0:
        raise SrdError(f"srd error {rc}: {lib().srd_last_error().decode()}")


class Context:

    def __init__(self, device: int = 0):
        self.device = device
        self.h = C.c_void_p()
        _check(lib().srd_ctx_create(device, C.byref(self.h)))

    def close(self):
        if self.h:
            lib().srd_ctx_destroy(self.h)
            self.h = C.c_void_p()

    def __del__(self):
        try:
            self.close()
        except Exception:
            pass

    def set_timing(self, level: int):
        _check(lib().srd_ctx_set_timing(self.h, level))

    def set_timing_every(self, n: int):
        _check(lib().srd_ctx_set_timing_every(self.h, n))

    def device_bytes(self) -> int:
        return int(lib().srd_ctx_device_bytes(self.h))

    def scan_loads(self) -> int:
        return int(lib().srd_ctx_scan_loads(self.h))

    def scan_trial(self):
        ms = (C.c_double * 2)()
        ch = int(lib().srd_ctx_scan_trial(self.h, ms))
        return ch, float(ms[0]), float(ms[1])

    def set_scan_blocks(self, starts, n_spans: int):
        st = np.ascontiguousarray(starts, dtype=np.uint64)
        _check(lib().srd_ctx_set_scan_blocks(self.h, C.c_void_p(st.ctypes.data), max(st.size, 1) - 1, n_spans))

    def scan_blocks(self, which: int = SCAN_BLOCKS_LAST):
        info = ScanBlocksInfo()
        _check(lib().srd_ctx_scan_blocks(self.h, which, None, 0, C.byref(info)))
        st = np.zeros(info.n_blocks + 1 if info.n_blocks else 0, np.uint64)
        if st.size:
            _check(lib().srd_ctx_scan_blocks(self.h, which, C.c_void_p(st.ctypes.data), st.size, C.byref(info)))
        return st, info

    def timings(self):
        a, n, b = C.c_double(), C.c_int(), C.c_double()
        _check(lib().srd_ctx_timings(self.h, C.byref(a), C.byref(n), C.byref(b)))
        return a.value, n.value, b.value

    def scan_list(self) -> list[float]:
        n = lib().srd_ctx_scan_list(self.h, None, 0)
        if n < 0:
            _check(n)
        buf = (C.c_float * max(n, 1))()
        lib().srd_ctx_scan_list(self.h, buf, n)
        return list(buf[:n])

    @property
    def stream(self) -> int:
        return lib().srd_ctx_stream(self.h)

    def stage_info(self) -> tuple[str, float]:
        m, ms = C.c_int(), C.c_double()
        _check(lib().srd_ctx_stage_info(self.h, C.byref(m), C.byref(ms)))
        return STAGE_MODES.get(m.value, "none"), ms.value

    def stage_mode(self) -> str:
        return self.stage_info()[0]

    def multi_summary(self) -> MultiSummary:
        m = MultiSummary()
        _check(lib().srd_ctx_multi_summary(self.h, C.byref(m)))
        return m


_default_ctx = None


def default_ctx() -> Context:
    global _default_ctx
    if _default_ctx is None:
        _default_ctx = Context(int(os.environ.get("SRD_DEVICE", "0")))
    return _default_ctx


def _u8(file) -> np.ndarray:
    if isinstance(file, np.ndarray):
        return np.ascontiguousarray(file, dtype=np.uint8).reshape(-1)
    return np.frombuffer(memoryview(file), dtype=np.uint8)


def _ptr(a: np.ndarray):
    return C.c_void_p(a.ctypes.data) if a.size else C.c_void_p(0)


class Result:

    def __init__(self, r: DeviceResult):
        self.file_len = r.file_len
        self.final_len = r.final_len
        self.n_chain = r.n_chain
        self.n_index = r.n_index
        self.n_crc_bad = r.n_crc_bad
        self.n_candidates = r.n_candidates
        self.full_reason = r.full_reason
        self.mode = r.mode

        def arr(p, n, dt):
            if n == 0 or not p:
                return np.zeros(0, dt)
            return np.ctypeslib.as_array(C.cast(p, C.POINTER(np.ctypeslib.as_ctypes_type(dt))), (n,)).copy()

        n, ni = r.n_chain, r.n_index
        self.meta_off = arr(r.meta_off, n, np.uint64)
        self.key_hash = arr(r.key_hash, n, np.uint64)
        self.prev_offset = arr(r.prev_offset, n, np.uint64)
        self.payload_start = arr(r.payload_start, n, np.uint64)
        self.payload_len = arr(r.payload_len, n, np.uint64)
        self.crc_stored = arr(r.crc_stored, n, np.uint32)
        self.crc_computed = arr(r.crc_computed, n, np.uint32)
        self.crc_ok = arr(r.crc_ok, n, np.uint8)
        self.index_key_hash = arr(r.index_key_hash, ni, np.uint64)
        self.index_packed = arr(r.index_packed, ni, np.uint64)

    def index(self) -> dict[int, int]:
        return {int(k): int(v) for k, v in zip(self.index_key_hash, self.index_packed)}

    def chain(self) -> list[dict]:
        keys = ["meta_off", "key_hash", "prev_offset", "payload_start", "payload_len",
                "crc_stored", "crc_computed", "crc_ok"]
        return [{k: int(getattr(self, k)[i]) for k in keys} for i in range(self.n_chain)]


def validate_index(file, flags: int = 0, ctx: Context | None = None) -> Result:
    ctx = ctx or default_ctx()
    a = _u8(file)
    r = DeviceResult()
    _check(lib().srd_validate_index(ctx.h, _ptr(a), a.size, flags, C.byref(r)))
    try:
        return Result(r)
    finally:
        lib().srd_result_free(C.byref(r))


def validate_index_call(file, flags: int = 0, ctx: Context | None = None) -> DeviceResult:
    ctx = ctx or default_ctx()
    a = _u8(file)
    r = DeviceResult()
    _check(lib().srd_validate_index(ctx.h, _ptr(a), a.size, flags, C.byref(r)))
    return r


def validate_index_multi(file, ctxs, flags: int = 0) -> Result:
    a = _u8(file)
    hs = (C.c_void_p * len(ctxs))(*[c.h.value for c in ctxs])
    r = DeviceResult()
    _check(lib().srd_validate_index_multi(hs, len(ctxs), _ptr(a), a.size, flags, C.byref(r)))
    try:
        return Result(r)
    finally:
        lib().srd_result_free(C.byref(r))


def validate_index_multi_device(ctxs, spans, span_offs, cuts, flags: int = 0):
    n = len(ctxs)
    hs = (C.c_void_p * n)(*[c.h.value for c in ctxs])
    sp = (C.c_void_p * n)(*[int(x or 0) for x in spans])
    so = np.ascontiguousarray(span_offs, np.uint64)
    cu = np.ascontiguousarray(cuts, np.uint64)
    assert so.size == n and cu.size == n + 1
    res = (DeviceResult * n)()
    summ = MultiSummary()
    _check(lib().srd_validate_index_multi_device(hs, n, sp, _ptr(so), _ptr(cu), flags, res, C.byref(summ)))
    return list(res), summ


def index_hash_device(d_keys: int, n: int, d_out: int, ctx: Context | None = None) -> None:
# ... 967 lines not shown
```

Before: 4858.

## Replace link2 pass with a speculative local wave-neighbour link check in finalize

Adds a local glue path that skips the separate link2 kernel. The fused chain-finalize kernel instead resolves each record's parent from neighbours within a small window, using wave shuffles across wave boundaries, and encodes the parent offset in the flag byte. It also computes K, max root and overflow with an in-kernel reduction, and folds the xpart update into extra blocks of the dedup kernel. If the local shape check fails, it falls back to link2 plus the normal rounds and stops trying the local path for that file for a while. The aim is to save a kernel launch and a full pass over the records, at the cost of extra work when the check fails.

```diff
diff --git a/include/srd_amd.h b/include/srd_amd.h
--- a/include/srd_amd.h
+++ b/include/srd_amd.h
@@ -38,6 +38,11 @@
 void *srd_ctx_stream(srd_ctx *ctx);
 uint64_t srd_ctx_device_bytes(srd_ctx *ctx);
 int srd_ctx_scan_loads(srd_ctx *ctx);
+#define SRD_GLUE_PATH_LOCAL 0
+#define SRD_GLUE_PATH_LINKED 1
+#define SRD_GLUE_PATH_LINKED_FAILED 2
+#define SRD_GLUE_PATH_LINKED_OFF 3
+int srd_ctx_glue_path(srd_ctx *ctx);
 int srd_ctx_scan_trial(srd_ctx *ctx, double *ms);
 #define SRD_SCAN_BLOCKS_LAST 0
 #define SRD_SCAN_BLOCKS_NEXT 1
diff --git a/rust-simd-r-drive_amd/csrc/srd_ctx.hip b/rust-simd-r-drive_amd/csrc/srd_ctx.hip
--- a/rust-simd-r-drive_amd/csrc/srd_ctx.hip
+++ b/rust-simd-r-drive_amd/csrc/srd_ctx.hip
@@ -107,6 +107,13 @@
   } tune;
   bool glue_fused = true;
   uint32_t lb_fail = ~0u;
+  bool glue_local = true;
+  int glue_path = SRD_GLUE_PATH_LINKED;
+  struct LocalOff {
+    bool off = false;
+    uint64_t ns = 0;
+    uint32_t g = 0, calls = 0;
+  } local_off;
   bool xpart_on = true, xp_valid = false;
   uint32_t xp_par = 0, xp_g = 0;
   uint64_t xp_ns = 0;
@@ -445,6 +452,11 @@
   c->glue_fused = fused != 0;
   return 0;
 }
+extern "C" int srd_debug_set_glue_local(srd_ctx* c, int local) {
+  if (!c) return SRD_ERR_ARG;
+  c->glue_local = local != 0;
+  return 0;
+}
 extern "C" int srd_debug_set_scan_weights(srd_ctx* c, const double* w, int n) {
   if (!c || !w || (n != 4 && n != 16)) return SRD_ERR_ARG;
   double f[16], sum = 0;
@@ -485,6 +497,7 @@
     else if (!strcmp(e, "coal")) c->loads_pin = 0;
   }
   if (const char* e = getenv("SRD_GLUE_FUSED")) c->glue_fused = strcmp(e, "0") != 0;
+  if (const char* e = getenv("SRD_GLUE_LOCAL")) c->glue_local = strcmp(e, "0") != 0;
   if (const char* e = getenv("SRD_XPART")) c->xpart_on = strcmp(e, "0") != 0;
   if (const char* e = getenv("SRD_LB_FAIL_BLOCK")) {
     char* end = nullptr;
@@ -544,6 +557,7 @@
 
 extern "C" void* srd_ctx_stream(srd_ctx* c) { return c ? (void*)c->stream : nullptr; }
 extern "C" int srd_ctx_scan_loads(srd_ctx* c) { return c ? c->last_loads : -1; }
+extern "C" int srd_ctx_glue_path(srd_ctx* c) { return c ? c->glue_path : -1; }
 extern "C" int srd_ctx_scan_trial(srd_ctx* c, double* ms) {
   if (!c) return -1;
   if (ms)
diff --git a/rust-simd-r-drive_amd/csrc/srd_glue.hip b/rust-simd-r-drive_amd/csrc/srd_glue.hip
--- a/rust-simd-r-drive_amd/csrc/srd_glue.hip
+++ b/rust-simd-r-drive_amd/csrc/srd_glue.hip
@@ -151,6 +151,8 @@
   uint32_t* zero;
   uint32_t n_zero;
   uint32_t lb_fail;
+  const uint64_t* wave_root;
+  uint64_t span_lo;
 };
 
 __device__ __forceinline__ uint64_t start_node(const ShapeArgs& a) {
@@ -418,10 +420,13 @@
 }
 
 
+constexpr uint8_t LOCAL_NOPAR = LINK_NB + 1;
+template <bool LOCAL = false>
 __device__ __forceinline__ bool fin_load_record(const ShapeArgs& a, const FinArgs& f, uint64_t gi, bool in, FinIn& e,
                                                 uint64_t& kh, int64_t& par, uint32_t& own_suf) {
-  const bool fl = in && a.flag[gi];
-  par = a.d_par[gi];
+  const uint8_t code = a.flag[gi];
+  const bool fl = in && code;
+  par = LOCAL ? (int64_t)code : (int64_t)a.d_par[gi];
   e.mo = f.c_m[gi];
   const u32x4 r0 = f.c_rec[gi], r1 = f.c_rec1[gi];
   e.p = (uint64_t)r0[0] | ((uint64_t)r0[1] << 32);
@@ -429,6 +434,7 @@
   e.crc_st = r0[3];
   e.sxv = r1[2];
   e.fl = r0[2];
+  if (LOCAL && link_node_test(e.mo, e.p, e.fl).tomb) e.fl |= F_TOMB;
   own_suf = r1[3];
   return fl;
 }
@@ -564,7 +570,107 @@
          ((uint64_t)(uint32_t)__builtin_amdgcn_readlane((uint32_t)(v >> 32), 63) << 32);
 }
 
-template <bool FUSED>
+__device__ __forceinline__ void local_check_wave(const ShapeArgs& a, uint64_t w, uint32_t n, uint32_t nprev,
+                                                 uint32_t nnext, uint64_t top, uint32_t& cnt, uint32_t& nr, bool& fail,
+                                                 unsigned long long* s_root_t) {
+  constexpr int HB = 2 * LINK_NB, HA = LINK_NB, STEP = 64 - HB - HA;
+  constexpr int CR = 5;
+  const int lane = threadIdx.x & 63;
+  const uint64_t gb = w * a.wcap;
+  for (uint32_t base0 = 0; base0 < n; base0 += CR * STEP) {
+    uint64_t g[CR], mg[CR];
+    u32x4 r0[CR];
+    bool have[CR];
+#pragma unroll
+    for (int r = 0; r < CR; r++) {
+      const int64_t i = (int64_t)base0 + r * STEP + lane - HB;
+      g[r] = gb;
+      have[r] = base0 + r * STEP < n;
+      if (!have[r]) continue;
+      if (i >= 0 && i < (int64_t)n) {
+        g[r] = gb + (uint64_t)i;
+      } else if (i < 0) {
+        if ((uint32_t)(-i) <= nprev) g[r] = gb - a.wcap + (nprev - (uint32_t)(-i));
+        else have[r] = link_slot_before(a.wave_total, a.wcap, w, 0, (uint32_t)(-i), &g[r]);
+      } else {
+        const uint32_t j = (uint32_t)(i - (int64_t)n);
+        if (j < nnext) g[r] = gb + a.wcap + j;
+        else have[r] = link_slot_after(a.wave_total, a.wcap, a.n_waves, w, n - 1, j + 1, &g[r]);
+      }
+      if (!have[r]) g[r] = gb;
+    }
+#pragma unroll
+    for (int r = 0; r < CR; r++) {
+      mg[r] = a.c_m[g[r]];
+      r0[r] = a.c_rec[g[r]];
+    }
+#pragma unroll
+    for (int r = 0; r < CR; r++) {
+      if (base0 + r * STEP >= n) break;
+      const int64_t i = (int64_t)base0 + r * STEP + lane - HB;
+      const uint64_t m = have[r] ? mg[r] : ~0ull;
+      const uint64_t p = (uint64_t)r0[r][0] | ((uint64_t)r0[r][1] << 32);
+      const bool node = have[r] && link_node_test(mg[r], p, r0[r][2]).node;
+      uint64_t mb[LINK_NB];
+#pragma unroll
+      for (int k = 1; k <= LINK_NB; k++) mb[k - 1] = __shfl(m, (lane - k) & 63);
+      int off = link_local_parent(node, p, 1, a.span_lo, mb, min(lane, LINK_NB));
+      int oa[LINK_NB];
+#pragma unroll
+      for (int j = 1; j <= LINK_NB; j++) oa[j - 1] = __shfl(off, (lane + j) & 63);
+      const bool claimed = link_local_claimed(oa, min(63 - lane, LINK_NB));
+      const bool mine = have[r] && lane >= HB && lane < 64 - HA && i < (int64_t)n;
+      bool start = false;
+      if (mine && top >= 21 && mg[r] == top - 20) {
+        uint64_t nx;
+        start = !link_slot_after(a.wave_total, a.wcap, a.n_waves, w, (uint64_t)i, 1, &nx);
+      }
+      if (off == LINK_MISS && node && (claimed || start) && !a.span_lo &&
+          link_root_rule(p, ld_u64_unaligned(a.file, p - 12), 0))
+        off = LINK_ROOT;
+      int ob[LINK_NB - 1];
+#pragma unroll
+      for (int j = 1; j < LINK_NB; j++) ob[j - 1] = __shfl(off, (lane - j) & 63);
+      const int poff = __shfl(off, (lane - (off >= 1 ? off : 1)) & 63);
+      const LinkShape s = link_local_shape(start, claimed, off, poff, off >= 1 && link_local_holds(off, ob));
+      if (!mine) continue;
+      GST(a.flag[g[r]], (uint8_t)(s == LINK_LEAF ? 0 : off >= 1 ? off : LOCAL_NOPAR));
+      if (s == LINK_LEAF) continue;
+      cnt++;
+      fail = fail || s == LINK_FAIL;
+      if (s == LINK_ROOTED) {
+        nr++;
+        *s_root_t = p;
+      }
+    }
+  }
+}
+__device__ __forceinline__ void local_reduce(const ShapeArgs& a, uint32_t t0, unsigned long long* red) {
+  if (threadIdx.x < t0) return;
+  uint64_t sum = 0, smax = 0, rmax = 0, o = 0;
+  for (uint32_t i = threadIdx.x - t0; i < a.n_waves; i += blockDim.x - t0) {
+    const uint64_t v = a.wave_total[i], c = v & ~(1ull << 63);
+    sum += c;
+    o |= v >> 63;
+    rmax = max(rmax, a.wave_root[i]);
+    if (c) smax = max(smax, (uint64_t)i * a.wcap + min(c, a.wcap));
+  }
+#pragma unroll
+  for (int d = 32; d; d >>= 1) {
+    sum += __shfl_xor(sum, d);
+    o |= __shfl_xor(o, d);
+    smax = max(smax, (uint64_t)__shfl_xor(smax, d));
+    rmax = max(rmax, (uint64_t)__shfl_xor(rmax, d));
+  }
+  if ((threadIdx.x & 63) == 0) {
+    atomicAdd(&red[0], (unsigned long long)sum);
+    atomicMax(&red[1], (unsigned long long)smax);
+    atomicMax(&red[2], (unsigned long long)rmax);
+    atomicOr(&red[3], (unsigned long long)o);
+  }
+}
+
+template <bool FUSED, bool LOCAL = false>
 __global__ __launch_bounds__(CHAIN_THREADS) void chain_finalize_kernel(ShapeArgs a, FinArgs f, IdxArgs ia,
                                                                       uint32_t log2_nbk,
                                                                       unsigned long long* lb_desc) {
@@ -576,8 +682,10 @@
   GLUE_STAMP(0);
   uint32_t ltw[FIN_LDS_WORDS];
   fin_lds_words(lt, threadIdx.x, ltw, false);
-  const uint64_t K = a.Kp[0];
-  const bool incomplete = dense_incomplete(a);
+  static_assert(FUSED || !LOCAL, "the local check is a form of the fused one");
+  uint64_t K = LOCAL ? 0 : a.Kp[0], max_root = LOCAL ? 0 : a.counters[0], overflow = LOCAL ? 0 : a.counters[2];
+  const bool incomplete = LOCAL ? false : dense_incomplete(a);
+  __shared__ unsigned long long red[4];
   uint64_t before = 0, total = 0;
   if constexpr (!FUSED)
     block_prefix_n<CHAIN_WAVES>(a.part, incomplete ? 0u : (uint32_t)CHAIN_BLOCKS, wsum, &before, &total);
@@ -591,7 +699,7 @@
   };
   const bool troot = a.coff && top >= 21 && ld_prev_at(top - 12) == 0;
   uint64_t root_t = troot ? top : FUSED ? 0 : pl->root_t;
-  if (a.counters[2]) st |= ST_OVERFLOW;
+  if (overflow) st |= ST_OVERFLOW;
   const uint64_t s1 = a.Kp[1];
   const uint64_t start = FUSED ? NO_NODE : incomplete ? NO_NODE : start_node(a);
   if (!FUSED && start == NO_NODE) st |= ST_NOSTART;
@@ -601,9 +709,9 @@
   const uint32_t nbk = 1u << log2_nbk;
   auto write_plan = [&](uint32_t s2, uint64_t tot) {
     pl->K = K;
-    pl->max_root = a.counters[0];
+    pl->max_root = max_root;
     pl->top_gap = top ? a.flen - top : 0;
-    pl->overflow = a.counters[2];
+    pl->overflow = overflow;
     pl->troot = troot;
     if (troot) {
       pl->status = 0;
@@ -619,6 +727,15 @@
   };
   const bool plan_block = FUSED ? blockIdx.x + 1 == gridDim.x : blockIdx.x == 0;
   if (!FUSED && plan_block && threadIdx.x == 0) write_plan(st, total);
+  if (LOCAL && troot && plan_block) {
+    if (threadIdx.x < 4) red[threadIdx.x] = 0;
+    __syncthreads();
+    local_reduce(a, 0, red);
+    __syncthreads();
+    K = red[0];
+    max_root = red[2];
+    overflow = red[3];
+  }
   if (FUSED && troot && plan_block && threadIdx.x == 0) write_plan(0, 0);
   if (st && !troot) return;
   __shared__ uint32_t s_vcnt[BW_MAX];
@@ -628,6 +745,7 @@
   if constexpr (FUSED) {
     if (!troot) {
       if (threadIdx.x == 0) { s_fail = 0; s_nroot = 0; s_root_t = 0; }
+      if (LOCAL && threadIdx.x < 4) red[threadIdx.x] = 0;
       __syncthreads();
       const uint64_t tag = (uint64_t)a.gen << 32;
       const uint32_t wi = threadIdx.x >> 6, lane = threadIdx.x & 63;
@@ -641,7 +759,13 @@
         int64_t c_par = PAR_MISS;
         uint64_t c_cg = 0;
         uint32_t cnt = 0;
-        for (uint32_t base = 0; base < n; base += CR * 64) {
+        if constexpr (LOCAL) {
+          if (w < a.n_waves && (a.wave_total[w] >> 63)) fail = true;
+          const uint32_t nprev = w > 0 && w - 1 < a.n_waves ? (uint32_t)link_wave_count(a.wave_total, a.wcap, w - 1) : 0u;
+          const uint32_t nnext = w + 1 < a.n_waves ? (uint32_t)link_wave_count(a.wave_total, a.wcap, w + 1) : 0u;
+          if (n) local_check_wave(a, w, n, nprev, nnext, top, cnt, nr, fail, &s_root_t);
+        }
+        for (uint32_t base = 0; !LOCAL && base < n; base += CR * 64) {
           uint64_t g[CR], cg[CR], cp[CR];
           int64_t par[CR], pp[CR];
           bool in[CR], need[CR];
@@ -708,6 +832,8 @@
       for (uint32_t v = 0; v < a.wpb; v++) btot += s_vcnt[v];
       const uint32_t ltag = lb_tag(a.gen);
       typedef __attribute__((address_space(1))) unsigned long long gu64;
+      __shared__ uint32_t s_pst;
+      if (LOCAL && plan_block) local_reduce(a, 64, red);
       if (threadIdx.x == 0 && blockIdx.x > 0)
         __hip_atomic_store((gu64*)(lb_desc + blockIdx.x), lb_pack(ltag, 1, s_fail, s_nroot, btot), __ATOMIC_RELAXED,
                            __HIP_MEMORY_SCOPE_AGENT);
@@ -725,7 +851,8 @@
           s_lb[0] = pc;
           s_lb[1] = pc + btot;
           s_lbok = ok;
-          if (plan_block) {
+          if (LOCAL) s_pst = (ok ? 0u : ST_LOOKBACK) | (f2 ? ST_SHAPE : 0u) | (n2 != 1 ? ST_ROOTS : 0u);
+          if (!LOCAL && plan_block) {
             const uint64_t stn = incomplete ? NO_NODE : start_node(a);
             pl->start = stn;
             write_plan((ok ? 0u : ST_LOOKBACK) | (f2 ? ST_SHAPE : 0u) | (n2 != 1 ? ST_ROOTS : 0u) |
@@ -738,6 +865,15 @@
       GLUE_STAMP(2);
       before = s_lb[0];
       total = s_lb[1];
+      if (LOCAL && plan_block && threadIdx.x == 0) {
+        K = red[0];
+        max_root = red[2];
+        overflow = red[3];
+        const uint64_t e1 = red[1];
+        const uint64_t stn = !overflow && e1 && top >= 21 && a.c_m[e1 - 1] == top - 20 ? e1 - 1 : NO_NODE;
+        pl->start = stn;
+        write_plan(s_pst | (overflow ? ST_OVERFLOW : 0u) | (stn == NO_NODE ? ST_NOSTART : 0u), total);
+      }
       if (!s_lbok) return;
       root_t = s_root_t;
     }
@@ -783,7 +919,14 @@
           for (int r = 0; r < FIN_R; r++) {
             const uint32_t i = base + (uint32_t)r * 64 + lane;
             gi[r] = gb + (i < n ? i : 0u);
-            fl[r] = fin_load_record(a, f, gi[r], i < n, e[r], kh[r], par[r], psuf[r]);
+            fl[r] = fin_load_record<LOCAL>(a, f, gi[r], i < n, e[r], kh[r], par[r], psuf[r]);
+            if constexpr (LOCAL) {
+              const uint32_t k = (uint32_t)par[r];
+              uint64_t ps = 0;
+              par[r] = !fl[r] || k > (uint32_t)LINK_NB ? PAR_ROOT
+                       : i >= k ? (int64_t)(gi[r] - k)
+                       : link_slot_before(a.wave_total, a.wcap, w, i, k, &ps) ? (int64_t)ps : PAR_ROOT;
+            }
           }
           const uint32_t tot = fin_rank(fl, lt_mask, rank);
           bool any = false, need[FIN_R];
@@ -953,7 +1096,15 @@
 
 constexpr int DD_SLOTS = 3 * IDX_TCAP / 2;
 constexpr uint32_t DD_EMPTY32 = 0xFFFFFFFFu;
-__global__ __launch_bounds__(512) __attribute__((amdgpu_waves_per_eu(8, 8))) void idx_dedup_kernel(IdxArgs a, FinArgs f) {
+constexpr uint32_t IDX_XBLOCKS = 8;
+__global__ __launch_bounds__(512) __attribute__((amdgpu_waves_per_eu(8, 8))) void idx_dedup_kernel(IdxArgs a, FinArgs f,
+                                                                                                  ScanArgs xa) {
+  const uint32_t xb = xa.xp ? IDX_XBLOCKS : 0u;
+  if (blockIdx.x < xb) {
+    if (blockIdx.x == 0) xpart_update<512>(xa);
+    return;
+  }
+  const uint32_t bid = blockIdx.x - xb, nblk = gridDim.x - xb;
   __shared__ unsigned long long dd_lds[DD_SLOTS + DD_SLOTS / 2];
   unsigned long long* const keys = dd_lds;
   uint32_t* const vals = (uint32_t*)(dd_lds + DD_SLOTS);
@@ -961,18 +1112,18 @@
   if (f.n_slow) {
     const unsigned long long ns = *f.n_slow;
     constexpr uint32_t NW = 512 / 64;
-    if ((uint64_t)blockIdx.x * NW < ns) {
+    if ((uint64_t)bid * NW < ns) {
       static_assert(sizeof(SlowLds) <= sizeof(dd_lds), "the slow path's tables in the hash table's LDS");
       SlowLds& L = *reinterpret_cast<SlowLds*>(dd_lds);
       load_slow_lds(L);
       __syncthreads();
-      for (uint64_t q = (uint64_t)blockIdx.x * NW + (threadIdx.x >> 6); q < ns; q += (uint64_t)gridDim.x * NW)
+      for (uint64_t q = (uint64_t)bid * NW + (threadIdx.x >> 6); q < ns; q += (uint64_t)nblk * NW)
         slow_one(f, f.slow_list[q], L);
       __syncthreads();
     }
   }
   if (*a.status) return;
-  const uint32_t k = blockIdx.x;
+  const uint32_t k = bid;
   const uint32_t fill = a.bfill[k];
   if (fill == 0) return;
   if (fill > IDX_TCAP) {
diff --git a/rust-simd-r-drive_amd/csrc/srd_index_build.hip b/rust-simd-r-drive_amd/csrc/srd_index_build.hip
--- a/rust-simd-r-drive_amd/csrc/srd_index_build.hip
+++ b/rust-simd-r-drive_amd/csrc/srd_index_build.hip
@@ -77,7 +77,7 @@
 static int launch_index_bucketed(Ctx* c, const uint64_t* kh, const uint64_t* mo, const uint64_t* n_dev,
                                  const uint32_t* status, uint32_t log2_nbk, uint64_t* okey, uint64_t* opacked,
                                  Plan* pl, bool fused = false, const FinArgs* slow = nullptr, bool zeroed = false,
-                                 const uint64_t* scan_ticks = nullptr) {
+                                 const uint64_t* scan_ticks = nullptr, const ScanArgs* xpart = nullptr) {
   TRY(next_lgen(c));
   IdxArgs ia = index_args(c, log2_nbk);
   ia.alias = fused ? 1u : 0u;
@@ -103,7 +103,9 @@
   }
   FinArgs fs{};
   if (slow) fs = *slow;
-  idx_dedup_kernel<<<nbk, 512, 0, c->stream>>>(ia, fs);
+  ScanArgs xa{};
+  if (xpart) xa = *xpart;
+  idx_dedup_kernel<<<nbk + (xa.xp ? IDX_XBLOCKS : 0u), 512, 0, c->stream>>>(ia, fs, xa);
   LAUNCHED(c->stream, "idx_dedup_kernel");
   idx_emit_kernel<<<GLUE_BLOCKS, GLUE_THREADS, 0, c->stream>>>(ia);
   LAUNCHED(c->stream, "idx_emit_kernel");
diff --git a/rust-simd-r-drive_amd/csrc/srd_kernels.hip b/rust-simd-r-drive_amd/csrc/srd_kernels.hip
--- a/rust-simd-r-drive_amd/csrc/srd_kernels.hip
+++ b/rust-simd-r-drive_amd/csrc/srd_kernels.hip
@@ -5,6 +5,7 @@
 #include "srd_xxh3.h"
 #include "srd_part.h"
 #include "srd_fin.h"
+#include "srd_link.h"
 
 namespace srd {
 
@@ -15,10 +16,6 @@
 
 constexpr int SPAN_TILES = 4;
 constexpr uint64_t SPAN_BYTES = (uint64_t)TILE * SPAN_TILES;
-constexpr int64_t PAR_ROOT = -1;
-constexpr int64_t PAR_MISS = -2;
-
-constexpr uint32_t F_NT = 256u, F_ZB = 512u;
 
 struct DevTables {
   uint32_t tab[4][256];
@@ -365,19 +362,16 @@
   const uint64_t m = a.c_m[gi], mprev = hp ? a.c_m[gprev] : 0, mprev2 = hp2 ? a.c_m[gi - 2] : 0;
   const u32x4 r0 = a.c_rec[gi];
   const uint64_t p = (uint64_t)r0[0] | ((uint64_t)r0[1] << 32);
-  bool node = true, tomb = false;
-  if (r0[2] & F_NT) {
-    const uint64_t dp = m - p;
-    tomb = dp == 1 && (r0[2] & F_ZB);
-    node = p >= 20 && p < m && (tomb || dp > prepad64(p));
-  }
+  const LinkNode nt = link_node_test(m, p, r0[2]);
+  const bool node = nt.node, tomb = nt.tomb;
   const uint64_t mp = p - 20;
   const uint64_t sp2 = (mp + 14) / SPAN_BYTES;
-  int64_t par = hp && mprev == mp ? (int64_t)gprev : hp2 && mprev2 == mp ? (int64_t)(gi - 2) : PAR_MISS;
+  int64_t par = hp && link_is_parent(mprev, p) ? (int64_t)gprev
+                : hp2 && link_is_parent(mprev2, p) ? (int64_t)(gi - 2) : PAR_MISS;
   uint64_t pp = 1;
   const bool res = mp >= a.k_lo * (uint64_t)TILE;
   if (node && par == PAR_MISS && res) pp = ld_u64_unaligned(a.file, p - 12);
-  const bool maybe_rec = !res || (pp >= 20 && pp < mp);
+  const bool maybe_rec = !res || link_parent_possible(pp, p);
   if (node && par == PAR_MISS && maybe_rec && sp2 >= a.part.s_lo && sp2 < a.n_spans) {
     const uint64_t w2 = part_span_wave(a.part, sp2 - a.part.s_lo);
     const uint32_t f2 = a.span_first[sp2];
@@ -392,12 +386,8 @@
   }
   if (!node) {
     par = PAR_MISS;
-  } else if (par == PAR_MISS) {
-    if (a.span_lo) {
-      if (p == a.span_lo) par = PAR_ROOT;
-    } else if (p >= 21 && pp == 0) {
-      par = PAR_ROOT;
-    }
+  } else if (par == PAR_MISS && link_root_rule(p, pp, a.span_lo)) {
+    par = PAR_ROOT;
   }
   if (tomb) a.c_rec[gi] = u32x4{r0[0], r0[1], r0[2] | F_TOMB, r0[3]};
   a.d_par[gi] = (int32_t)par;
@@ -405,17 +395,18 @@
 }
 
 constexpr uint32_t LINK_WPB = 1;
+template <int NT>
 __device__ void xpart_update(const ScanArgs& a) {
   __shared__ unsigned long long s_sp[8], s_du[8], s_t0, s_t1;
   __shared__ float s_w[8];
-  __shared__ double s_pre[256 / 64 + 1];
+  __shared__ double s_pre[NT / 64 + 1];
   XPart* xp = a.xp;
   const ScanPart& p = a.part;
   const uint32_t g = p.g, t = threadIdx.x, lane = t & 63, wv = t >> 6;
   if (t < 8) { s_sp[t] = 0; s_du[t] = 0; }
   if (t == 0) { s_t0 = ~0ull; s_t1 = 0; }
   __syncthreads();
-  for (uint32_t b = t; b < g; b += 256) {
+  for (uint32_t b = t; b < g; b += NT) {
     const uint32_t x = xp->xcc[b] & 7u;
     const uint64_t t0 = xp->t0[b], du = xp->dur[b];
     atomicAdd(&s_sp[x], (unsigned long long)(part_block_start(p, b + 1) - part_block_start(p, b)));
@@ -444,16 +435,17 @@
   __syncthreads();
   auto q_of = [&](uint32_t b) -> double { return b < g ? (double)s_w[xp->xcc[b] & 7u] : 0.0; };
   double part = 0;
-  for (uint32_t b = t; b < g; b += 256) part += q_of(b);
+  for (uint32_t b = t; b < g; b += NT) part += q_of(b);
 #pragma unroll
   for (int o = 32; o; o >>= 1) part += __shfl_xor(part, o);
   if (lane == 0) s_pre[wv] = part;
   __syncthreads();
-  const double tot = s_pre[0] + s_pre[1] + s_pre[2] + s_pre[3];
+  double tot = 0;
+  for (int i = 0; i < NT / 64; i++) tot += s_pre[i];
   __syncthreads();
   uint64_t* nb = xp->bs[a.xp_next];
   double acc = 0;
-  for (uint32_t b0 = 0; b0 < g; b0 += 256) {
+  for (uint32_t b0 = 0; b0 < g; b0 += NT) {
     const uint32_t b = b0 + t;
     const double q = q_of(b);
     double x = q;
@@ -465,7 +457,7 @@
     if (lane == 63) s_pre[wv] = x;
     __syncthreads();
     double wpre = 0, ctot = 0;
-    for (uint32_t i = 0; i < 4; i++) {
+    for (uint32_t i = 0; i < NT / 64; i++) {
       wpre += i < wv ? s_pre[i] : 0.0;
       ctot += s_pre[i];
     }
@@ -516,7 +508,7 @@
     for (uint64_t r = threadIdx.x % 256; r < nrec; r += 256) link_record(a, w, r);
   }
   if ((uint64_t)blockIdx.x * 256 < n_waves) scan_reduce(a, n_waves);
-  if (a.xp && blockIdx.x == min((n_waves + 255) / 256, gridDim.x - 1)) xpart_update(a);
+  if (a.xp && blockIdx.x == min((n_waves + 255) / 256, gridDim.x - 1)) xpart_update<256 * LINK_WPB>(a);
 }
 
 __device__ __forceinline__ uint32_t coal_lane_off(int lane, int j) {
diff --git a/rust-simd-r-drive_amd/csrc/srd_link.h b/rust-simd-r-drive_amd/csrc/srd_link.h
--- /dev/null
+++ b/rust-simd-r-drive_amd/csrc/srd_link.h
@@ -0,0 +1,105 @@
+#pragma once
+#include <stdint.h>
+
+#include "srd_fin.h"
+
+namespace srd {
+
+constexpr int64_t PAR_ROOT = -1;
+constexpr int64_t PAR_MISS = -2;
+
+constexpr uint32_t F_NT = 256u, F_ZB = 512u;
+
+struct LinkNode {
+  bool node, tomb;
+};
+SRD_FIN_HD LinkNode link_node_test(uint64_t m, uint64_t p, uint32_t fl) {
+  LinkNode r = {true, false};
+  if (fl & F_NT) {
+    const uint64_t dp = m - p;
+    r.tomb = dp == 1 && (fl & F_ZB);
+    r.node = p >= 20 && p < m && (r.tomb || dp > prepad64(p));
+  }
+  return r;
+}
+
+SRD_FIN_HD bool link_is_parent(uint64_t mc, uint64_t p) { return mc == p - 20; }
+
+SRD_FIN_HD bool link_parent_possible(uint64_t pp, uint64_t p) { return pp >= 20 && pp < p - 20; }
+
+SRD_FIN_HD bool link_root_rule(uint64_t p, uint64_t pp, uint64_t span_lo) {
+  return span_lo ? p == span_lo : (p >= 21 && pp == 0);
+}
+
+constexpr int LINK_NB = 4;
+constexpr int LINK_ROOT = -1, LINK_MISS = -2;
+
+SRD_FIN_HD int link_local_parent(bool node, uint64_t p, uint64_t pp, uint64_t span_lo, const uint64_t* mb, int nb) {
+  if (!node) return LINK_MISS;
+  SRD_UNROLL
+  for (int k = 1; k <= LINK_NB; k++)
+    if (k <= nb && link_is_parent(mb[k - 1], p)) return k;
+  return link_root_rule(p, pp, span_lo) ? LINK_ROOT : LINK_MISS;
+}
+SRD_FIN_HD bool link_found(int off) { return off >= 1 || off == LINK_ROOT; }
+
+SRD_FIN_HD bool link_local_claimed(const int* oa, int na) {
+  bool c = false;
+  SRD_UNROLL
+  for (int j = 1; j <= LINK_NB; j++) c = c || (j <= na && oa[j - 1] == j);
+  return c;
+}
+SRD_FIN_HD bool link_local_holds(int k, const int* ob) {
+  bool h = true;
+  SRD_UNROLL
+  for (int j = 1; j < LINK_NB; j++) h = h && !(j < k && ob[j - 1] == k - j);
+  return h;
+}
+
+enum LinkShape { LINK_LEAF, LINK_CORE, LINK_ROOTED, LINK_FAIL };
+SRD_FIN_HD LinkShape link_local_shape(bool is_start, bool claimed, int off, int poff, bool holds) {
+  if (!(is_start || (claimed && link_found(off)))) return LINK_LEAF;
+  if (off == LINK_ROOT) return LINK_ROOTED;
+  if (off < 1 || !link_found(poff)) return LINK_FAIL;
+  return holds ? LINK_CORE : LINK_FAIL;
+}
+
+template <class WT>
+SRD_FIN_HD uint64_t link_wave_count(const WT& wave_total, uint64_t wcap, uint64_t w) {
+  const uint64_t c = (uint64_t)wave_total[w] & ~(1ull << 63);
+  return c < wcap ? c : wcap;
+}
+template <class WT>
+SRD_FIN_HD bool link_slot_before(const WT& wave_total, uint64_t wcap, uint64_t w, uint64_t r, uint32_t k, uint64_t* slot) {
+  for (;;) {
+    if (r >= k) {
+      *slot = w * wcap + (r - k);
+      return true;
+    }
+    k -= (uint32_t)r;
+    do {
+      if (w == 0) return false;
+      w--;
+      r = link_wave_count(wave_total, wcap, w);
+    } while (r == 0);
+  }
+}
+template <class WT>
+SRD_FIN_HD bool link_slot_after(const WT& wave_total, uint64_t wcap, uint64_t n_waves, uint64_t w, uint64_t r, uint32_t k,
+                                uint64_t* slot) {
+  uint64_t left = link_wave_count(wave_total, wcap, w) - r - 1;
+  for (;;) {
+    if (left >= k) {
+      *slot = w * wcap + (r + k);
+      return true;
+    }
+    k -= (uint32_t)left;
+    do {
+      if (++w >= n_waves) return false;
+      left = link_wave_count(wave_total, wcap, w);
+    } while (left == 0);
+    r = ~0ull;
+  }
+}
+
+}
diff --git a/rust-simd-r-drive_amd/csrc/srd_validate.hip b/rust-simd-r-drive_amd/csrc/srd_validate.hip
--- a/rust-simd-r-drive_amd/csrc/srd_validate.hip
+++ b/rust-simd-r-drive_amd/csrc/srd_validate.hip
@@ -320,6 +320,8 @@
   sa.plan = P<Plan>(c, B_PLAN);
   sa.zero = index_zero_words(c, o.log2_nbk, &sa.n_zero);
   sa.lb_fail = c->lb_fail;
+  sa.wave_root = o.a.wave_root;
+  sa.span_lo = o.a.span_lo;
   return sa;
 }
 
@@ -346,16 +348,23 @@
   return 0;
 }
 
-static int opt_glue(Ctx* c, const OptAttempt& o, Plan* hp) {
+static int launch_link2(Ctx* c, const OptAttempt& o) {
+  link2_kernel<<<(unsigned)((o.total_waves + LINK_WPB - 1) / LINK_WPB), 256 * LINK_WPB, 0, c->stream>>>(
+      o.a, (uint32_t)o.total_waves);
+  LAUNCHED(c->stream, "link2_kernel");
+  return 0;
+}
+
+static int opt_glue(Ctx* c, OptAttempt& o, Plan* hp, bool* local) {
   Plan* pl = P<Plan>(c, B_PLAN);
   uint32_t* marks = P<uint32_t>(c, B_HASCHILD);
   uint32_t* marks2 = P<uint32_t>(c, B_HASCHILD2);
   uint32_t mgen = c->gen;
   const uint32_t log2_nbk = o.log2_nbk;
-  for (int rounds = 0;; rounds += 2) {
-    if (rounds) HIPCHK(hipMemsetAsync(pl, 0, sizeof(Plan), c->stream));
+  for (int rounds = *local ? -1 : 0;; rounds += rounds < 0 ? 1 : 2) {
+    if (rounds > 0) HIPCHK(hipMemsetAsync(pl, 0, sizeof(Plan), c->stream));
     ShapeArgs sa = shape_args(c, o);
-    if (rounds == 0) {
+    if (rounds <= 0) {
       sa.has_child = nullptr;
       sa.gen = mgen;
     } else {
@@ -378,7 +387,7 @@
       child2_kernel<<<GLUE_BLOCKS, GLUE_THREADS, 0, c->stream>>>(sa);
       LAUNCHED(c->stream, "child2_kernel");
     }
-    const bool fused = rounds == 0 && c->glue_fused;
+    const bool fused = rounds < 0 || (rounds == 0 && c->glue_fused);
     if (!fused) {
       check_kernel<<<CHAIN_BLOCKS, CHAIN_THREADS, 0, c->stream>>>(sa);
       LAUNCHED(c->stream, "check_kernel");
@@ -390,7 +399,10 @@
     f.n_slow = (unsigned long long*)&pl->n_slow;
     f.o_packed = P<uint64_t>(c, B_O_PACKED);
     unsigned long long* lb = P<unsigned long long>(c, B_LOOKB);
-    if (fused)
+    if (rounds < 0)
+      chain_finalize_kernel<true, true><<<CHAIN_BLOCKS, CHAIN_THREADS, (1u << log2_nbk) * 4, c->stream>>>(
+          sa, f, index_args(c, log2_nbk), log2_nbk, lb);
+    else if (fused)
       chain_finalize_kernel<true><<<CHAIN_BLOCKS, CHAIN_THREADS, (1u << log2_nbk) * 4, c->stream>>>(
           sa, f, index_args(c, log2_nbk), log2_nbk, lb);
     else
@@ -398,7 +410,8 @@
           sa, f, index_args(c, log2_nbk), log2_nbk, lb);
     LAUNCHED(c->stream, "chain_finalize_kernel");
     TRY(launch_index_bucketed(c, f.o_kh, f.o_mo, &pl->n_chain, &pl->status, log2_nbk, P<uint64_t>(c, B_IKEY),
-                              P<uint64_t>(c, B_IPACKED), pl, true, &f, false, o.xp ? &o.xp->scan_ticks : nullptr));
+                              P<uint64_t>(c, B_IPACKED), pl, true, &f, false, o.xp ? &o.xp->scan_ticks : nullptr,
+                              rounds < 0 && o.xp ? &o.a : nullptr));
     if (c->timing >= SRD_TIMING_CALL) {
       HIPCHK(hipEventRecord(c->ev[3], c->stream));
       c->ev3_recorded = true;
@@ -410,6 +423,18 @@
               (unsigned long)hp->K, (unsigned long)hp->n_chain, (unsigned long)hp->root_t, (unsigned long)hp->start,
               (unsigned long)hp->n_index, (unsigned long)hp->n_bad, (unsigned long)hp->n_slow, hp->status, hp->nroot,
               hp->troot, hp->idx_overflow, log2_nbk, (unsigned long)o.capK, rounds);
+    }
+    if (rounds < 0) {
+      const uint32_t relink = ST_SHAPE | ST_ROOTS | ST_NOSTART;
+      if (!(hp->status & relink) || (hp->status & ~relink)) return 0;
+      *local = false;
+      mgen = ++c->gen;
+      o.a.gen = mgen;
+      o.a.xp = nullptr;
+      HIPCHK(hipMemsetAsync(pl, 0, sizeof(Plan), c->stream));
+      HIPCHK(hipMemsetAsync(sa.zero, 0, (size_t)sa.n_zero * 4, c->stream));
+      TRY(launch_link2(c, o));
+      continue;
     }
     const uint32_t retry_bits = ST_SHAPE | ST_ROOTS;
     if (!(hp->status & retry_bits) || (hp->status & ~retry_bits) || rounds >= 6) return 0;
@@ -479,9 +504,16 @@
       return 0;
     }
 #endif
-    link2_kernel<<<(unsigned)((o.total_waves + LINK_WPB - 1) / LINK_WPB), 256 * LINK_WPB, 0, c->stream>>>(
-        o.a, (uint32_t)o.total_waves);
-    LAUNCHED(c->stream, "link2_kernel");
+    bool local = c->glue_local && c->glue_fused;
+    c->glue_path = SRD_GLUE_PATH_LINKED;
+    Ctx::LocalOff& lo_st = c->local_off;
+    const bool off_here = lo_st.off && lo_st.ns == ns_rel && lo_st.g == g;
+    if (local && off_here && ++lo_st.calls % 4096 != 0) {
+      local = false;
+      c->glue_path = SRD_GLUE_PATH_LINKED_OFF;
+    }
+    const bool tried = local;
+    if (!local) TRY(launch_link2(c, o));
     if (o.xp) {
       c->xp_par ^= 1u;
       c->xp_valid = true;
@@ -490,7 +522,12 @@
       c->xp_g = g;
     }
     Plan hp{};
-    TRY(opt_glue(c, o, &hp));
+    TRY(opt_glue(c, o, &hp, &local));
+    if (tried) {
+      c->glue_path = local ? SRD_GLUE_PATH_LOCAL : SRD_GLUE_PATH_LINKED_FAILED;
+      if (!local) lo_st = {true, ns_rel, g, 0};
+      else if (off_here) lo_st.off = false;
+    }
     out->n_candidates = hp.K;
     if (hp.status & ST_OVERFLOW) {
       if (c->copt.cap >= SPAN_BYTES) { out->full_reason = SRD_FULL_CAP; return 0; }
diff --git a/rust-simd-r-drive_amd/srd_amd.py b/rust-simd-r-drive_amd/srd_amd.py
--- a/rust-simd-r-drive_amd/srd_amd.py
+++ b/rust-simd-r-drive_amd/srd_amd.py
@@ -29,11 +29,13 @@
 SPAN_ALIGN = 16384
 METADATA_SIZE = 20
 NULL_BYTE = b"\x00"
+GLUE_PATH_LOCAL, GLUE_PATH_LINKED, GLUE_PATH_LINKED_FAILED, GLUE_PATH_LINKED_OFF = 0, 1, 2, 3
 TAG_BITS = 16
 OFFSET_MASK = (1 << 48) - 1
 
 EXPORTS = [
     "srd_ctx_create", "srd_ctx_destroy", "srd_ctx_stream", "srd_ctx_device_bytes", "srd_ctx_scan_loads",
+    "srd_ctx_glue_path",
     "srd_ctx_scan_trial", "srd_ctx_set_scan_blocks", "srd_ctx_scan_blocks",
     "srd_last_error", "srd_build_info",
     "srd_ctx_timings",
@@ -125,6 +127,7 @@
         L.srd_ctx_device_bytes.argtypes = [vp]
         L.srd_ctx_device_bytes.restype = u64
         L.srd_ctx_scan_loads.argtypes = [vp]
+        L.srd_ctx_glue_path.argtypes = [vp]
         L.srd_ctx_scan_trial.argtypes = [vp, C.POINTER(C.c_double)]
         L.srd_ctx_set_scan_blocks.argtypes = [vp, vp, u32, u64]
         L.srd_ctx_scan_blocks.argtypes = [vp, i32, vp, u32, C.POINTER(ScanBlocksInfo)]
@@ -245,6 +248,9 @@
     def device_bytes(self) -> int:
         return int(lib().srd_ctx_device_bytes(self.h))
 
+    def glue_path(self) -> int:
+        return int(lib().srd_ctx_glue_path(self.h))
+
     def scan_loads(self) -> int:
         return int(lib().srd_ctx_scan_loads(self.h))
 
```

Result: no change. 4892 (median of 6 runs) (+0.7%).
